# tkwa/iit

Measured on AMD Instinct MI355X. Metric: IIT (base,source) intervened pairs/sec, IOI GPT-2-small, IOI_ModelPair IIT+strict+behavior step, higher is better.
Workload: dtype bf16; 1 GPU; model=gpt2-small 12L/768d/12H (TL GPT-2 cfg, LNPre, gelu_new, V=50257), global_batch=256, seq_len=16, parallelism=dp1, engine=native, graphs=True

## Files before the change

### csrc/attn_mfma.hip

```cpp
#include "common.h"
#include "splice_spec.h"

typedef __attribute__((address_space(3))) i16x4 lds_i16x4_t;

__device__ __forceinline__ bf16x8 half_frag(const i16x4 v) {
  const i16x4 z = {0, 0, 0, 0};
  return __builtin_bit_cast(bf16x8, (i16x8)__builtin_shufflevector(v, z, 0, 1, 2, 3, 4, 5, 6, 7));
}

__device__ __forceinline__ bf16x8 regs_frag(float a, float b, float c, float d) {
  bf16x8 o = {f2bf(a), f2bf(b), f2bf(c), f2bf(d), f2bf(0.f), f2bf(0.f), f2bf(0.f), f2bf(0.f)};
  return o;
}

__device__ __forceinline__ bf16x8 load8(const __bf16* p, bool ok) {
  if (!ok) {
    const i16x8 z = {0, 0, 0, 0, 0, 0, 0, 0};
    return __builtin_bit_cast(bf16x8, z);
  }
  return *(const bf16x8*)p;
}

template <int LDSR>
__device__ __forceinline__ i16x4 tr_block(const __bf16* img, int g, int lane_in_group, int col0) {
  const int q = lane_in_group >> 2, p = lane_in_group & 3;
  return __builtin_amdgcn_ds_read_tr16_b64_v4i16((lds_i16x4_t*)(img + (4 * g + q) * LDSR + col0 + 4 * p));
}


template <int DH, bool SP>
__global__ __launch_bounds__(256) void attn_mfma_fwd_kernel(const __bf16* __restrict__ qkv, __bf16* __restrict__ z,
                                                            float* __restrict__ lse, const __bf16* __restrict__ zsrc,
                                                            unsigned long long head_mask, int BH, int S, int H,
                                                            long ld_qkv, long ld_z, long ld_src, float scale,
                                                            int causal, __bf16* __restrict__ z2, int pair_seqs,
                                                            unsigned long long pair_mask, SpliceSpec sp, int use_sp) {
  constexpr int LDSR = DH + 8;
  __shared__ __attribute__((aligned(16))) __bf16 smem[4][16 * LDSR];
  const int wave = threadIdx.x >> 6, l = threadIdx.x & 63, g = l >> 4, c = l & 15;
  const int bh = blockIdx.x * 4 + wave;
  const bool valid = bh < BH;
  const int b = valid ? bh / H : 0, h = valid ? bh % H : 0;
  const int HD = H * DH;
  const long row0 = (long)b * S;
  const bool patched = valid && ((head_mask >> h) & 1ull);
  const bool mirrored = valid && pair_seqs > 0 && ((pair_mask >> h) & 1ull);
  const bool mirror_base = mirrored && b < pair_seqs;
  const bool mirror_src = mirrored && b >= pair_seqs;
  __bf16* Vs = smem[wave];
  if (valid && !patched && !mirror_base) {
    for (int i = l; i < 16 * DH / 8; i += 64) {
      const int r = i / (DH / 8), ch = i % (DH / 8);
      *(bf16x8*)(Vs + r * LDSR + ch * 8) = load8(qkv + (row0 + r) * ld_qkv + 2 * HD + h * DH + ch * 8, r < S);
    }
  }
  __syncthreads();
  if (!valid) return;
  if (mirror_base) {
    if (lse && l < S) lse[(long)bh * S + l] = 0.f;
    return;
  }
  if (patched) {
    for (int i = l; i < S * DH / 8; i += 64) {
      const int r = i / (DH / 8), ch = i % (DH / 8);
      const uint4 v = *(const uint4*)(zsrc + (row0 + r) * ld_src + h * DH + ch * 8);
      *(uint4*)(z + (row0 + r) * ld_z + h * DH + ch * 8) = v;
      if (z2) *(uint4*)(z2 + (row0 + r) * ld_z + h * DH + ch * 8) = v;
    }
    if (lse && l < S) lse[(long)bh * S + l] = 0.f;
    return;
  }
  f32x4 acc = {0.f, 0.f, 0.f, 0.f};
#pragma unroll
  for (int s = 0; s < DH / 32; ++s) {
    const long off = (row0 + c) * ld_qkv + h * DH + 32 * s + 8 * g;
    const bf16x8 kf = load8(qkv + off + HD, c < S);
    const bf16x8 qf = load8(qkv + off, c < S);
    acc = __builtin_amdgcn_mfma_f32_16x16x32_bf16(kf, qf, acc, 0, 0, 0);
  }
  float sc[4];
  float m = -INFINITY;
#pragma unroll
  for (int r = 0; r < 4; ++r) {
    const int kj = 4 * g + r;
    const bool ok = kj < S && (!causal || kj <= c);
    sc[r] = ok ? acc[r] * scale : -INFINITY;
    m = fmaxf(m, sc[r]);
  }
  m = fmaxf(m, __shfl_xor(m, 16, 64));
  m = fmaxf(m, __shfl_xor(m, 32, 64));
  float p[4], sum = 0.f;
#pragma unroll
  for (int r = 0; r < 4; ++r) {
    p[r] = sc[r] == -INFINITY ? 0.f : __expf(sc[r] - m);
    sum += p[r];
  }
  sum += __shfl_xor(sum, 16, 64);
  sum += __shfl_xor(sum, 32, 64);
  const float inv = sum > 0.f ? 1.f / sum : 0.f;
  if (lse && g == 0 && c < S) lse[(long)bh * S + c] = m + __logf(sum);
  const bf16x8 bp = regs_frag(p[0] * inv, p[1] * inv, p[2] * inv, p[3] * inv);
  f32x4 o[DH / 16];
#pragma unroll
  for (int t = 0; t < DH / 16; ++t) {
    const bf16x8 av = half_frag(tr_block<LDSR>(Vs, g, c, 16 * t));
    const f32x4 zero = {0.f, 0.f, 0.f, 0.f};
    o[t] = __builtin_amdgcn_mfma_f32_16x16x32_bf16(av, bp, zero, 0, 0, 0);
  }
  asm volatile("s_waitcnt lgkmcnt(0)" ::: "memory");
#pragma unroll
  for (int t = 0; t < DH / 16; ++t)
    *(bf16x4*)(Vs + c * LDSR + 16 * t + 4 * g) = bf16x4{f2bf(o[t][0]), f2bf(o[t][1]), f2bf(o[t][2]), f2bf(o[t][3])};
  asm volatile("s_waitcnt lgkmcnt(0)" ::: "memory");
#pragma unroll
  for (int i = l; i < 16 * DH / 8; i += 64) {
    const int r = i / (DH / 8), ch = i % (DH / 8);
    if (r < S) {
      const bf16x8 v = *(const bf16x8*)(Vs + r * LDSR + ch * 8);
      __bf16* zo = z + (row0 + r) * ld_z + h * DH + ch * 8;
      if (SP && use_sp && pair_seqs > 0) {
        const bool base = b < pair_seqs;
        const int bb = base ? b : b - pair_seqs;
        const bool rowsel = in_ranges(sp, 0, bb) && in_ranges(sp, 1, r) && in_ranges(sp, 2, h);
        unsigned m = 0;
        if (rowsel) {
#pragma unroll
          for (int e = 0; e < 8; ++e) m |= (unsigned)in_ranges(sp, 3, ch * 8 + e) << e;
        }
        if (base) {
          if (m == 0) *(bf16x8*)zo = v;
          else if (m != 0xffu) {
#pragma unroll
            for (int e = 0; e < 8; ++e)
              if (!((m >> e) & 1u)) zo[e] = v[e];
          }
        } else {
          *(bf16x8*)zo = v;
          __bf16* zb = z + (row0 - (long)pair_seqs * S + r) * ld_z + h * DH + ch * 8;
          if (m == 0xffu) *(bf16x8*)zb = v;
          else if (m) {
#pragma unroll
            for (int e = 0; e < 8; ++e)
              if ((m >> e) & 1u) zb[e] = v[e];
          }
        }
        continue;
      }
      *(bf16x8*)zo = v;
      if (z2) *(bf16x8*)(z2 + (row0 + r) * ld_z + h * DH + ch * 8) = v;
      if (mirror_src) *(bf16x8*)(z + (row0 - (long)pair_seqs * S + r) * ld_z + h * DH + ch * 8) = v;
    }
  }
}

template <int DH, bool SP>
__global__ __launch_bounds__(256) void attn_mfma_bwd_kernel(const __bf16* __restrict__ qkv, const __bf16* __restrict__ dz,
                                                            const float* __restrict__ lse, __bf16* __restrict__ dqkv,
                                                            unsigned long long head_mask, int BH, int S, int H,
                                                            long ld_qkv, long ld_dz, float scale, int causal,
                                                            SpliceSpec sp, int use_sp) {
  constexpr int LDSR = DH + 8;
  __shared__ __attribute__((aligned(16))) __bf16 smem[4][3][16 * LDSR];
  __shared__ float Dsh[4][16];
  const int wave = threadIdx.x >> 6, l = threadIdx.x & 63, g = l >> 4, c = l & 15;
  const int bh = blockIdx.x * 4 + wave;
  const bool valid = bh < BH;
  const int b = valid ? bh / H : 0, h = valid ? bh % H : 0;
  const int HD = H * DH;
  const long row0 = (long)b * S;
  const bool patched = valid && ((head_mask >> h) & 1ull);
  const bool work = valid && !patched;
  __bf16* Qs = smem[wave][0];
  __bf16* Ks = smem[wave][1];
  __bf16* Gs = smem[wave][2];
  bf16x8 qf[DH / 32], kf[DH / 32], vf[DH / 32], gf[DH / 32];
#pragma unroll
  for (int s = 0; s < DH / 32; ++s) {
    const long off = (row0 + c) * ld_qkv + h * DH + 32 * s + 8 * g;
    const bool ok = work && c < S;
    qf[s] = load8(qkv + off, ok);
    kf[s] = load8(qkv + off + HD, ok);
    vf[s] = load8(qkv + off + 2 * HD, ok);
    gf[s] = load8(dz + (row0 + c) * ld_dz + h * DH + 32 * s + 8 * g, ok);
    if (SP && use_sp && ok && in_ranges(sp, 0, b) && in_ranges(sp, 1, c) && in_ranges(sp, 2, h)) {
#pragma unroll
      for (int e = 0; e < 8; ++e)
        if (in_ranges(sp, 3, 32 * s + 8 * g + e)) gf[s][e] = f2bf(0.f);
    }
    if (work) {
      *(bf16x8*)(Qs + c * LDSR + 32 * s + 8 * g) = qf[s];
      *(bf16x8*)(Ks + c * LDSR + 32 * s + 8 * g) = kf[s];
      *(bf16x8*)(Gs + c * LDSR + 32 * s + 8 * g) = gf[s];
    }
  }
  f32x4 Sa = {0.f, 0.f, 0.f, 0.f}, STa = Sa, dPa = Sa, dPTa = Sa;
#pragma unroll
  for (int s = 0; s < DH / 32; ++s) {
    Sa = __builtin_amdgcn_mfma_f32_16x16x32_bf16(qf[s], kf[s], Sa, 0, 0, 0);
    STa = __builtin_amdgcn_mfma_f32_16x16x32_bf16(kf[s], qf[s], STa, 0, 0, 0);
    dPa = __builtin_amdgcn_mfma_f32_16x16x32_bf16(gf[s], vf[s], dPa, 0, 0, 0);
    dPTa = __builtin_amdgcn_mfma_f32_16x16x32_bf16(vf[s], gf[s], dPTa, 0, 0, 0);
  }
  float P[4], PT[4], Dr[4];
  const float lse_c = (work && c < S) ? lse[(long)bh * S + c] : 0.f;
#pragma unroll
  for (int r = 0; r < 4; ++r) {
    const int qi = 4 * g + r, kj = c;
    const bool ok = work && qi < S && kj < S && (!causal || kj <= qi);
    P[r] = ok ? __expf(Sa[r] * scale - lse[(long)bh * S + qi]) : 0.f;
    const int kj2 = 4 * g + r, qi2 = c;
    const bool ok2 = work && qi2 < S && kj2 < S && (!causal || kj2 <= qi2);
    PT[r] = ok2 ? __expf(STa[r] * scale - lse_c) : 0.f;
    float d = P[r] * dPa[r];
    d += __shfl_xor(d, 1, 64);
    d += __shfl_xor(d, 2, 64);
    d += __shfl_xor(d, 4, 64);
    d += __shfl_xor(d, 8, 64);
    Dr[r] = d;
  }
  if (c == 0) {
#pragma unroll
    for (int r = 0; r < 4; ++r) Dsh[wave][4 * g + r] = Dr[r];
  }
  __syncthreads();
  if (!valid) return;
  __bf16* dq = dqkv + h * DH;
  __bf16* dk = dqkv + HD + h * DH;
  __bf16* dv = dqkv + 2 * HD + h * DH;
  if (patched) {
    for (int i = l; i < S * DH / 8; i += 64) {
      const int r = i / (DH / 8), ch = i % (DH / 8);
      const uint4 zz = make_uint4(0, 0, 0, 0);
      *(uint4*)(dq + (row0 + r) * ld_qkv + ch * 8) = zz;
      *(uint4*)(dk + (row0 + r) * ld_qkv + ch * 8) = zz;
      *(uint4*)(dv + (row0 + r) * ld_qkv + ch * 8) = zz;
    }
    return;
  }
  const float Dc = Dsh[wave][c];
  float dS[4], dST[4];
#pragma unroll
  for (int r = 0; r < 4; ++r) {
    dS[r] = P[r] * (dPa[r] - Dr[r]) * scale;
    dST[r] = PT[r] * (dPTa[r] - Dc) * scale;
  }
  const bf16x8 bP = regs_frag(P[0], P[1], P[2], P[3]);
  const bf16x8 bdS = regs_frag(dS[0], dS[1], dS[2], dS[3]);
  const bf16x8 bdST = regs_frag(dST[0], dST[1], dST[2], dST[3]);
  const f32x4 zero = {0.f, 0.f, 0.f, 0.f};
  f32x4 dvT[DH / 16], dkT[DH / 16], dqT[DH / 16];
#pragma unroll
  for (int t = 0; t < DH / 16; ++t) {
    const bf16x8 aG = half_frag(tr_block<LDSR>(Gs, g, c, 16 * t));
    const bf16x8 aQ = half_frag(tr_block<LDSR>(Qs, g, c, 16 * t));
    const bf16x8 aK = half_frag(tr_block<LDSR>(Ks, g, c, 16 * t));
    dvT[t] = __builtin_amdgcn_mfma_f32_16x16x32_bf16(aG, bP, zero, 0, 0, 0);
    dkT[t] = __builtin_amdgcn_mfma_f32_16x16x32_bf16(aQ, bdS, zero, 0, 0, 0);
    dqT[t] = __builtin_amdgcn_mfma_f32_16x16x32_bf16(aK, bdST, zero, 0, 0, 0);
  }
  asm volatile("s_waitcnt lgkmcnt(0)" ::: "memory");
#pragma unroll
  for (int t = 0; t < DH / 16; ++t) {
    const int o = c * LDSR + 16 * t + 4 * g;
    *(bf16x4*)(Gs + o) = bf16x4{f2bf(dvT[t][0]), f2bf(dvT[t][1]), f2bf(dvT[t][2]), f2bf(dvT[t][3])};
    *(bf16x4*)(Ks + o) = bf16x4{f2bf(dkT[t][0]), f2bf(dkT[t][1]), f2bf(dkT[t][2]), f2bf(dkT[t][3])};
    *(bf16x4*)(Qs + o) = bf16x4{f2bf(dqT[t][0]), f2bf(dqT[t][1]), f2bf(dqT[t][2]), f2bf(dqT[t][3])};
  }
  asm volatile("s_waitcnt lgkmcnt(0)" ::: "memory");
  constexpr int CPR = DH / 8;
#pragma unroll
  for (int i = l; i < 16 * CPR; i += 64) {
    const int r = i / CPR, ch = i % CPR;
    if (r < S) {
      const long o = (row0 + r) * ld_qkv + ch * 8;
      *(bf16x8*)(dv + o) = *(const bf16x8*)(Gs + r * LDSR + ch * 8);
      *(bf16x8*)(dk + o) = *(const bf16x8*)(Ks + r * LDSR + ch * 8);
      *(bf16x8*)(dq + o) = *(const bf16x8*)(Qs + r * LDSR + ch * 8);
    }
  }
}

IIT_EXPORT int iit_attn_mfma_fwd_pair(const void* qkv, void* z, float* lse, const void* zsrc,
                                      unsigned long long head_mask, int B, int S, int H, int dh, long ld_qkv, long ld_z,
                                      long ld_src, float scale, int causal, void* z2, int pair_seqs,
                                      unsigned long long pair_mask, void* stream);

IIT_EXPORT int iit_attn_mfma_fwd(const void* qkv, void* z, float* lse, const void* zsrc, unsigned long long head_mask,
                                 int B, int S, int H, int dh, long ld_qkv, long ld_z, long ld_src, float scale,
                                 int causal, void* stream) {
  return iit_attn_mfma_fwd_pair(qkv, z, lse, zsrc, head_mask, B, S, H, dh, ld_qkv, ld_z, ld_src, scale, causal,
                                nullptr, 0, 0ull, stream);
}

static int attn_fwd_launch(const void* qkv, void* z, float* lse, const void* zsrc, unsigned long long head_mask,
                           int B, int S, int H, int dh, long ld_qkv, long ld_z, long ld_src, float scale, int causal,
                           void* z2, int pair_seqs, unsigned long long pair_mask, const SpliceSpec& sp, int use_sp,
                           void* stream);

IIT_EXPORT int iit_attn_mfma_fwd_pair(const void* qkv, void* z, float* lse, const void* zsrc,
                                      unsigned long long head_mask, int B, int S, int H, int dh, long ld_qkv, long ld_z,
                                      long ld_src, float scale, int causal, void* z2, int pair_seqs,
                                      unsigned long long pair_mask, void* stream) {
  const SpliceSpec none{};
  return attn_fwd_launch(qkv, z, lse, zsrc, head_mask, B, S, H, dh, ld_qkv, ld_z, ld_src, scale, causal, z2,
                         pair_seqs, pair_mask, none, 0, stream);
}

IIT_EXPORT int iit_attn_mfma_fwd_spec(const void* qkv, void* z, float* lse, int B, int S, int H, int dh, long ld_qkv,
                                      long ld_z, float scale, int causal, int pair_seqs, const void* spec,
                                      void* stream) {
  if (pair_seqs <= 0) return (int)hipErrorInvalidValue;
  return attn_fwd_launch(qkv, z, lse, nullptr, 0ull, B, S, H, dh, ld_qkv, ld_z, 0, scale, causal, nullptr, pair_seqs,
                         0ull, *(const SpliceSpec*)spec, 1, stream);
}

static int attn_fwd_launch(const void* qkv, void* z, float* lse, const void* zsrc, unsigned long long head_mask,
                           int B, int S, int H, int dh, long ld_qkv, long ld_z, long ld_src, float scale, int causal,
                           void* z2, int pair_seqs, unsigned long long pair_mask, const SpliceSpec& sp, int use_sp,
                           void* stream) {
  if (S > 16) return (int)hipErrorInvalidValue;
  if (pair_seqs < 0 || (pair_seqs > 0 && 2 * pair_seqs != B)) return (int)hipErrorInvalidValue;
  const int BH = B * H;
  dim3 grid((BH + 3) / 4), block(256);
  hipStream_t s = (hipStream_t)stream;
#define AF(D)                                                                                                       \
  hipLaunchKernelGGL((use_sp ? attn_mfma_fwd_kernel<D, true> : attn_mfma_fwd_kernel<D, false>), grid, block, 0, s,    \
                     (const __bf16*)qkv, (__bf16*)z, lse,                                                           \
                     (const __bf16*)zsrc, head_mask, BH, S, H, ld_qkv, ld_z, ld_src, scale, causal, (__bf16*)z2,    \
                     pair_seqs, pair_mask, sp, use_sp)
  if (dh == 32) AF(32);
  else if (dh == 64) AF(64);
  else if (dh == 96) AF(96);
  else if (dh == 128) AF(128);
  else return (int)hipErrorInvalidValue;
#undef AF
  return hipGetLastError();
}

static int attn_bwd_launch(const void* qkv, const void* dz, const float* lse, void* dqkv, unsigned long long head_mask,
                           int B, int S, int H, int dh, long ld_qkv, long ld_dz, float scale, int causal,
                           const SpliceSpec& sp, int use_sp, void* stream);

IIT_EXPORT int iit_attn_mfma_bwd(const void* qkv, const void* dz, const float* lse, void* dqkv,
                                 unsigned long long head_mask, int B, int S, int H, int dh, long ld_qkv, long ld_dz,
                                 float scale, int causal, void* stream) {
  const SpliceSpec none{};
  return attn_bwd_launch(qkv, dz, lse, dqkv, head_mask, B, S, H, dh, ld_qkv, ld_dz, scale, causal, none, 0, stream);
}

IIT_EXPORT int iit_attn_mfma_bwd_spec(const void* qkv, const void* dz, const float* lse, void* dqkv, int B, int S,
                                      int H, int dh, long ld_qkv, long ld_dz, float scale, int causal,
                                      const void* spec, void* stream) {
  return attn_bwd_launch(qkv, dz, lse, dqkv, 0ull, B, S, H, dh, ld_qkv, ld_dz, scale, causal,
                         *(const SpliceSpec*)spec, 1, stream);
}

static int attn_bwd_launch(const void* qkv, const void* dz, const float* lse, void* dqkv, unsigned long long head_mask,
                           int B, int S, int H, int dh, long ld_qkv, long ld_dz, float scale, int causal,
                           const SpliceSpec& sp, int use_sp, void* stream) {
  if (S > 16) return (int)hipErrorInvalidValue;
  const int BH = B * H;
  dim3 grid((BH + 3) / 4), block(256);
// ... 14 lines not shown
```

### csrc/gemm_dual.hip

```cpp
#include "gemm_glds_body.h"
#include "gemm_tiles.h"
#include "prefetch.h"

namespace {

template <int BM_, int BN_, int NS_, int NW_ = 4, int OCC_ = 2>
struct Cfg {
  static constexpr int BM = BM_, BN = BN_, NS = NS_, NW = NW_, OCC = OCC_;
  static constexpr int SMEM = GldsSmem<BM_, BN_, NS_, NW_, 64, OCC_>::BYTES;
};


template <class TW, int EW, class TX, int EX>
__global__ __launch_bounds__(TW::NW * 64, TW::OCC) void gemm_dual_kernel(G2Args pw, G2Args px, int w_tiles,
                                                                         int w_splits, int x_tiles, Prefetch pf) {
  static_assert(TW::NW == TX::NW && TW::OCC == TX::OCC, "one launch geometry");
  __shared__ __attribute__((aligned(16))) char smem[TW::SMEM > TX::SMEM ? TW::SMEM : TX::SMEM];
  if ((int)blockIdx.x < pf.wgs) {
    prefetch_part(pf, blockIdx.x);
    return;
  }
  const int b = blockIdx.x - pf.wgs;
  const int nw = w_tiles * w_splits;
  if (b < nw) {
    gemm_glds_body<TW::BM, TW::BN, TW::NS, true, true, EW, TW::NW, 64, TW::OCC>(pw, b % w_tiles, w_tiles,
                                                                                b / w_tiles, w_splits, smem);
  } else {
    gemm_glds_body<TX::BM, TX::BN, TX::NS, false, false, EX, TX::NW, 64, TX::OCC>(px, b - nw, x_tiles, 0, 1, smem);
  }
}

template <class TW, int EW, class TX, int EX>
hipError_t launch2(const G2Args& w, const G2Args& x, int w_splits, const Prefetch& pf, hipStream_t s) {
  const int wt = (w.M / TW::BM) * (w.N / TW::BN), xt = (x.M / TX::BM) * (x.N / TX::BN);
  hipLaunchKernelGGL((gemm_dual_kernel<TW, EW, TX, EX>), dim3(pf.wgs + wt * w_splits + xt), dim3(TW::NW * 64), 0, s,
                     w, x, wt, w_splits, xt, pf);
  return hipGetLastError();
}

template <class TW, int EW, int EX>
hipError_t pick_x(const G2Args& w, const G2Args& x, int w_splits, int xtile, const Prefetch& pf, hipStream_t s) {
  switch (xtile) {
#define X(IDX, BM_, BN_, NS_, NW_, OCC_, GLDS)                                          \
  case IDX:                                                                             \
    if constexpr (TW::NW == NW_ && TW::OCC == OCC_)                                     \
      return launch2<TW, EW, Cfg<BM_, BN_, NS_, NW_, OCC_>, EX>(w, x, w_splits, pf, s); \
    break;
    IIT_DUAL_X_TILE_LIST(X)
#undef X
  }
  return hipErrorInvalidValue;
}

template <int EW, int EX>
hipError_t pick_w(const G2Args& w, const G2Args& x, int w_splits, int wtile, int xtile, const Prefetch& pf,
                  hipStream_t s) {
  switch (wtile) {
#define X(IDX, BM, BN, NS, NW, OCC, GLDS) \
  case IDX: return pick_x<Cfg<BM, BN, NS, NW, OCC>, EW, EX>(w, x, w_splits, xtile, pf, s);
    IIT_DUAL_W_TILE_LIST(X)
#undef X
    default: return hipErrorInvalidValue;
  }
}

}

extern "C" int iit_gemm_glds_ok(const void* A, const void* B, const void* C, const void* C2, const void* resid,
                                long lda, long ldb, long ldc, long ldc2, long ldr, int M, int N, int K, int mode,
                                int epi, int bias_cols, int tile, int splits, int reduce);

IIT_EXPORT int iit_gemm_dual_ok(const void* wA, const void* wB, const void* wC, long wlda, long wldb, long wldc, int wM,
                                int wN, int wK, int wepi, int wtile, int wsplits, int reduce, const void* xA,
                                const void* xB, const void* xC, const void* xC2, long xlda, long xldb, long xldc,
                                long xldc2, int xM, int xN, int xK, int xepi, int xtile) {
  const TileRow* wt = find_tile(kDualWRows, wtile);
  const TileRow* xt = find_tile(kDualXRows, xtile);
  if (!wt || !xt || wt->nw != xt->nw || wt->occ != xt->occ) return 0;
  if (!(wepi == E_F32_STORE || wepi == E_F32_ACC) || !(xepi == E_BF16 || xepi == E_DGELU)) return 0;
  if (!iit_gemm_glds_ok(wA, wB, wC, nullptr, nullptr, wlda, wldb, wldc, 0, 0, wM, wN, wK, 3, wepi, 0, wt->aux,
                        wsplits, reduce))
    return 0;
  if (!iit_gemm_glds_ok(xA, xB, xC, xepi == E_DGELU ? xC2 : nullptr, nullptr, xlda, xldb, xldc, xldc2, 0, xM, xN, xK,
                        0, xepi, 0, xt->aux, 1, 0))
    return 0;
  const long wg = (long)(wM / wt->bm) * (wN / wt->bn) * wsplits + (long)(xM / xt->bm) * (xN / xt->bn);
  return wg > 0 && wg < (1L << 31) ? 1 : 0;
}

static int g_dual_group_m = 0;
IIT_EXPORT void iit_gemm_dual_set_group_m(int gm) { g_dual_group_m = gm; }

IIT_EXPORT int iit_gemm_dual(const void* wA, const void* wB, void* wC, long wlda, long wldb, long wldc, int wM, int wN,
                             int wK, int wepi, int wtile, int wsplits, float* ws, int* counters, const void* xA,
                             const void* xB, void* xC, void* xC2, long xlda, long xldb, long xldc, long xldc2, int xM,
                             int xN, int xK, int xepi, int xtile, float* csum, float* bsum, float* gsq,
                             const void* pf0, long pf0_bytes, const void* pf1, long pf1_bytes, int pf_wgs,
                             void* stream) {
  const int reduce = ws != nullptr;
  if (!iit_gemm_dual_ok(wA, wB, wC, wlda, wldb, wldc, wM, wN, wK, wepi, wtile, wsplits, reduce, xA, xB, xC, xC2, xlda,
                        xldb, xldc, xldc2, xM, xN, xK, xepi, xtile))
    return (int)hipErrorInvalidValue;
  if (reduce && !counters) return (int)hipErrorInvalidValue;
  G2Args w{};
  w.A = (const __bf16*)wA; w.B = (const __bf16*)wB; w.C = wC;
  w.lda = wlda; w.ldb = wldb; w.ldc = wldc;
  w.M = wM; w.N = wN; w.K = wK; w.k_per_split = wK / wsplits;
  w.ws = reduce ? ws : nullptr;
  w.counters = reduce ? counters : nullptr;
  w.bsum = bsum;
  w.gsq = wepi == E_F32_STORE ? gsq : nullptr;
  G2Args x{};
  x.A = (const __bf16*)xA; x.B = (const __bf16*)xB; x.C = xC; x.C2 = xC2;
  x.lda = xlda; x.ldb = xldb; x.ldc = xldc; x.ldc2 = xldc2;
  x.M = xM; x.N = xN; x.K = xK; x.k_per_split = xK;
  x.csum = xepi == E_DGELU ? csum : nullptr;
  w.group_m = x.group_m = g_dual_group_m;
  Prefetch pf{{(const char*)pf0, (const char*)pf1}, {pf0 ? pf0_bytes : 0, pf1 ? pf1_bytes : 0}, 0};
  if ((pf.bytes[0] > 0 || pf.bytes[1] > 0) && pf_wgs > 0) pf.wgs = ((pf_wgs + 7) / 8) * 8;
  if (pf.wgs > 1024) pf.wgs = 1024;
  hipStream_t s = (hipStream_t)stream;
  if (wepi == E_F32_STORE && xepi == E_BF16)
    return (int)pick_w<E_F32_STORE, E_BF16>(w, x, wsplits, wtile, xtile, pf, s);
  if (wepi == E_F32_STORE && xepi == E_DGELU)
    return (int)pick_w<E_F32_STORE, E_DGELU>(w, x, wsplits, wtile, xtile, pf, s);
  if (wepi == E_F32_ACC && xepi == E_BF16) return (int)pick_w<E_F32_ACC, E_BF16>(w, x, wsplits, wtile, xtile, pf, s);
  if (wepi == E_F32_ACC && xepi == E_DGELU) return (int)pick_w<E_F32_ACC, E_DGELU>(w, x, wsplits, wtile, xtile, pf, s);
  return (int)hipErrorInvalidValue;
}
```

### csrc/gemm_glds.hip

```cpp
#include "gemm_glds_body.h"
#include "gemm_tiles.h"

namespace {

template <int BM, int BN, int NS, bool AKM, bool BKM, int EPI, int NW, int BK = 64, int OCC = 1>
__global__ __launch_bounds__(NW * 64, OCC) void gemm_glds_kernel(G2Args p) {
  __shared__ __attribute__((aligned(16))) char smem[GldsSmem<BM, BN, NS, NW, BK, OCC>::BYTES];
  gemm_glds_body<BM, BN, NS, AKM, BKM, EPI, NW, BK, OCC>(p, blockIdx.x, gridDim.x, blockIdx.y, gridDim.y, smem);
}

template <int BM, int BN, int NS, bool AKM, bool BKM, int EPI, int NW = 4, int BK = 64, int OCC = 1>
hipError_t launch(const G2Args& a, hipStream_t s) {
  const int tiles = (a.M / BM) * (a.N / BN);
  hipLaunchKernelGGL((gemm_glds_kernel<BM, BN, NS, AKM, BKM, EPI, NW, BK, OCC>), dim3(tiles, a.K / a.k_per_split),
                     dim3(NW * 64), 0, s, a);
  return hipGetLastError();
}

template <bool AKM, bool BKM, int EPI>
hipError_t launch_tile(const G2Args& a, int tile, hipStream_t s) {
  switch (tile) {
#define X(ID, BM, BN, NS, NW, BK, OCC) \
  case ID: return launch<BM, BN, NS, AKM, BKM, EPI, NW, BK, OCC>(a, s);
    IIT_GLDS_TILE_LIST(X)
// ... 27 lines not shown
extern "C" int iit_gemm_8ph_run(const void* args, int mode, int epi, void* stream);
extern "C" int iit_gemm_4w_run(const void* args, int mode, int epi, int bk, void* stream);

IIT_EXPORT int iit_gemm_glds_ok(const void* A, const void* B, const void* C, const void* C2, const void* resid,
                                long lda, long ldb, long ldc, long ldc2, long ldr, int M, int N, int K, int mode,
                                int epi, int bias_cols, int tile, int splits, int reduce) {
  if (tile == IIT_8PH_TILE || tile == IIT_4W_TILE || tile == IIT_4W32_TILE) {
    if (splits != 1 || reduce || !iit_gemm_8ph_ok(M, N, K, mode, epi)) return 0;
    if ((epi == E_DGELU || epi == E_DGELU_ERF) && !C2) return 0;
    if (lda % 8 || ldb % 8 || ldc % 8 || (C2 && ldc2 % 8) || (resid && ldr % 8)) return 0;
    if (((uintptr_t)A | (uintptr_t)B | (uintptr_t)C | (uintptr_t)C2 | (uintptr_t)resid) & 15) return 0;
    if (epi == E_BF16_BIAS3 && bias_cols % 8) return 0;
    return 1;
  }
  const TileRow* t = find_tile(kGldsRows, tile);
  if (!t) return 0;
  if (tile == 20 && mode != 3) return 0;
  const bool split_epi = epi == E_F32_ACC || (reduce && (epi == E_F32_STORE || epi == E_F32_RESID));
  const int bk = t->bk;
  if (splits < 1 || (splits > 1 && (!split_epi || K % (bk * splits)))) return 0;
  if (reduce && splits < 2) return 0;
  if (!combo_ok(mode, epi)) return 0;
  const bool dg = epi == E_DGELU || epi == E_DGELU_ERF;
  if (dg && (mode != 0 || !C2)) return 0;
  if (M <= 0 || N <= 0 || K <= 0 || M % t->bm || N % t->bn || K % bk) return 0;
  if (lda % 8 || ldb % 8 || ldc % 8 || (C2 && ldc2 % 8) || (resid && ldr % 8)) return 0;
  const uintptr_t al = (uintptr_t)A | (uintptr_t)B | (uintptr_t)C | (uintptr_t)C2 | (uintptr_t)resid;
  if (al & 15) return 0;
  if (epi == E_BF16_BIAS3 && bias_cols % 8) return 0;
  return 1;
}

static thread_local long long* g_prof_buf = nullptr;
IIT_EXPORT void iit_gemm_glds_set_prof(void* buf) { g_prof_buf = (long long*)buf; }
static int g_group_m = 0;
IIT_EXPORT void iit_gemm_glds_set_group_m(int gm) { g_group_m = gm; }

IIT_EXPORT int iit_gemm_glds_sm(const void* A, const void* B, void* C, void* C2, const float* bias0,
                                const float* bias1, const float* bias2, const float* resid, long lda, long ldb, long ldc,
                                long ldc2, long ldr, int M, int N, int K, int mode, int epi, int bias_cols, int tile,
                                int splits, float* csum, float* ws, int* counters, int store_mode, float* bsum,
                                float* gsq, void* stream) {
  const int reduce = ws != nullptr;
  if (!iit_gemm_glds_ok(A, B, C, C2, resid, lda, ldb, ldc, ldc2, ldr, M, N, K, mode, epi, bias_cols, tile, splits,
                        reduce))
    return (int)hipErrorInvalidValue;
  if (reduce && !counters) return (int)hipErrorInvalidValue;
  G2Args a{};
  a.A = (const __bf16*)A; a.B = (const __bf16*)B; a.C = C; a.C2 = C2;
  a.bias0 = bias0; a.bias1 = bias1; a.bias2 = bias2; a.resid = resid;
  a.lda = lda; a.ldb = ldb; a.ldc = ldc; a.ldc2 = ldc2; a.ldr = ldr;
  a.M = M; a.N = N; a.K = K; a.bias_cols = bias_cols; a.k_per_split = K / splits;
  a.csum = (epi == E_DGELU || epi == E_DGELU_ERF) ? csum : nullptr;
  a.ws = reduce ? ws : nullptr;
  a.counters = reduce ? counters : nullptr;
  a.store_mode = store_mode;
  a.prof = g_prof_buf;
  g_prof_buf = nullptr;
  a.group_m = g_group_m;
  a.bsum = mode == 3 ? bsum : nullptr;
  a.gsq = epi == E_F32_STORE ? gsq : nullptr;
  hipStream_t s = (hipStream_t)stream;
  if (tile == IIT_8PH_TILE) return iit_gemm_8ph_run(&a, mode, epi, stream);
  if (tile == IIT_4W_TILE) return iit_gemm_4w_run(&a, mode, epi, 64, stream);
  if (tile == IIT_4W32_TILE) return iit_gemm_4w_run(&a, mode, epi, 32, stream);
#define X(MODE, AKM, BKM, EPI) \
  if (mode == (MODE) && epi == (EPI)) return (int)launch_tile<AKM, BKM, EPI>(a, tile, s);
  IIT_GLDS_COMBO_LIST(X)
#undef X
  return (int)hipErrorInvalidValue;
}

IIT_EXPORT int iit_tile_table(int family, TileRow* out, int cap) {
  const TileRow* rows = nullptr;
  int n = 0;
#define FAMILY(F, ROWS) \
  if (family == (F)) rows = ROWS, n = (int)(sizeof(ROWS) / sizeof(TileRow));
  FAMILY(0, kGldsRows)
  FAMILY(1, kEdgeRows)
  FAMILY(2, kDualWRows)
  FAMILY(3, kDualXRows)
  FAMILY(4, kConvRows)
  FAMILY(5, kConvWgRows)
#undef FAMILY
  for (int i = 0; i < n && i < cap; ++i) out[i] = rows[i];
  return n;
}
```

### csrc/gemm_glds_body.h

```cpp
#pragma once
#include <type_traits>

#include "common.h"

namespace {

enum : int { E_BF16 = 0, E_BF16_BIAS3 = 1, E_F32_RESID = 2, E_GELU = 3, E_DGELU = 4, E_F32_ACC = 5,
             E_F32_STORE = 7, E_GELU_ERF = 8, E_DGELU_ERF = 9, E_BF16_CS = 10 };

struct G2Args {
  const __bf16* A;
  const __bf16* B;
  void* C;
  void* C2;
  const float* bias0;
  const float* bias1;
  const float* bias2;
  const float* resid;
  long lda, ldb, ldc, ldc2, ldr;
  int M, N, K, bias_cols;
  int k_per_split;
  float* csum;
  float* ws;
  int* counters;
  int store_mode;
  long long* prof;
  int group_m;
  float* bsum;
  float* gsq;
  const __bf16* zero;
  int conv_h, conv_w, conv_c, conv_flip;
  int conv_sh, conv_sw, conv_k, conv_s, conv_pad;
  float* cstat;
};

__device__ __forceinline__ void prof_mark(long long* prof, int slot, int e, bool on) {
  if (on) prof[(long)slot * 64 + e] = clock64();
}

typedef __attribute__((address_space(3))) void lds_void_t;
typedef __attribute__((address_space(3))) i16x4 lds_i16x4_t;
typedef const __attribute__((address_space(1))) void gbl_void_t;

__device__ __forceinline__ void glds16(const __bf16* g, char* lds_wave_base) {
  __builtin_amdgcn_global_load_lds((gbl_void_t*)g, (lds_void_t*)lds_wave_base, 16, 0, 0);
}

template <int R>
__device__ __forceinline__ int kmaj_swz(int kr) {
  if constexpr (R == 128) return (kr & 3) | (((kr >> 3) & 1) << 2);
  else if constexpr (R == 64) return ((kr >> 1) & 1) | (((kr >> 3) & 1) << 1);
  else return (kr >> 3) & 1;
}

template <int BK>
__device__ __forceinline__ int kcont_swz(int row) {
  if constexpr (BK == 128) return row & 15;
  else if constexpr (BK == 32) return (row >> 2) & 3;
  else return (row >> 1) & 7;
}

template <bool KMAJ, int R, int NW = 4, int BK = 64, bool LEAN = false>
struct Stager {
  static constexpr int RPI = 1024 / (BK * 2);
  static constexpr int N = KMAJ ? BK / (NW * (64 / (R / 8))) : R / (RPI * NW);
  static_assert(N >= 1, "tile too narrow for the workgroup's waves");
  static_assert(!LEAN || NW % 2 == 0, "the lean stager needs an even wave count");
  static constexpr int NP_ = LEAN ? 1 : N;
  const __bf16* ptr[NP_];
  int off[NP_];
  long kstep;
  long istep;
  int ostep;

  __device__ __forceinline__ void init(const __bf16* base, long ld, int r0g, int kbeg, int wave, int lane) {
    if constexpr (!KMAJ) {
      constexpr int CPR = BK / 8;
#pragma unroll
      for (int i = 0; i < NP_; ++i) {
        const int r0 = i * RPI * NW + wave * RPI;
        const int row = r0 + lane / CPR;
        const int c = (lane % CPR) ^ kcont_swz<BK>(row);
        ptr[i] = base + (long)(r0g + row) * ld + kbeg + c * 8;
        off[i] = r0 * BK * 2;
      }
      kstep = BK;
      istep = (long)RPI * NW * ld;
      ostep = RPI * NW * BK * 2;
    } else {
      constexpr int CH = R / 8;
      constexpr int KRI = 64 / CH;
// ... 299 lines not shown
      }
    } else if constexpr (EPI == E_F32_ACC) {
      float* dst = (float*)p.C + (long)row * p.ldc + col;
      add8v(v, pf[2 * k], pf[2 * k + 1]);
      store8_f32(dst, v, p.store_mode);
    } else {
      if (p.bias0) add8(v, p.bias0 + col);
      store8_f32((float*)p.C + (long)row * p.ldc + col, v, p.store_mode);
      if (p.gsq) {
#pragma unroll
        for (int e = 0; e < 8; ++e) sq += v[e] * v[e];
      }
    }
  }
  if constexpr (EPI == E_DGELU || EPI == E_DGELU_ERF) {
    if (p.csum) {
      __syncthreads();
      constexpr int G = NT / BN > 0 ? NT / BN : 1;
      for (int c = tid; c < BN * G; c += NT) {
        const int col = c % BN, g = c / BN;
        float s[8] = {0.f, 0.f, 0.f, 0.f, 0.f, 0.f, 0.f, 0.f};
#pragma unroll
        for (int r0 = g; r0 < ER; r0 += 8 * G)
#pragma unroll
          for (int u = 0; u < 8; ++u)
            if (r0 + u * G < ER) s[u] += E[(r0 + u * G) * EPS + col];
        atomicAdd(p.csum + n0 + col, ((s[0] + s[1]) + (s[2] + s[3])) + ((s[4] + s[5]) + (s[6] + s[7])));
      }
    }
  }
  if constexpr (EPI == E_BF16_CS) {
    __syncthreads();
    static_assert(NT % BN == 0, "column groups");
    constexpr int G = NT / BN;
    const int col = tid % BN, g = tid / BN;
    if (ch == 0) cpiv = E[col];
    for (int r = g; r < ER; r += G) {
      const float d = E[r * EPS + col] - cpiv;
      cs1 += d;
      cs2 = __builtin_fmaf(d, d, cs2);
    }
  }
  }
  if constexpr (EPI == E_BF16_CS) {
    constexpr int G = NT / BN;
    float* red = (float*)smem;
    __syncthreads();
    red[tid] = cs1;
    red[NT + tid] = cs2;
    __syncthreads();
    if (tid < BN) {
      float a = 0.f, b = 0.f;
#pragma unroll
      for (int g = 0; g < G; ++g) {
        a += red[g * BN + tid];
        b += red[NT + g * BN + tid];
      }
      const long T = p.M / BM, tm = m0 / BM, c = n0 + tid;
      p.cstat[c * T + tm] = cpiv;
      p.cstat[((long)p.N + c) * T + tm] = a;
      p.cstat[(2L * p.N + c) * T + tm] = b;
    }
  }
  if constexpr (EPI == E_F32_STORE) {
    if (p.gsq) {
      sq = wave_sum(sq);
      float* red = (float*)smem;
      __syncthreads();
      if (lane == 0) red[wave] = sq;
      __syncthreads();
      if (tid == 0) {
        float t = 0.f;
#pragma unroll
        for (int w = 0; w < NW; ++w) t += red[w];
        atomicAdd(p.gsq + (lin & 63), t);
      }
    }
  }
}

template <int BM, int BN, int NS, bool AKM, bool BKM, int EPI, int NW, int BK = 64, int OCC = 1, bool LEAN = false,
          class ASTG = void, class BSTG = void, bool EDGE = false>
__device__ __forceinline__ void gemm_glds_body(const G2Args& p, const int lin, const int nlin, const int split,
                                               const int nsplit, char* smem) {
  using SA = std::conditional_t<std::is_void_v<ASTG>, OperandStager<AKM, BM, NW, BK, LEAN>, ASTG>;
  using SB = std::conditional_t<std::is_void_v<BSTG>, OperandStager<BKM, BN, NW, BK, LEAN>, BSTG>;
  constexpr int HALVES = BK / 64;
  constexpr int NT = NW * 64;
  constexpr int WMR = NW / 2;
  constexpr int WM = BM / WMR, WN = BN / 2;
  constexpr int TM = WM / 16, TN = WN / 16;
  constexpr int A_BYTES = BM * BK * 2, B_BYTES = BN * BK * 2;
  constexpr int STAGE = A_BYTES + B_BYTES;
  constexpr int LOADS = SA::N + SB::N;
  using SM = GldsSmem<BM, BN, NS, NW, BK, OCC>;
  constexpr int EPS = SM::EPS;
  constexpr int ECH = SM::ECH;
  static_assert(SM::BYTES <= SM::LDS_BUDGET, "LDS budget");
  static_assert(STAGE == SM::STAGE, "stage size");

  constexpr bool TR = EPI != E_F32_ACC;
  const int tid = threadIdx.x, lane = tid & 63, wave = tid >> 6;
  const int wm = wave >> 1, wn = wave & 1;
  static_assert(!EDGE || (BKM && !std::is_void_v<BSTG>), "the edge variant stages its k-major B itself");
  const int tiles_n = EDGE ? (p.N + BN - 1) / BN : p.N / BN;
  const int t = xcd_remap(lin, nlin);
  int tm, tn;
  grouped_tile(t, p.M / BM, tiles_n, tm, tn, p.group_m > 0 ? p.group_m : 8);
  const int m0 = tm * BM, n0 = tn * BN;
  const int kbeg = split * p.k_per_split;
  const int nt = p.k_per_split / BK;
  const bool prof_on = p.prof != nullptr && tid == 0;
  const int prof_slot = split * nlin + lin;
  if (prof_on) {
    p.prof[(long)prof_slot * 64 + 63] = wall_clock64();
    prof_mark(p.prof, prof_slot, 0, true);
  }

  f32x4 acc[TM][TN];
  constexpr bool CS = AKM && BKM && (EPI == E_F32_ACC || EPI == E_F32_STORE);
  const bool do_cs = CS && p.bsum != nullptr && tm == 0 && wm == 0;
  float cs[CS ? TN : 1];
#pragma unroll
  for (int j = 0; j < (CS ? TN : 1); ++j) cs[j] = 0.f;
#pragma unroll
  for (int i = 0; i < TM; ++i)
#pragma unroll
    for (int j = 0; j < TN; ++j) acc[i][j] = f32x4{0.f, 0.f, 0.f, 0.f};

  RawFrag<AKM> ca[TM], na[TM];
  RawFrag<BKM> cb[TN], nb[TN];
  SA stA;
  SB stB;
  if constexpr (std::is_void_v<ASTG>) stA.init(p.A, p.lda, m0, kbeg, wave, lane);
  else stA.init(p, m0, kbeg, wave, lane);
  if constexpr (std::is_void_v<BSTG>) stB.init(p.B, p.ldb, n0, kbeg, wave, lane);
  else stB.init(p, n0, kbeg, wave, lane);
#pragma unroll
  for (int s = 0; s < NS; ++s)
    if (s < nt) {
      char* buf = smem + s * STAGE;
      stA.stage(s, buf);
      stB.stage(s, buf + A_BYTES);
    }
  wait_tiles<LOADS>(min(NS - 1, nt - 1));
  __builtin_amdgcn_s_barrier();
  prof_mark(p.prof, prof_slot, 1, prof_on);
#pragma unroll
  for (int i = 0; i < TM; ++i) frag_issue_t<AKM, BM, BK>(smem, wm * WM + i * 16, 0, lane, ca[i]);
#pragma unroll
  for (int j = 0; j < TN; ++j) frag_issue_t<BKM, BN, BK>(smem + A_BYTES, wn * WN + j * 16, 0, lane, cb[j]);

  for (int kt = 0; kt < nt; ++kt) {
    const char* sa = smem + (kt % NS) * STAGE;
    const char* sb = sa + A_BYTES;
#pragma unroll
    for (int h = 0; h < HALVES; ++h) {
    asm volatile("s_waitcnt lgkmcnt(0)" ::: "memory");
    __builtin_amdgcn_sched_barrier(0);
#pragma unroll
    for (int i = 0; i < TM; ++i) frag_issue_t<AKM, BM, BK>(sa, wm * WM + i * 16, h * 64 + 32, lane, na[i]);
#pragma unroll
    for (int j = 0; j < TN; ++j) frag_issue_t<BKM, BN, BK>(sb, wn * WN + j * 16, h * 64 + 32, lane, nb[j]);
    __builtin_amdgcn_sched_barrier(0);
    {
      bf16x8 a[TM], b[TN];
#pragma unroll
// ... 69 lines not shown
    __builtin_amdgcn_sched_barrier(0);
    }
  }
  prof_mark(p.prof, prof_slot, 61, prof_on);
  if constexpr (CS) {
    if (do_cs) {
#pragma unroll
      for (int j = 0; j < TN; ++j) {
        float v = cs[j];
        v += __shfl_xor(v, 16);
        v += __shfl_xor(v, 32);
        if (lane < 16 && (!EDGE || n0 + wn * WN + j * 16 + lane < p.N))
          atomicAdd(p.bsum + n0 + wn * WN + j * 16 + lane, v);
      }
    }
  }
  if constexpr (EPI == E_F32_ACC || EPI == E_F32_STORE || EPI == E_F32_RESID || EPI == E_BF16 || EPI == E_BF16_CS) {
    if (p.ws != nullptr) {
      const long tile_elems = (long)BM * BN;
      f32x4* mine = (f32x4*)(p.ws + ((long)split * nlin + t) * tile_elems);
#pragma unroll
      for (int i = 0; i < TM; ++i)
#pragma unroll
        for (int j = 0; j < TN; ++j)
          asm volatile("global_store_dwordx4 %0, %1, off sc1" ::"v"(mine + (i * TN + j) * NT + tid), "v"(acc[i][j])
                       : "memory");
      asm volatile("s_waitcnt vmcnt(0)" ::: "memory");
      __syncthreads();
      int* flag = (int*)smem;
      if (tid == 0) {
        const int last = atomicAdd(p.counters + t, 1) == nsplit - 1;
        if (last) __hip_atomic_store(p.counters + t, 0, __ATOMIC_RELAXED, __HIP_MEMORY_SCOPE_AGENT);
        flag[0] = last;
      }
      __syncthreads();
      if (!flag[0]) return;
      f32x4 sum[TM][TN];
#pragma unroll
      for (int i = 0; i < TM; ++i)
#pragma unroll
        for (int j = 0; j < TN; ++j) sum[i][j] = f32x4{0.f, 0.f, 0.f, 0.f};
      for (int sp = 0; sp < nsplit; ++sp) {
        if (sp == split) {
#pragma unroll
          for (int i = 0; i < TM; ++i)
#pragma unroll
            for (int j = 0; j < TN; ++j) sum[i][j] += acc[i][j];
          continue;
        }
        const f32x4* other = (const f32x4*)(p.ws + ((long)sp * nlin + t) * tile_elems);
        f32x4 v[TM][TN];
#pragma unroll
        for (int i = 0; i < TM; ++i)
#pragma unroll
          for (int j = 0; j < TN; ++j)
            asm volatile("global_load_dwordx4 %0, %1, off sc1" : "=v"(v[i][j]) : "v"(other + (i * TN + j) * NT + tid)
                         : "memory");
        asm volatile("s_waitcnt vmcnt(0)" ::: "memory");
#pragma unroll
        for (int i = 0; i < TM; ++i)
#pragma unroll
          for (int j = 0; j < TN; ++j) sum[i][j] += v[i][j];
      }
#pragma unroll
      for (int i = 0; i < TM; ++i)
#pragma unroll
        for (int j = 0; j < TN; ++j) acc[i][j] = sum[i][j];
    }
  }
  if constexpr (EPI == E_F32_ACC) {
    if (nsplit > 1 && p.ws == nullptr) {
#pragma unroll
      for (int i = 0; i < TM; ++i)
#pragma unroll
        for (int j = 0; j < TN; ++j) {
          const int col = n0 + wn * WN + j * 16 + (lane & 15);
          const int row = m0 + wm * WM + i * 16 + 4 * (lane >> 4);
#pragma unroll
          for (int r = 0; r < 4; ++r) unsafeAtomicAdd((float*)p.C + (long)(row + r) * p.ldc + col, acc[i][j][r]);
        }
      return;
    }
  }
  glds_epilogue<BM, BN, EPI, NT, ECH, SM::EPS, EDGE>(p, smem, m0, n0, lin, [&](float* E, int ch) {
    if (wm / (WMR / ECH) == ch) {
#pragma unroll
      for (int i = 0; i < TM; ++i)
#pragma unroll
        for (int j = 0; j < TN; ++j) {
          if constexpr (TR) {
            const int col = wn * WN + j * 16 + 4 * (lane >> 4);
            const int row = (wm % (WMR / ECH)) * WM + i * 16 + (lane & 15);
            *(f32x4*)(E + row * EPS + col) = acc[i][j];
          } else {
            const int col = wn * WN + j * 16 + (lane & 15);
            const int row = (wm % (WMR / ECH)) * WM + i * 16 + 4 * (lane >> 4);
#pragma unroll
            for (int r = 0; r < 4; ++r) E[(row + r) * EPS + col] = acc[i][j][r];
          }
        }
    }
  });
  if (p.prof != nullptr) {
    asm volatile("s_waitcnt vmcnt(0)" ::: "memory");
    __syncthreads();
    prof_mark(p.prof, prof_slot, 62, prof_on);
    if (prof_on) p.prof[(long)prof_slot * 64 + 60] = wall_clock64();
  }
}

}
```

### csrc/gemm_tiles.h

```cpp
#pragma once

struct TileRow { int id, bm, bn, bk, ns, nw, occ, aux; };

#define IIT_GLDS_TILE_LIST(X)                                                                                         \
  X(0, 128, 128, 3, 4, 64, 1) X(1, 128, 64, 4, 4, 64, 1) X(2, 64, 128, 4, 4, 64, 1) X(3, 64, 64, 4, 4, 64, 1)         \
            \
  X(5, 256, 192, 2, 8, 64, 1) X(6, 128, 128, 4, 8, 64, 1) X(7, 256, 128, 2, 8, 64, 1)                                 \
      \
                                                 \
  X(8, 96, 96, 4, 4, 64, 1)                                                                                           \
            \
  X(9, 128, 96, 4, 4, 64, 1)                                                                                          \
       \
                \
  X(10, 96, 192, 4, 4, 64, 1) X(11, 192, 96, 4, 4, 64, 1)                                                             \
      \
  X(12, 96, 96, 6, 4, 64, 1) X(13, 128, 96, 5, 4, 64, 1) X(14, 64, 64, 8, 4, 64, 1)                                   \
         \
  X(15, 128, 96, 2, 4, 128, 1) X(16, 96, 96, 3, 4, 128, 1) X(17, 64, 64, 4, 4, 128, 1) X(18, 128, 128, 2, 4, 128, 1)  \
      \
        \
                                                                \
                \
                                                         \
  X(20, 192, 192, 2, 4, 64, 1)                                                                                        \
                        \
  X(21, 192, 128, 4, 4, 64, 1) X(22, 128, 192, 4, 4, 64, 1)                                                           \
            \
                                    \
  X(23, 128, 96, 2, 4, 64, 2) X(24, 64, 96, 3, 4, 64, 2) X(25, 128, 128, 2, 4, 64, 2)                                 \
  X(26, 96, 96, 3, 4, 64, 2) X(27, 128, 192, 2, 4, 64, 2) X(28, 64, 192, 2, 4, 64, 2)                                 \
        \
  X(29, 64, 96, 2, 4, 64, 3) X(30, 64, 64, 2, 4, 64, 4) X(31, 64, 128, 2, 4, 64, 3)                                   \
      \
                                           \
  X(32, 256, 128, 3, 8, 64, 1) X(33, 128, 256, 3, 8, 64, 1) X(34, 256, 256, 2, 8, 64, 1)                              \
      \
        \
                                            \
  X(4, 128, 128, 4, 4, 64, 1)
#define IIT_GLDS_BIG_TILE_LIST(X) X(40, 256, 256, 2, 8, 64, 1) X(41, 256, 256, 2, 4, 64, 1) X(42, 256, 256, 4, 4, 64, 1)

#define IIT_EDGE_TILE_LIST(X) X(0, 128, 128, 3, 4, 1) X(7, 256, 128, 2, 8, 1) X(25, 128, 128, 2, 4, 2)

#define IIT_DUAL_W_TILE_LIST(X)                                                                                  \
  X(0, 128, 96, 2, 4, 2, 23) X(1, 128, 128, 2, 4, 2, 25) X(2, 96, 96, 3, 4, 2, 26) X(3, 64, 96, 3, 4, 2, 24)     \
  X(4, 64, 64, 4, 4, 2, 3)                                                                                       \
  X(5, 256, 128, 2, 8, 1, 7) X(6, 128, 128, 4, 8, 1, 6)                                                          \
  X(7, 128, 128, 4, 4, 1, 4) X(8, 128, 96, 4, 4, 1, 13)
#define IIT_DUAL_X_TILE_LIST(X)                                                                                  \
  X(0, 128, 96, 2, 4, 2, 23) X(1, 64, 96, 3, 4, 2, 24) X(2, 128, 192, 2, 4, 2, 27) X(3, 128, 128, 2, 4, 2, 25)   \
  X(4, 256, 192, 2, 8, 1, 5) X(5, 256, 128, 2, 8, 1, 7) X(6, 128, 128, 4, 8, 1, 6)                               \
  X(7, 128, 128, 4, 4, 1, 4) X(8, 128, 192, 3, 4, 1, 22)

#define IIT_CONV_TILE_LIST(X)                                                 \
  X(0, 128, 64, 4, 4, 1) X(1, 128, 128, 3, 4, 1) X(2, 64, 64, 4, 4, 2)        \
  X(3, 128, 128, 2, 4, 2) X(4, 64, 128, 2, 4, 3) X(5, 128, 64, 2, 4, 2)
#define IIT_CONV_WG_TILE_LIST(X) X(0, 64, 64, 4) X(1, 128, 64, 4) X(2, 128, 128, 3) X(3, 64, 128, 4)

#define IIT_ROW_GLDS(ID, BM, BN, NS, NW, BK, OCC) {ID, BM, BN, BK, NS, NW, OCC, 0},
#define IIT_ROW_K64(ID, BM, BN, NS, NW, OCC) {ID, BM, BN, 64, NS, NW, OCC, 0},
#define IIT_ROW_DUAL(ID, BM, BN, NS, NW, OCC, GLDS) {ID, BM, BN, 64, NS, NW, OCC, GLDS},
#define IIT_ROW_WG(ID, BM, BN, NS) {ID, BM, BN, 64, NS, 4, 1, 0},
constexpr TileRow kGldsRows[] = {IIT_GLDS_TILE_LIST(IIT_ROW_GLDS) IIT_GLDS_BIG_TILE_LIST(IIT_ROW_GLDS)};
constexpr TileRow kEdgeRows[] = {IIT_EDGE_TILE_LIST(IIT_ROW_K64)};
constexpr TileRow kDualWRows[] = {IIT_DUAL_W_TILE_LIST(IIT_ROW_DUAL)};
constexpr TileRow kDualXRows[] = {IIT_DUAL_X_TILE_LIST(IIT_ROW_DUAL)};
constexpr TileRow kConvRows[] = {IIT_CONV_TILE_LIST(IIT_ROW_K64)};
constexpr TileRow kConvWgRows[] = {IIT_CONV_WG_TILE_LIST(IIT_ROW_WG)};

template <int N>
constexpr const TileRow* find_tile(const TileRow (&rows)[N], int id) {
  for (int i = 0; i < N; ++i)
    if (rows[i].id == id) return &rows[i];
  return nullptr;
}

constexpr bool same_tile(const TileRow& r, const TileRow* g, bool ring) {
  return g && g->bm == r.bm && g->bn == r.bn && g->bk == r.bk &&
         (!ring || (g->ns == r.ns && g->nw == r.nw && g->occ == r.occ));
}
constexpr bool tile_lists_agree() {
  for (const TileRow& r : kEdgeRows)
    if (!same_tile(r, find_tile(kGldsRows, r.id), true)) return false;
  for (const TileRow& r : kDualWRows)
    if (!same_tile(r, find_tile(kGldsRows, r.aux), false)) return false;
  for (const TileRow& r : kDualXRows)
    if (!same_tile(r, find_tile(kGldsRows, r.aux), false)) return false;
  return true;
}
static_assert(tile_lists_agree(), "gemm_tiles.h: an edge or dual row disagrees with the glds row it names");
```

### iit_amd/ops/build.py

```python
from __future__ import annotations

import hashlib
import os
import subprocess
import sys

ROOT = os.path.dirname(os.path.dirname(os.path.dirname(os.path.abspath(__file__))))
CSRC = os.path.join(ROOT, "csrc")
OUT_DIR = os.path.join(ROOT, "iit_amd", "_native")
LIB = os.path.join(OUT_DIR, "libiit_hip.so")
OBJ_CACHE = os.path.join(ROOT, "build", "objcache")
SOURCES = ["gemm.hip", "gemm_glds.hip", "gemm_edge.hip", "gemm_dual.hip", "gemm_8ph.hip", "gemm_4w.hip", "conv_nhwc.hip", "kernels.hip", "layer_norm.hip", "attn_mfma.hip", "flash_attn.hip", "llama_ops.hip",
           "splice.hip", "ioi_hl.hip", "bn_nhwc.hip", "gemm_f32.hip", "attn_fp32.hip", "block_f32.hip"]
EXTRA_FLAGS = {"gemm_glds.hip": ["-mllvm", "-amdgpu-mfma-vgpr-form"], "gemm_edge.hip": ["-mllvm", "-amdgpu-mfma-vgpr-form"], "conv_nhwc.hip": ["-mllvm", "-amdgpu-mfma-vgpr-form"], "gemm_dual.hip": ["-mllvm", "-amdgpu-mfma-vgpr-form"],
               "gemm_8ph.hip": ["-mllvm", "-amdgpu-mfma-vgpr-form"]}
HEADERS = ["common.h", "gemm_glds_body.h", "gemm_tiles.h", "gemm_w4.h", "splice_spec.h", "prefetch.h"]
ARCH = os.environ.get("IIT_OFFLOAD_ARCH", "gfx950")


def _hipcc() -> str:
    for c in (os.environ.get("HIPCC"), "/opt/rocm/bin/hipcc"):
        if c and os.path.exists(c):
            return c
    return "hipcc"


def sources():
    return [os.path.join(CSRC, s) for s in SOURCES if os.path.exists(os.path.join(CSRC, s))]


def source_hash() -> str:
    h = hashlib.sha256()
    for p in sources() + [os.path.join(CSRC, h) for h in HEADERS]:
        with open(p, "rb") as f:
            h.update(f.read())
    h.update(ARCH.encode())
    h.update(repr(sorted(EXTRA_FLAGS.items())).encode())
    return h.hexdigest()[:16]


def is_up_to_date() -> bool:
    stamp = LIB + ".stamp"
    return os.path.exists(LIB) and os.path.exists(stamp) and open(stamp).read().strip() == source_hash()


def _obj_key(src: str) -> str:
    h = hashlib.sha256()
    for p in [src] + [os.path.join(CSRC, x) for x in HEADERS]:
        with open(p, "rb") as f:
            h.update(f.read())
    h.update(ARCH.encode())
    h.update(repr(EXTRA_FLAGS.get(os.path.basename(src), [])).encode())
    return h.hexdigest()[:16]


def build(force: bool = False, verbose: bool = False) -> str:
    if not force and is_up_to_date():
        return LIB
    os.makedirs(OBJ_CACHE, exist_ok=True)
    objs = []
    procs = []
    for src in sources():
        obj = os.path.join(OBJ_CACHE, f"{os.path.basename(src)}.{_obj_key(src)}.o")
        objs.append(obj)
        if os.path.exists(obj) and not force:
            continue
        cmd = [_hipcc(), f"--offload-arch={ARCH}", "-O3", "-std=c++17", "-fPIC", "-munsafe-fp-atomics",
               "-I", CSRC, "-c", src, "-o", obj + ".tmp"] + EXTRA_FLAGS.get(os.path.basename(src), [])
        procs.append((cmd, obj, subprocess.Popen(cmd, stdout=subprocess.PIPE, stderr=subprocess.STDOUT)))
    for cmd, obj, p in procs:
        out, _ = p.communicate()
        if p.returncode != 0:
            raise RuntimeError(f"hipcc failed: {' '.join(cmd)}\n{out.decode(errors='replace')}")
        os.replace(obj + ".tmp", obj)
        if verbose and out:
            print(out.decode(errors="replace"))
    tmp = LIB + ".tmp"
    cmd = [_hipcc(), f"--offload-arch={ARCH}", "-shared", "-fPIC", "-o", tmp] + objs
    res = subprocess.run(cmd, stdout=subprocess.PIPE, stderr=subprocess.STDOUT)
    if res.returncode != 0:
        raise RuntimeError(f"link failed: {res.stdout.decode(errors='replace')}")
    os.replace(tmp, LIB)
    keep = set(objs)
    for f in os.listdir(OBJ_CACHE):
        if os.path.join(OBJ_CACHE, f) not in keep:
            os.remove(os.path.join(OBJ_CACHE, f))
    with open(LIB + ".stamp", "w") as f:
        f.write(source_hash())
    return LIB


if __name__ == "__main__":
    print(build(force="--force" in sys.argv, verbose=True))
```

### iit_amd/ops/gemm_dispatch.py

```python
from __future__ import annotations

import os
import re
from typing import Dict, Optional, Tuple

import torch
import torch.nn.functional as F

from . import hip_kernels as K

POLICY = os.environ.get("IIT_GEMM", "auto")
DECISIONS: Dict[Tuple, Tuple[str, Dict[str, float]]] = {}
FORCE: Dict[Tuple, str] = {}
TIMING = None
BF16, F32 = torch.bfloat16, torch.float32
_BLAS_OK = {}
_BLAS_SELECTED = False


def select_graph_safe_blas() -> None:
    global _BLAS_SELECTED
    if _BLAS_SELECTED or not torch.cuda.is_available():
        return
    _BLAS_SELECTED = True
# ... 491 lines not shown

            def _passes(c):
                if sc_bs is not None:
                    K_.colsum_accum(B, ldb, sc_bs, Kd, N)
                if sc_sq is not None:
                    K_.sumsq_2d(c, ldc, M, N, sc_sq)

            timed = {name: (lambda c, c2, c3, f=f: f(c, c2, c3, bs=sc_bs, sq=sc_sq)) if name.startswith("glds") else
                     (lambda c, c2, c3, f=f: (f(c, c2, c3), _passes(c)))
                     for name, f in calls.items()}
        try:
            times = {name: min(_time(lambda f=f: f(sc, sc2, sc3)) for _ in range(2)) for name, f in timed.items()}
            for name in sorted(times, key=times.get)[:3] if len(times) > 1 else ():
                f = timed[name]
                times[name] = min(_time(lambda f=f: f(sc, sc2, sc3), reps=30) for _ in range(3))
        finally:
            if box is not None:
                box[0] = colsum
        best = min(times, key=times.get)
        choice = DECISIONS[key] = (best, times)
    if _decide_only:
        return choice[1][choice[0]]
    name = FORCE.get(key, choice[0])
    if name not in calls:
        name = choice[0]
    if _SPLIT_STORE and "s+hip" in calls:
        name = "s+hip"
    if _TRACE and key not in _TRACED:
        _TRACED.add(key)
        print(f"[gemm] {key!r} -> {name}", flush=True)
    if TIMING is not None:
        s_ev, e_ev = torch.cuda.Event(enable_timing=True), torch.cuda.Event(enable_timing=True)
        s_ev.record()
        _run(name)
        e_ev.record()
        TIMING.append((key, name, s_ev, e_ev))
        return name
    return _run(name)


K_ = K

DUAL = os.environ.get("IIT_GEMM_DUAL", "1") != "0"
DUAL_DECISIONS: Dict[Tuple, Tuple[str, Dict[str, float]]] = {}
_DUAL_X_EPIS = (K.EPI_BF16, K.EPI_DGELU)
_DUAL_W_EPIS = (K.EPI_F32_STORE, K.EPI_F32_ACC)


def _dual_eligible(x: dict, w: dict) -> bool:
    return (DUAL and POLICY == "auto" and x["A"].is_cuda and x.get("mode", 0) == 0 and x.get("epi", 0) in _DUAL_X_EPIS
            and w.get("mode") == (K.MODE_AKM | K.MODE_BKM) and w.get("epi") in _DUAL_W_EPIS
            and all(x.get(k) is None for k in ("bias0", "resid", "C2", "splits"))
            and all(w.get(k) is None for k in ("bias0", "resid", "C2", "splits", "aux", "colsum")))


def _dual_specs(x: dict, w: dict, xc, wc, csum, bsum=None, gsq=None):
    ws = dict(A=w["A"], B=w["B"], C=wc, M=w["M"], N=w["N"], K=w["K"], lda=w["lda"], ldb=w["ldb"], ldc=w["ldc"],
              epi=w["epi"], bsum=bsum, gsq=gsq)
    xs = dict(A=x["A"], B=x["B"], C=xc, C2=x.get("aux"), M=x["M"], N=x["N"], K=x["K"], lda=x["lda"], ldb=x["ldb"],
              ldc=x["ldc"], ldc2=x.get("ldc2", 0), epi=x["epi"], csum=csum)
    return ws, xs


def _dual_candidates(x: dict, w: dict, xc, wc, csum, bsum=None, gsq=None):
    ws, xs = _dual_specs(x, w, xc, wc, csum, bsum, gsq)
    det = deterministic()
    out = {}
    for wt in K.DUAL_W_TILES:
        for xt in K.DUAL_X_TILES:
            if not K.dual_family_ok(wt, xt):
                continue
            for sp, red in ((1, False), (2, True), (4, True), (8, True), (2, False), (4, False), (8, False)):
                if not red and sp > 1 and (w["epi"] != K.EPI_F32_ACC or det):
                    continue
                if sp > 1 and w["K"] // sp < 256:
                    continue
                if K.gemm_dual_ok(ws, xs, wt, xt, sp, red) and not _excluded(
                        f"dual{wt}.{xt}" + (f"{'r' if red else 'k'}{sp}" if sp > 1 else "")):
                    out[f"dual{wt}.{xt}" + (f"{'r' if red else 'k'}{sp}" if sp > 1 else "")] = \
                        lambda wt=wt, xt=xt, sp=sp, red=red: K.gemm_dual(ws, xs, wt, xt, sp, red)
    return out


def gemm_pair(x: dict, w: dict, prefetch=None) -> Optional[str]:
    def serial():
        gemm(**x)
        return gemm(**w)

    if not _dual_eligible(x, w):
        return serial()
    fresh = bool(w.get("fresh")) and w["epi"] == K.EPI_F32_STORE
    key = ("dual", x["M"], x["N"], x["K"], x["epi"], x.get("colsum") is not None,
           w["M"], w["N"], w["K"], w["epi"], fresh, deterministic())
    choice = DUAL_DECISIONS.get(key)
    if choice is None:
        shipped = _table().get(repr(key))
        if shipped is not None and not _excluded(shipped):
            choice = DUAL_DECISIONS[key] = (shipped, {shipped: float("nan")})
    if choice is None:
        if torch.cuda.is_current_stream_capturing():
            return serial()
        _frozen_miss(key)
        xc = _scratch(x["C"], x["M"], max(x["ldc"], x["N"]))
        wc = _scratch(w["C"], w["M"], max(w["ldc"], w["N"]))
        cs = torch.zeros_like(x["colsum"]) if x.get("colsum") is not None else None
        bs = torch.zeros_like(w["bsum"]) if w.get("bsum") is not None else None
        sq = torch.zeros_like(w["gsq"]) if w.get("gsq") is not None else None
        calls = _dual_candidates(x, w, xc, wc, cs, bs, sq)
        calls["serial"] = lambda: (gemm(**{**x, "C": xc, "colsum": cs}),
                                   gemm(**{**w, "C": wc, "bsum": bs, "gsq": sq}))
        times = {n: min(_time(f) for _ in range(2)) for n, f in calls.items()}
        for n in sorted(times, key=times.get)[:3] if len(times) > 1 else ():
            times[n] = min(_time(calls[n], reps=30) for _ in range(3))
        best = min(times, key=times.get)
        choice = DUAL_DECISIONS[key] = (best, times)
    name = FORCE.get(key, choice[0])
    cfg = _parse_dual(name)
    ws, xs = _dual_specs(x, w, x["C"], w["C"], x.get("colsum"), w.get("bsum"), w.get("gsq"))
    if cfg is None or not K.gemm_dual_ok(ws, xs, *cfg):
        name, cfg = "serial", None
    s_ev = e_ev = None
    if TIMING is not None:
        s_ev, e_ev = torch.cuda.Event(enable_timing=True), torch.cuda.Event(enable_timing=True)
        s_ev.record()
    if cfg is None:
        res = serial()
    else:
        K.gemm_dual(ws, xs, *cfg, prefetch=prefetch)
        res = name
    if TIMING is not None:
        e_ev.record()
        TIMING.append((key, name, s_ev, e_ev))
    return res


def _parse_dual(name: str):
    import re
    m = re.fullmatch(r"dual(\d+)\.(\d+)(?:([rk])(\d+))?", name)
    if m is None:
        return None
    return int(m.group(1)), int(m.group(2)), int(m.group(4) or 1), m.group(3) == "r"

_TABLE_PATH = os.path.join(os.path.dirname(os.path.abspath(__file__)), "tuned", "gemm_decisions_gfx950.json")
_TABLE = None
_RAGGED_TABLE: Dict[str, bool] = {}
_EDGE_TABLE: Dict[str, str] = {}


def _edge_table() -> Dict[str, str]:
    _table()
    return _EDGE_TABLE


def _ragged_table() -> Dict[str, bool]:
    _table()
    return _RAGGED_TABLE


def _table() -> Dict[str, str]:
    global _TABLE
    if _TABLE is None:
        _TABLE = {}
        _RAGGED_TABLE.clear()
        _EDGE_TABLE.clear()
        path = os.environ.get("IIT_GEMM_TABLE", _TABLE_PATH)
        if path != "0" and os.path.exists(path) and torch.cuda.is_available():
            import json
            try:
                with open(path) as f:
                    data = json.load(f)
                arch = getattr(torch.cuda.get_device_properties(0), "gcnArchName", "").split(":")[0]
                if data.get("arch") == arch:
                    _TABLE = dict(data.get("decisions", {}))
                    _RAGGED_TABLE.update({k: bool(v) for k, v in data.get("ragged", {}).items()})
                    _EDGE_TABLE.update({k: str(v) for k, v in data.get("edge", {}).items()})
            except (OSError, ValueError) as e:
                print(f"[iit] GEMM decision table not loaded ({e})")
    return _TABLE


def sync_decisions(group=None) -> int:
    import torch.distributed as dist
    if not (dist.is_available() and dist.is_initialized()) or dist.get_world_size(group) == 1:
        return 0
    ws = dist.get_world_size(group)
    mine = {"gemm": dict(DECISIONS), "dual": dict(DUAL_DECISIONS), "ragged": dict(RAGGED)}
    every = [None] * ws
    dist.all_gather_object(every, mine, group=group)
    changed = 0
    for name, table in (("gemm", DECISIONS), ("dual", DUAL_DECISIONS), ("ragged", RAGGED)):
        merged = {}
        for r in reversed(range(ws)):
            merged.update(every[r][name])
        for k, v in merged.items():
            old = table.get(k)
            if old is None or old[0] != v[0]:
                changed += 1
            table[k] = v
    return changed


def export_table(path: str) -> int:
    import json
    dec = {repr(k): v[0] for k, v in DECISIONS.items()}
    dec.update({repr(k): v[0] for k, v in DUAL_DECISIONS.items()})
    ragged = {repr(k): bool(v[0]) for k, v in RAGGED.items() if v[0] is not None}
    arch = getattr(torch.cuda.get_device_properties(0), "gcnArchName", "").split(":")[0] \
        if torch.cuda.is_available() else None
    with open(path, "w") as f:
        json.dump({"arch": arch, "device": torch.cuda.get_device_name(0) if torch.cuda.is_available() else None,
                   "decisions": dec, "ragged": ragged, "edge": {repr(k): v for k, v in EDGE.items() if v}}, f,
# ... 18 lines not shown
```

### iit_amd/ops/hip_kernels.py

```python
from __future__ import annotations

import ctypes
import math
import os
from typing import Optional, Sequence

import numpy as np
import torch

from . import build as _build

c_void_p, c_long, c_int, c_float, c_ull = ctypes.c_void_p, ctypes.c_long, ctypes.c_int, ctypes.c_float, ctypes.c_ulonglong

EPI_BF16, EPI_BF16_BIAS3, EPI_F32_RESID, EPI_GELU, EPI_DGELU, EPI_F32_ACC, EPI_F32_ACC_QKV, EPI_F32_STORE = range(8)
EPI_GELU_ERF = 8
EPI_DGELU_ERF = 9
MODE_NN, MODE_AKM, MODE_BKM, MODE_AF32, MODE_BF32 = 0, 1, 2, 4, 8

_LIB = None
GEMM_GROUP_M = 4
GEMM_DUAL_GROUP_M = 2

_SIGS = {
    "iit_gemm": [c_void_p] * 10 + [c_long] * 5 + [c_int] * 12 + [c_void_p],
# ... 11 lines not shown
    "iit_attn_f32_lds": [c_int] * 3,
    "iit_attn_f32_waves": [c_int] * 3,
    "iit_attn_f32_ok": [c_void_p] * 4 + [c_int] * 4,
    "iit_attn_f32_fwd": [c_void_p] * 6 + [c_int] * 4 + [c_float, c_int, c_void_p],
    "iit_attn_f32_bwd": [c_void_p] * 9 + [c_int] * 4 + [c_float, c_int, c_void_p],
    "iit_gemm_glds_ok": [c_void_p] * 5 + [c_long] * 5 + [c_int] * 9,
    "iit_gemm_glds_sm": [c_void_p] * 8 + [c_long] * 5 + [c_int] * 8 + [c_void_p] * 3 + [c_int] + [c_void_p] * 3,
    "iit_embed_pos_fwd": [c_void_p, c_void_p, c_void_p, c_void_p, c_int, c_int, c_int, c_void_p],
    "iit_embed_pos_bwd": [c_void_p, c_void_p, c_void_p, c_void_p, c_int, c_int, c_int, c_void_p],
    "iit_ln_fwd": [c_void_p] * 7 + [c_int, c_int, c_float, c_ull, c_int, c_int, c_void_p],
    "iit_ln_fwd_pf": [c_void_p] * 7 + [c_int, c_int, c_float, c_ull, c_int, c_int, c_void_p, c_long, c_void_p, c_long,
                      c_int, c_void_p],
    "iit_ln_bwd": [c_void_p, c_int, c_void_p, c_int] + [c_void_p] * 10 + [c_int, c_int, c_int, c_ull, c_int, c_void_p],
    "iit_ln_bwd_part_rows": [],
    "iit_attn_small_fwd": [c_void_p] * 4 + [c_ull, c_int, c_int, c_int, c_int, c_long, c_long, c_long, c_float, c_int,
                                            c_void_p],
    "iit_attn_small_bwd": [c_void_p] * 4 + [c_ull, c_int, c_int, c_int, c_int, c_long, c_long, c_float, c_int, c_void_p],
    "iit_attn_mfma_fwd": [c_void_p] * 4 + [c_ull, c_int, c_int, c_int, c_int, c_long, c_long, c_long, c_float, c_int,
                                           c_void_p],
    "iit_attn_mfma_fwd_pair": [c_void_p] * 4 + [c_ull, c_int, c_int, c_int, c_int, c_long, c_long, c_long, c_float,
                                                c_int, c_void_p, c_int, c_ull, c_void_p],
    "iit_attn_mfma_bwd": [c_void_p] * 4 + [c_ull, c_int, c_int, c_int, c_int, c_long, c_long, c_float, c_int, c_void_p],
    "iit_attn_mfma_fwd_spec": [c_void_p] * 3 + [c_int] * 4 + [c_long, c_long, c_float, c_int, c_int, c_void_p,
                                                               c_void_p],
    "iit_attn_mfma_bwd_spec": [c_void_p] * 4 + [c_int] * 4 + [c_long, c_long, c_float, c_int, c_void_p, c_void_p],
    "iit_ce_fwd": [c_void_p, c_long, c_void_p, c_void_p, c_void_p, c_void_p, c_int, c_int, c_void_p],
    "iit_ce_bwd": [c_void_p, c_long, c_void_p, c_void_p, c_void_p, c_float, c_void_p, c_long, c_int, c_int, c_int,
                   c_void_p, c_void_p],
    "iit_gemm_glds_edge_ok": [c_void_p] * 4 + [c_long] * 3 + [c_int] * 6,
    "iit_gemm_glds_edge": [c_void_p] * 4 + [c_long] * 3 + [c_int] * 7 + [c_void_p, c_void_p, c_int, c_void_p],
    "iit_gemm_edge_plan": [c_int, c_int, c_long, c_int, c_int, c_void_p],
    "iit_ce_bwd16": [c_void_p, c_long, c_void_p, c_void_p, c_void_p, c_float, c_void_p, c_long, c_int, c_int, c_void_p],
    "iit_adam_flat": [c_void_p] * 6 + [c_int, c_void_p, c_int] + [c_float] * 6 + [c_void_p] * 3
                     + [c_void_p, c_int, c_void_p, c_void_p],
    "iit_sumsq_2d": [c_void_p, c_long, c_int, c_int, c_void_p, c_void_p],
    "iit_kl_rows": [c_void_p, c_long, c_void_p, c_long, c_int, c_int, c_void_p, c_void_p],
    "iit_adam_span_size": [],
    "iit_sumsq_spans": [c_void_p, c_void_p, c_int, c_void_p, c_int, c_int, c_void_p, c_void_p],
    "iit_adam_spans": [c_void_p] * 6 + [c_int, c_void_p] + [c_float] * 6 + [c_void_p] * 4,
    "iit_gelu_fwd": [c_void_p, c_long, c_void_p, c_long, c_int, c_int, c_int, c_void_p],
    "iit_shadow_refresh": [c_void_p, c_int, c_void_p],
    "iit_shadow_desc_size": [],
    "iit_colsum_accum": [c_void_p, c_int, c_long, c_void_p, c_int, c_int, c_void_p],
    "iit_dgelu": [c_void_p, c_void_p, c_void_p, c_long, c_int, c_void_p],
    "iit_add_bf16": [c_void_p, c_long, c_void_p, c_long, c_void_p, c_long, c_void_p, c_int, c_int, c_void_p],
    "iit_device_sync": [],
    "iit_zero_chunks": [c_void_p, c_void_p, c_int, c_void_p],
    "iit_zero_ranges": [c_void_p, c_void_p, c_void_p, c_int, c_void_p],
    "iit_colsum_multi": [c_void_p] * 6 + [c_int, c_void_p],
    "iit_rms_fwd": [c_void_p, c_int, c_void_p, c_void_p, c_void_p, c_int, c_int, c_float, c_void_p],
    "iit_rms_bwd": [c_void_p, c_void_p, c_int, c_void_p, c_void_p, c_void_p, c_void_p, c_int, c_int, c_void_p],
    "iit_rms_bwd_res": [c_void_p, c_void_p, c_int, c_void_p, c_void_p, c_void_p, c_void_p, c_void_p, c_int, c_int,
                        c_void_p],
    "iit_rotary": [c_void_p, c_long, c_long, c_long, c_void_p, c_void_p, c_void_p] + [c_int] * 8 + [c_void_p],
    "iit_swiglu_fwd": [c_void_p, c_void_p, c_void_p, c_long, c_void_p],
    "iit_swiglu_bwd": [c_void_p] * 5 + [c_long, c_void_p],
    "iit_swiglu_splice_fwd": [c_void_p] * 4 + [c_long, c_void_p, c_void_p],
    "iit_sparse_pair": [c_void_p, c_long, c_long, c_void_p, c_int, c_void_p],
    "iit_gemm_dual_set_group_m": [c_int],
    "iit_swiglu_splice_bwd": [c_void_p] * 5 + [c_long, c_void_p, c_void_p],
    "iit_embed_splice_fwd": [c_void_p, c_void_p, c_long, c_void_p, c_void_p, c_long, c_int, c_void_p, c_void_p],
    "iit_embed_splice_bwd": [c_void_p, c_void_p, c_int, c_void_p, c_long, c_long, c_int, c_void_p, c_void_p],
    "iit_flash_fwd": [c_void_p] * 3 + [c_void_p, c_void_p, c_void_p, c_void_p, c_void_p, c_void_p, c_ull] + [c_int] * 5
                     + [c_float, c_int, c_void_p, c_void_p],
    "iit_flash_bwd": [c_void_p] * 3 + [c_void_p] * 11 + [c_ull] + [c_int] * 5 + [c_float, c_int, c_void_p, c_void_p],
    "iit_flash_fwd_blocks": [c_void_p] * 3 + [c_void_p, c_void_p, c_void_p, c_void_p, c_void_p, c_void_p, c_ull]
                            + [c_int] * 5 + [c_float, c_int, c_void_p, c_void_p, c_int],
    "iit_flash_bwd_blocks": [c_void_p] * 3 + [c_void_p] * 11 + [c_ull] + [c_int] * 5 + [c_float, c_int, c_void_p,
                                                                                       c_void_p, c_int],
    "iit_flash_plan": [c_int] * 6 + [c_void_p],
    "iit_splice": [c_void_p, c_void_p, c_void_p, c_long, c_void_p, c_int, c_int, c_float, c_void_p],
    "iit_splice_spec_size": [],
    "iit_bn_fwd": [c_void_p] * 8 + [c_long, c_int, c_float, c_int, c_int, c_void_p, c_float, c_void_p, c_void_p,
                                    c_void_p, c_int, c_int, c_int, c_int, c_void_p],
    "iit_bn_bwd": [c_void_p] * 7 + [c_long, c_int, c_int, c_void_p, c_void_p, c_void_p, c_void_p, c_void_p, c_void_p,
                                    c_int, c_int, c_int, c_int, c_void_p],
    "iit_gemm_glds_set_prof": [c_void_p],
    "iit_maxpool3s2_fwd": [c_void_p] * 3 + [c_int] * 5 + [c_void_p],
    "iit_bn_ws_floats": [c_int],
    "iit_maxpool3s2_bwd": [c_void_p] * 3 + [c_int] * 5 + [c_void_p],
    "iit_gemm_dual_ok": [c_void_p] * 3 + [c_long] * 3 + [c_int] * 7 + [c_void_p] * 4 + [c_long] * 4 + [c_int] * 5,
    "iit_gemm_dual": [c_void_p] * 3 + [c_long] * 3 + [c_int] * 6 + [c_void_p] * 2 + [c_void_p] * 4 + [c_long] * 4
                     + [c_int] * 5 + [c_void_p] * 3 + [c_void_p, c_long, c_void_p, c_long, c_int, c_void_p],
    "iit_gemm_glds_set_group_m": [c_int],
    "iit_ioi_hl_label": [c_void_p, c_void_p, c_void_p, c_int, c_int, c_int, c_int, c_int, c_void_p, c_void_p],
    "iit_tile_table": [c_int, c_void_p, c_int],
    "iit_conv2d_ok": [c_long] + [c_int] * 12,
    "iit_conv2d": [c_void_p] * 4 + [c_long] + [c_int] * 12 + [c_void_p] * 4,
    "iit_conv2d_wgrad_ok": [c_long] + [c_int] * 11,
    "iit_conv2d_wgrad": [c_void_p] * 4 + [c_long] + [c_int] * 12 + [c_void_p] * 3,
    "iit_bn_fwd_tiles": [c_void_p] * 4 + [c_int, c_int] + [c_void_p] * 4 + [c_long, c_int, c_float, c_int, c_void_p,
                                                                           c_float, c_void_p, c_void_p],
}


def lib():
    global _LIB
    if _LIB is None:
        if not _build.is_up_to_date():
            _build.build()
        L = ctypes.CDLL(_build.LIB)
        for name, argtypes in _SIGS.items():
            fn = getattr(L, name)
            fn.argtypes = argtypes
            fn.restype = c_int
        check_tile_tables(L)
        _LIB = L
        gm = os.environ.get("IIT_GEMM_GROUP_M", str(GEMM_GROUP_M))
        if gm:
            L.iit_gemm_glds_set_group_m(int(gm))
        dgm = os.environ.get("IIT_GEMM_DUAL_GROUP_M", str(GEMM_DUAL_GROUP_M))
        if dgm:
            L.iit_gemm_dual_set_group_m(int(dgm))
    return _LIB


TILE_FAMILIES = ("glds", "edge", "dual_w", "dual_x", "conv", "conv_wgrad")
TILE_FIELDS = ("bm", "bn", "bk", "ns", "nw", "occ", "aux")


def tile_table(family: str, L=None) -> dict:
    L = L or lib()
    fam = TILE_FAMILIES.index(family)
    n = L.iit_tile_table(fam, None, 0)
    buf = (c_int * (8 * n))()
    L.iit_tile_table(fam, buf, n)
    return {buf[8 * i]: dict(zip(TILE_FIELDS, buf[8 * i + 1:8 * i + 8])) for i in range(n)}


def check_tile_tables(L=None) -> None:
    ours = {"glds": GLDS_TILES, "edge": {t: GLDS_TILES.get(t) for t in GLDS_EDGE_TILES}, "conv": CONV_TILES,
            "conv_wgrad": CONV_WG_TILES, "dual_w": {t: v + DUAL_W_WAVES.get(t, ()) for t, v in DUAL_W_TILES.items()},
            "dual_x": {t: v + DUAL_X_WAVES.get(t, ()) for t, v in DUAL_X_TILES.items()}}
    for family, mine in ours.items():
        theirs = {t: (r["bm"], r["bn"], r["nw"], r["occ"])[:4 if family.startswith("dual") else 2]
                  for t, r in tile_table(family, L).items()}
        for t in sorted(set(mine) | set(theirs)):
            if mine.get(t) != theirs.get(t):
                raise RuntimeError(f"tile table {family!r}, tile {t}: hip_kernels.py has {mine.get(t)}, the library "
                                   f"has {theirs.get(t)} (csrc/gemm_tiles.h)")


def available() -> bool:
    try:
        lib()
        return True
    except Exception:
        return False


def _p(t: Optional[torch.Tensor]):
    return None if t is None else t.data_ptr()


def _stream():
    return torch.cuda.current_stream().cuda_stream


CHECK_BOUNDS = os.environ.get("IIT_CHECK_BOUNDS", "0") == "1"


def _avail(t: torch.Tensor) -> int:
    st = t.untyped_storage()
    return (st.nbytes() - (t.data_ptr() - st.data_ptr())) // t.element_size()


def _bounds(what: str, *spans):
    for name, t, rows, cols, ld in spans:
        if t is None or rows <= 0 or cols <= 0:
            continue
        need = (rows - 1) * ld + cols
        have = _avail(t)
        if need > have or ld < cols and rows > 1:
            raise RuntimeError(f"{what}: operand {name} needs {rows}x{cols} (ld {ld}) = {need} elements, "
                               f"storage holds {have} (shape {tuple(t.shape)}, stride {t.stride()})")


def _check(rc: int, what: str):
    if rc != 0:
        raise RuntimeError(f"{what} failed with hip error {rc}")


N_CU = 256


def _tiling(M: int, N: int, K: int, allow_split: bool):
    t128 = math.ceil(M / 128) * math.ceil(N / 128)
    if t128 >= 240:
        return 1, 1
    t64 = math.ceil(M / 64) * math.ceil(N / 64)
    splits = 1
    if allow_split and t64 < 240 and K >= 1024:
        splits = max(1, min(math.ceil(480 / t64), K // 512))
    return 0, splits


def gemm(A, B, C, *, M: int, N: int, K: int, lda: int, ldb: int, ldc: int, mode: int = MODE_NN, epi: int = EPI_BF16,
         C2=None, C3=None, bias0=None, bias1=None, bias2=None, resid=None, ldr: int = 0, aux=None, ldc2: int = 0,
         bias_cols: int = 0, qkv=(0, 0, 0), atomic: bool = False, splits: Optional[int] = None):
    can_split = epi in (EPI_F32_ACC, EPI_F32_ACC_QKV)
    big, auto_splits = _tiling(M, N, K, can_split)
    if splits is None:
        splits = auto_splits
    if CHECK_BOUNDS:
        _gemm_bounds("iit_gemm", A, B, C, C2, resid, M, N, K, lda, ldb, ldc, ldc2, ldr, mode, qkv)
    rc = lib().iit_gemm(_p(A), _p(B), _p(C), _p(C2), _p(C3), _p(bias0), _p(bias1), _p(bias2), _p(resid), _p(aux),
                        lda, ldb, ldc, ldc2, ldr, M, N, K, mode, epi, splits, big, bias_cols, qkv[0], qkv[1], qkv[2],
                        int(atomic), _stream())
    _check(rc, "iit_gemm")


GLDS_TILES = {0: (128, 128), 1: (128, 64), 2: (64, 128), 3: (64, 64), 4: (128, 128),
              5: (256, 192),
              6: (128, 128), 7: (256, 128),
              8: (96, 96),
              9: (128, 96),
# ... 209 lines not shown
    n = pre.numel()
    _vec_f32("dgelu_f32", n, dpost=dpost, pre=pre, dpre=dpre)
    if not lib().iit_dgelu_f32_ok(_p(dpost), _p(pre), _p(dpre), n):
        raise ValueError(f"dgelu_f32: iit_dgelu_f32_ok refuses n={n}")
    _check(lib().iit_dgelu_f32(_p(dpost), _p(pre), _p(dpre), n, _stream()), "iit_dgelu_f32")


ATTN_F32_LDS_MAX = 160 * 1024
ATTN_F32_MAX_S = ATTN_F32_MAX_DH = 64


def attn_f32_lds(S: int, dh: int, backward: bool) -> int:
    return int(lib().iit_attn_f32_lds(S, dh, int(backward))) * attn_f32_waves(S, dh, backward)


def attn_f32_waves(S: int, dh: int, backward: bool) -> int:
    return int(lib().iit_attn_f32_waves(S, dh, int(backward)))


def _attn_f32_why(ts: dict) -> Optional[str]:
    shape = None
    for name, t in ts.items():
        if not isinstance(t, torch.Tensor) or t.dim() != 4:
            return f"{name} must be a [B][S][H][dh] tensor"
        if not t.is_cuda or t.dtype != torch.float32:
            return f"{name} must be fp32 on the GPU, got {t.dtype} on {t.device}"
        shape = shape or tuple(t.shape)
        if tuple(t.shape) != shape:
            return f"{name} has shape {tuple(t.shape)}, expected {shape}"
        if t.shape[3] > 1 and t.stride(3) != 1:
            return f"{name} must have unit stride on its last dimension, got stride {t.stride()}"
    B, S, H, dh = shape
    if min(shape) < 1 or S > ATTN_F32_MAX_S or dh > ATTN_F32_MAX_DH:
        return f"shape {shape} outside 1 <= S <= {ATTN_F32_MAX_S}, 1 <= dh <= {ATTN_F32_MAX_DH}"
    ptrs = [_p(t) for t in ts.values()][:4]
    ptrs += ptrs[:1] * (4 - len(ptrs))
    if not lib().iit_attn_f32_ok(*ptrs, B, S, H, dh):
        return f"iit_attn_f32_ok refuses shape {shape}"
    return None


def attn_f32_ok(q, k, v) -> bool:
    return _attn_f32_why({"q": q, "k": k, "v": v}) is None


def _strides3(*ts):
    vals = [s for t in ts for s in t.stride()[:3]]
    return (c_long * len(vals))(*vals)


def _attn_f32_check(what: str, ts: dict, lse):
    why = _attn_f32_why(ts)
    if why is None:
        B, S, H, _ = next(iter(ts.values())).shape
        if not (lse.is_cuda and lse.dtype == torch.float32 and tuple(lse.shape) == (B, H, S) and lse.is_contiguous()):
            why = f"lse must be contiguous fp32 [B][H][S] on the GPU, got {lse.dtype} {tuple(lse.shape)}"
    if why is not None:
        raise ValueError(f"{what}: {why}")


def attn_f32_fwd(q, k, v, z, lse, scale: float, causal: bool):
    _attn_f32_check("attn_f32_fwd", {"q": q, "k": k, "v": v, "z": z}, lse)
    B, S, H, dh = q.shape
    _check(lib().iit_attn_f32_fwd(_p(q), _p(k), _p(v), _p(z), _p(lse), _strides3(q, k, v, z), B, S, H, dh, scale,
                                  int(causal), _stream()), "iit_attn_f32_fwd")


def attn_f32_bwd(q, k, v, do, lse, dq, dk, dv, scale: float, causal: bool):
    _attn_f32_check("attn_f32_bwd", {"q": q, "k": k, "v": v, "do": do, "dq": dq, "dk": dk, "dv": dv}, lse)
    B, S, H, dh = q.shape
    _check(lib().iit_attn_f32_bwd(_p(q), _p(k), _p(v), _p(do), _p(lse), _p(dq), _p(dk), _p(dv),
                                  _strides3(q, k, v, do, dq, dk, dv), B, S, H, dh, scale, int(causal), _stream()),
           "iit_attn_f32_bwd")


DUAL_W_TILES = {0: (128, 96), 1: (128, 128), 2: (96, 96), 3: (64, 96), 4: (64, 64),
                5: (256, 128), 6: (128, 128), 7: (128, 128), 8: (128, 96)}
DUAL_X_TILES = {0: (128, 96), 1: (64, 96), 2: (128, 192), 3: (128, 128),
                4: (256, 192), 5: (256, 128), 6: (128, 128), 7: (128, 128), 8: (128, 192)}


DUAL_W_WAVES = {0: (4, 2), 1: (4, 2), 2: (4, 2), 3: (4, 2), 4: (4, 2), 5: (8, 1), 6: (8, 1), 7: (4, 1), 8: (4, 1)}
DUAL_X_WAVES = {0: (4, 2), 1: (4, 2), 2: (4, 2), 3: (4, 2), 4: (8, 1), 5: (8, 1), 6: (8, 1), 7: (4, 1), 8: (4, 1)}


def dual_family_ok(wtile: int, xtile: int) -> bool:
    return DUAL_W_WAVES[wtile] == DUAL_X_WAVES[xtile]


def _bf16_cuda(*ts) -> bool:
    return all(t is not None and t.is_cuda and t.dtype == torch.bfloat16 for t in ts)


def gemm_dual_ok(w: dict, x: dict, wtile: int, xtile: int, splits: int = 1, reduce: bool = False) -> bool:
    if not _bf16_cuda(w["A"], w["B"], x["A"], x["B"]):
        return False
    return bool(lib().iit_gemm_dual_ok(
        _p(w["A"]), _p(w["B"]), _p(w["C"]), w["lda"], w["ldb"], w["ldc"], w["M"], w["N"], w["K"], w["epi"], wtile,
        splits, int(reduce), _p(x["A"]), _p(x["B"]), _p(x["C"]), _p(x.get("C2")), x["lda"], x["ldb"], x["ldc"],
        x.get("ldc2", 0), x["M"], x["N"], x["K"], x["epi"], xtile))


def gemm_dual(w: dict, x: dict, wtile: int, xtile: int, splits: int = 1, reduce: bool = False,
              prefetch=None) -> None:
    ws = cnt = None
    if reduce:
        ws, cnt = split_workspace(w["M"], w["N"], DUAL_W_TILES[wtile], splits, w["A"].device)
    if CHECK_BOUNDS:
        _gemm_bounds("iit_gemm_dual(dW)", w["A"], w["B"], w["C"], None, None, w["M"], w["N"], w["K"], w["lda"],
                     w["ldb"], w["ldc"], 0, 0, MODE_AKM | MODE_BKM)
        _gemm_bounds("iit_gemm_dual(dX)", x["A"], x["B"], x["C"], x.get("C2"), None, x["M"], x["N"], x["K"],
                     x["lda"], x["ldb"], x["ldc"], x.get("ldc2", 0), 0, MODE_NN)
        _bounds("iit_gemm_dual", ("csum", x.get("csum"), 1, x["N"], x["N"]))
    _check(lib().iit_gemm_dual(
        _p(w["A"]), _p(w["B"]), _p(w["C"]), w["lda"], w["ldb"], w["ldc"], w["M"], w["N"], w["K"], w["epi"], wtile,
        splits, _p(ws), _p(cnt), _p(x["A"]), _p(x["B"]), _p(x["C"]), _p(x.get("C2")), x["lda"], x["ldb"], x["ldc"],
        x.get("ldc2", 0), x["M"], x["N"], x["K"], x["epi"], xtile, _p(x.get("csum")), _p(w.get("bsum")),
        _p(w.get("gsq")) if w["epi"] == EPI_F32_STORE else None, *_prefetch_args(prefetch), _stream()),
        "iit_gemm_dual")


_PF_PER_MB = float(os.environ.get("IIT_DUAL_PREFETCH_WGS_PER_MB", "16"))


def _prefetch_args(prefetch):
    ts = [t for t in (prefetch or ()) if t is not None and t.is_cuda and t.is_contiguous()
          and t.numel() * t.element_size() >= 64][:2]
    if not ts or _PF_PER_MB <= 0:
        return (None, 0, None, 0, 0)
    ts += [None] * (2 - len(ts))
    nb = [t.numel() * t.element_size() // 64 * 64 if t is not None else 0 for t in ts]
    wgs = max(8, min(1024, int(sum(nb) / 2 ** 20 * _PF_PER_MB)))
    return (_p(ts[0]), nb[0], _p(ts[1]), nb[1], wgs)


def kl_rows(a, b):
    R, V = a.shape
    out = torch.empty(R, 4, dtype=torch.float32, device=a.device)
    if CHECK_BOUNDS:
        _bounds("kl_rows", ("a", a, R, V, a.stride(0)), ("b", b, R, V, b.stride(0)))
    _check(lib().iit_kl_rows(_p(a), a.stride(0), _p(b), b.stride(0), R, V, _p(out), _stream()), "kl_rows")
    return out


_ADAM_SPAN4 = int(os.environ.get("IIT_ADAM_SPAN4", "1024"))


def sumsq_2d(c, ldc: int, M: int, N: int, gsq) -> None:
    if CHECK_BOUNDS:
        _bounds("sumsq_2d", ("c", c, M, N, ldc))
    _check(lib().iit_sumsq_2d(_p(c), ldc, M, N, _p(gsq), _stream()), "sumsq_2d")


def sumsq_spans(g, spans, nspans, part, step_dev, do_norm: bool):
    _check(lib().iit_sumsq_spans(_p(g), _p(spans), nspans, _p(part), part.numel(), int(do_norm), _p(step_dev),
                                 _stream()), "sumsq_spans")


def adam_spans(flat, g, m, v, spans, nspans, total, step_dev, *, lr, b1, b2, eps, wd, clip_norm, skipped=None,
               hyper=None):
    _check(lib().iit_adam_spans(_p(flat.data), _p(g), _p(m), _p(v), _p(flat.shadow), _p(spans), nspans, _p(total),
                                float(clip_norm or 0.0), lr, b1, b2, eps, wd, _p(hyper), _p(step_dev), _p(skipped),
                                _stream()), "adam_spans")


def splice(act, src, out, n, spec_ptr, f32, mode, scale=1.0):
    if CHECK_BOUNDS:
        _bounds("iit_splice", ("act", act, 1, n, n), ("out", out, 1, n, n))
    _check(lib().iit_splice(_p(act), _p(src), _p(out), n, spec_ptr, int(f32), int(mode), float(scale), _stream()),
           "iit_splice")


def embed_pos_fwd(tokens, W_E, W_pos, out, B, S, d):
    _check(lib().iit_embed_pos_fwd(_p(tokens), _p(W_E), _p(W_pos), _p(out), B * S, S, d, _stream()), "embed_pos_fwd")


def embed_pos_bwd(tokens, g, dWE, dWpos, B, S, d):
    _check(lib().iit_embed_pos_bwd(_p(tokens), _p(g), _p(dWE), _p(dWpos), B, S, d, _stream()), "embed_pos_bwd")


def prefetch_wgs(nbytes: int, per_mb: float) -> int:
    gran = int(nbytes) // 64
    if gran <= 0 or per_mb <= 0:
        return 0
    return max(1, min(1024, gran, int(nbytes / 2 ** 20 * per_mb)))


def _ln_prefetch_args(prefetch, wgs):
    ts = [t for t in (prefetch or ()) if t is not None and t.is_cuda and t.is_contiguous()][:2]
    nb = [t.numel() * t.element_size() // 64 * 64 for t in ts]
    if wgs is None:
        wgs = prefetch_wgs(sum(nb), _PF_PER_MB)
    if not any(nb) or wgs <= 0:
        return (None, 0, None, 0, 0)
    ts += [None] * (2 - len(ts))
    nb += [0] * (2 - len(nb))
    return (_p(ts[0]), nb[0], _p(ts[1]), nb[1], int(wgs))


def _ln_fwd(what, x, w, b, y, y32, mean, rstd, T, d, eps, pos_mask=0, S=1, Tb=0, prefetch=None,
            pf_wgs=None) -> int:
    if CHECK_BOUNDS:
# ... 536 lines not shown
```

### iit_amd/ops/hip_ops.py

```python
from __future__ import annotations

import math
import os
from typing import Optional, Sequence

import torch
from torch.autograd import Function

from ..engine import grad_hooks
from . import hip_kernels as K
from .gemm_dispatch import gemm, gemm_pair
from .torch_ops import TorchOps, act_fn

BF16 = torch.bfloat16
F32 = torch.float32


def _pad8(n: int) -> int:
    return (n + 7) // 8 * 8


def _grad_slot(p: Optional[torch.Tensor]) -> Optional[torch.Tensor]:
    if p is None or not p.requires_grad:
        return None
    g = p.grad
    if g is None:
        flat = getattr(p, "_iit_flat", None)
        if flat is not None and flat.owns(p):
            return flat.bind_zero(p)
        g = torch.zeros_like(p, memory_format=torch.contiguous_format)
        p.grad = g
    return g


def _settle_claim(choice, *ps) -> None:
    if choice is not None and choice.startswith("z+"):
        ps[0]._iit_flat.unclaim(*ps)


def _claim_store(*ps) -> bool:
    if any(p is None or not p.requires_grad for p in ps):
        return False
    flat = getattr(ps[0], "_iit_flat", None)
    if flat is None or not all(flat.owns(p) for p in ps):
        return False
    return flat.claim(*ps)


_FUSE_BIAS = os.environ.get("IIT_FUSED_BIAS_SUMS", "1") != "0"
_FUSE_BIAS_MAX_N = int(os.environ.get("IIT_FUSED_BIAS_MAX_N", str(1 << 30)))


def _fused_bias(gb: Optional[torch.Tensor], N: int) -> Optional[torch.Tensor]:
    if gb is None or not _FUSE_BIAS or not gb.is_cuda or gb.dtype != F32 or not gb.is_contiguous() or \
            gb.numel() != N or N > _FUSE_BIAS_MAX_N:
        return None
    from .gemm_dispatch import deterministic
    return None if deterministic() else gb


def _norm_slots(store: bool, *ps) -> Optional[torch.Tensor]:
    flat = getattr(ps[0], "_iit_flat", None)
    if flat is None:
        return None
    flat.norm_intent(*ps)
    return flat.norm_cover(*ps) if store else None


def _done(*params):
    for p in params:
        if p is not None and p.requires_grad:
            grad_hooks.notify(p)


class _BiasSums:

    def __init__(self):
        self.items, self.params, self.stream = [], [], None
        self.task = None

    def add(self, x, ld, out, T, N, *params):
        if _DEFER_BIAS_SUMS and x.is_cuda and K.colsum_vec_ok(x, ld, out, N) and self._armed():
            self.items.append((x, ld, out, T, N))
            self.params.extend(params)
            return
        K.colsum_accum(x, ld, out, T, N)
        _done(*params)

    def _armed(self) -> bool:
        task = torch._C._current_graph_task_id()
        if task < 0:
            return False
        if task == self.task:
            return True
# ... 334 lines not shown
        return _ln_forward(ctx, x, w, b, eps)[0]

    @staticmethod
    def backward(ctx, dy):
        return _ln_backward(ctx, dy), None, None, None


class LayerNormTwinFn(Function):

    @staticmethod
    def forward(ctx, x, w, b, eps):
        return _ln_forward(ctx, x, w, b, eps, twin=True)

    @staticmethod
    def backward(ctx, dy, dy32):
        return _ln_backward(ctx, dy, dy2=dy32), None, None, None


def _f32_of(t: torch.Tensor) -> torch.Tensor:
    twin = getattr(t, "_iit_f32", None)
    if twin is not None and twin[0] == t.data_ptr() and twin[1] == t._version and twin[2].shape == t.shape:
        return twin[2]
    return t


def _set_bf16_twin(t: torch.Tensor, t16: torch.Tensor) -> None:
    t._iit_bf16 = (t.data_ptr(), t._version, t16)


def _bf16_of(t: torch.Tensor) -> torch.Tensor:
    if t.dtype == BF16:
        return t
    twin = getattr(t, "_iit_bf16", None)
    if twin is not None and twin[0] == t.data_ptr() and twin[1] == t._version and twin[2].numel() == t.numel():
        return twin[2].view(t.shape)
    return t.to(BF16)


class LayerNormForkFn(Function):

    @staticmethod
    def forward(ctx, x, w, b, eps):
        y, _ = _ln_forward(ctx, x, w, b, eps, xhat16=_xhat16(w, b, x.shape[-1]))
        return y, x.view_as(x)

    @staticmethod
    def backward(ctx, dy, dpass):
        return _ln_backward(ctx, dy, dres=dpass), None, None, None


def _packed3(a: Optional[torch.Tensor], b: Optional[torch.Tensor], c: Optional[torch.Tensor], n: int) -> bool:
    if a is None or b is None or c is None:
        return False
    st = a.untyped_storage().data_ptr()
    if b.untyped_storage().data_ptr() != st or c.untyped_storage().data_ptr() != st:
        return False
    es = a.element_size()
    return b.data_ptr() == a.data_ptr() + n * es and c.data_ptr() == a.data_ptr() + 2 * n * es


def _rows_bf16(x, x_full):
    rows = x if x_full is None else x_full
    x2 = _flat2(rows.to(BF16).contiguous())
    return x2, x2.shape[0] * x.shape[0] // rows.shape[0]


def _base_rows(t2, T: int):
    return t2 if t2.shape[0] == T else t2[:T]


def _wgrad_slots(layout_ok: bool, *Ws):
    store = layout_ok and _claim_store(*Ws)
    return store, [W.grad if store else _grad_slot(W) for W in Ws]


def _wgrad_rows(gW, Kd: int, N: int):
    if gW is None:
        return None, 0
    gW2 = gW.reshape(Kd, N) if gW.is_contiguous() else gW
    assert gW2.stride(-1) == 1 and gW2.dim() == 2, "weight gradient must have unit column stride"
    return gW2, gW2.stride(0)


def _wgrad_tail(ctx, xspec, x2, g2, ldg, Ws, C, ldc, store, gb):
    bs = None
    if C is not None:
        T, N = g2.shape
        bs = _fused_bias(gb, N)
        wspec = dict(A=x2, B=g2, C=C, M=x2.shape[1], N=N, K=T, lda=x2.shape[1], ldb=ldg, ldc=ldc,
                     mode=K.MODE_AKM | K.MODE_BKM, epi=K.EPI_F32_STORE if store else K.EPI_F32_ACC, fresh=store,
                     bsum=bs, gsq=_norm_slots(store, *Ws))
        choice = gemm_pair(xspec, wspec, prefetch=_pf_next(ctx)) if xspec is not None else gemm(**wspec)
        if store:
            _settle_claim(choice, *Ws)
    elif xspec is not None:
        gemm(**xspec)
    return bs


def _bias_tail(bs, gb, g2, ldg, bias, Ws) -> None:
    if gb is not None and bs is None:
        _BIAS_SUMS.add(g2, ldg, gb, g2.shape[0], gb.numel(), *bias)
    else:
        _done(*bias)
    _done(*Ws)


def _qkv_forward(ctx, x, layer, bias_bf16, W_Q, W_K, W_V, b_Q, b_K, b_V, x_full=None):
    ctx.set_materialize_grads(False)
    B, S, d = x.shape
    H, dh = W_Q.shape[0], W_Q.shape[2]
    HD = H * dh
    x2, T = _rows_bf16(x, x_full)
    T2 = x2.shape[0]
    out = torch.empty(T2 // S, S, 3, H, dh, dtype=BF16, device=x.device)
    gemm(x2, layer["qkv"], out, M=T2, N=3 * HD, K=d, lda=d, ldb=3 * HD, ldc=3 * HD, mode=K.MODE_BKM,
         epi=K.EPI_BF16_BIAS3, bias0=b_Q, bias1=b_K, bias2=b_V, bias_cols=HD, blas_bias=bias_bf16)
    xb = _base_rows(x2, T)
    ctx.save_for_backward(xb)
    ctx.layer = layer
    ctx.params = (W_Q, W_K, W_V, b_Q, b_K, b_V)
    ctx.dims = (B, S, d, H, dh)
    _pf_register(ctx, xb, layer["qkv"])
    return out


class QKVFn(Function):

    @staticmethod
    def forward(ctx, x, layer, bias_bf16, W_Q, W_K, W_V, b_Q, b_K, b_V):
        return _qkv_forward(ctx, x, layer, bias_bf16, W_Q, W_K, W_V, b_Q, b_K, b_V)

    @staticmethod
    def backward(ctx, dqkv):
        if dqkv is None:
            return (None,) * 9
        (x2,) = ctx.saved_tensors
        W_Q, W_K, W_V, b_Q, b_K, b_V = ctx.params
        B, S, d, H, dh = ctx.dims
        HD = H * dh
        T = B * S
        g = dqkv.to(BF16).contiguous().view(T, 3 * HD)
        dx = torch.empty(T, d, dtype=BF16, device=g.device)
        xspec = dict(A=g, B=ctx.layer["qkv"], C=dx, M=T, N=d, K=3 * HD, lda=3 * HD, ldb=3 * HD, ldc=d, epi=K.EPI_BF16)
        Ws = (W_Q, W_K, W_V)
        store, (gq, gk, gv) = _wgrad_slots(W_Q.stride() == (dh, 3 * HD, 1) and _packed3(W_Q, W_K, W_V, HD), *Ws)
        gbs = [_grad_slot(bp) for bp in (b_Q, b_K, b_V)]
        have_b = all(s is not None for s in gbs)
        gb = None
        if have_b and all(s.is_contiguous() for s in gbs) and _packed3(*gbs, HD):
            gb = torch.as_strided(gbs[0], (3 * HD,), (1,))
        have_w = gq is not None and gk is not None and gv is not None
        packed_w = have_w and gq.stride() == (dh, 3 * HD, 1) and _packed3(gq, gk, gv, HD)
        bs = _wgrad_tail(ctx, xspec, x2, g, 3 * HD, Ws, gq if packed_w else None, 3 * HD, store, gb)
        if have_w and not packed_w:
            gemm(x2, g, gq, C2=gk, C3=gv, M=d, N=3 * HD, K=T, lda=d, ldb=3 * HD, ldc=0,
                 mode=K.MODE_AKM | K.MODE_BKM, epi=K.EPI_F32_ACC_QKV, qkv=(dh, H, d))
        if have_b and gb is None:
            K.colsum3_accum(g, 3 * HD, gbs, T, HD)
        _bias_tail(bs, gb, g, 3 * HD, (b_Q, b_K, b_V) if have_b else (), Ws)
        return (dx.view(B, S, d),) + (None,) * 8


class AttnFn(Function):

    @staticmethod
    def forward(ctx, qkv, zsrc, mask, causal, scale):
        ctx.set_materialize_grads(False)
        B, S, _, H, dh = qkv.shape
        qkv = qkv.contiguous()
        z = torch.empty(B, S, H, dh, dtype=BF16, device=qkv.device)
        lse = torch.empty(B * H * S, dtype=F32, device=qkv.device)
        src = None
        if mask:
            src = zsrc.to(BF16).contiguous()
        K.attn_small_fwd(qkv, z, lse, src, mask, B, S, H, dh, 3 * H * dh, H * dh, H * dh, scale, causal)
        ctx.save_for_backward(qkv, lse)
        ctx.cfg = (mask, causal, scale)
        return z

    @staticmethod
    def backward(ctx, dz):
        if dz is None:
            return None, None, None, None, None
        qkv, lse = ctx.saved_tensors
        mask, causal, scale = ctx.cfg
        B, S, _, H, dh = qkv.shape
        dz = dz.to(BF16).contiguous()
        dqkv = torch.empty_like(qkv)
        K.attn_small_bwd(qkv, dz, lse, dqkv, mask, B, S, H, dh, 3 * H * dh, H * dh, scale, causal)
        return dqkv, None, None, None, None


def _flash_grads(ctx, dz, q, k, v, dq, dk, dv):
    z, lse = ctx.saved_tensors[-2:]
    mask, causal, scale = ctx.cfg
    B, S, Hq, _ = q.shape
    dz = dz.to(BF16)
    if dz.stride(-1) != 1 or dz.stride(1) % 8 or dz.stride(2) % 8:
        dz = dz.contiguous()
    dd = torch.empty(B, Hq, S, dtype=F32, device=q.device)
    K.flash_bwd(q, k, v, z, dz, lse, dd, dq, dk, dv, mask, scale, causal, spec=getattr(ctx, "spec", None))


class FlashPackedFn(Function):

    @staticmethod
    def forward(ctx, qkv, zsrc, mask, causal, scale):
        ctx.set_materialize_grads(False)
        B, S, _, H, dh = qkv.shape
        q, k, v = qkv[:, :, 0], qkv[:, :, 1], qkv[:, :, 2]
        z = torch.empty(B, S, H, dh, dtype=BF16, device=qkv.device)
        lse = torch.empty(B, H, S, dtype=F32, device=qkv.device)
        src = zsrc.to(BF16).contiguous() if mask else None
        K.flash_fwd(q, k, v, z, lse, src, mask, scale, causal)
        ctx.save_for_backward(qkv, z, lse)
        ctx.cfg = (mask, causal, scale)
        return z

    @staticmethod
    def backward(ctx, dz):
        if dz is None:
            return None, None, None, None, None
        qkv = ctx.saved_tensors[0]
        dqkv = torch.empty_like(qkv)
        _flash_grads(ctx, dz, qkv[:, :, 0], qkv[:, :, 1], qkv[:, :, 2], dqkv[:, :, 0], dqkv[:, :, 1], dqkv[:, :, 2])
        return dqkv, None, None, None, None


class FlashFn(Function):

    @staticmethod
    def forward(ctx, q, k, v, causal, scale, src=None, spec=None):
        ctx.set_materialize_grads(False)
        B, S, Hq, dh = q.shape
        z = torch.empty(B, S, Hq, dh, dtype=BF16, device=q.device)
        lse = torch.empty(B, Hq, S, dtype=F32, device=q.device)
        K.flash_fwd(q, k, v, z, lse, src, 0, scale, causal, spec=spec)
        ctx.save_for_backward(q, k, v, z, lse)
        ctx.cfg = (0, causal, scale)
        ctx.spec = spec
        ctx.keep = src
        return z

    @staticmethod
    def backward(ctx, dz):
        if dz is None:
            return None, None, None, None, None, None, None
        q, k, v = ctx.saved_tensors[:3]
        dq, dk, dv = torch.empty_like(q), torch.empty_like(k), torch.empty_like(v)
        _flash_grads(ctx, dz, q, k, v, dq, dk, dv)
        return dq, dk, dv, None, None, None, None


def _flash_view(t: torch.Tensor) -> torch.Tensor:
    t = t.to(BF16)
    if t.stride(-1) != 1 or t.stride(1) % 8 or t.stride(2) % 8 or t.stride(0) % 8 or t.data_ptr() % 16:
        t = t.contiguous()
    return t


def flash_supported(q: torch.Tensor) -> bool:
    return q.is_cuda and q.shape[-1] in (64, 128) and os.environ.get("IIT_FLASH", "1") != "0"


def flash_attention(q, k, v, causal: bool, attn_scale: float) -> torch.Tensor:
    return FlashFn.apply(_flash_view(q), _flash_view(k), _flash_view(v), causal, 1.0 / attn_scale)


def flash_attention_spliced(q, k, v, causal: bool, attn_scale: float, index, src) -> Optional[torch.Tensor]:
    if os.environ.get("IIT_FLASH_SPLICE", "1") == "0":
        return None
    from .splice import patch_spec
# ... 142 lines not shown
    return SwiGLUSpliceFn.apply(pre, pre_linear, src, spec)


class EmbedSpliceFn(Function):

    @staticmethod
    def forward(ctx, tokens, W_E, flat, src, spec):
        tok = tokens.reshape(-1).to(torch.int64).contiguous()
        W16 = flat.shadow_view(W_E)
        out = torch.empty(*tokens.shape, W_E.shape[-1], dtype=BF16, device=W_E.device)
        K.embed_splice_fwd(tok, W16, out, src, spec.ptr)
        ctx.save_for_backward(tok)
        ctx.p, ctx.flat, ctx.spec = W_E, flat, spec
        return out

    @staticmethod
    def backward(ctx, g):
        (tok,) = ctx.saved_tensors
        from ..engine import grad_hooks
        W_E = ctx.p
        slot = W_E.grad
        if slot is None:
            slot = ctx.flat.bind_zero(W_E)
        g = g.reshape(-1, g.shape[-1])
        if g.dtype not in (BF16, torch.float32):
            g = g.float()
        K.embed_splice_bwd(tok, g.contiguous(), slot, ctx.spec.ptr)
        grad_hooks.notify(W_E)
        return None, None, None, None, None


def embed_spliced(tokens, W_E, flat, index, src) -> Optional[torch.Tensor]:
    from .splice import patch_spec
    d = W_E.shape[-1]
    if os.environ.get("IIT_EMBED_SPLICE", "1") == "0" or d % 8 or W_E.stride(-1) != 1 or W_E.stride(0) % 8:
        return None
    if src.dtype != BF16 or src.device != W_E.device:
        src = src.to(device=W_E.device, dtype=BF16)
    shape = tuple(tokens.shape) + (d,)
    spec = patch_spec(index, shape, src)
    if spec is None or spec.dims[3][0] % 8:
        return None
    return EmbedSpliceFn.apply(tokens, W_E, flat, src, spec)


def llama_fused_ok(x: torch.Tensor) -> bool:
    return x.is_cuda and x.dtype == BF16 and os.environ.get("IIT_LLAMA_FUSED", "1") != "0"


def _resid_rows(resid, resid_full):
    return _flat2((resid if resid_full is None else resid_full).float().contiguous())


def _linear_forward(ctx, x, W, b, w, ldw, resid, out_kind, x_full=None, resid_full=None):
    ctx.set_materialize_grads(False)
    lead = (x if x_full is None else x_full).shape[:-1]
    Kd = x.shape[-1]
    N = W.shape[-1]
    x2, T = _rows_bf16(x, x_full)
    T2 = x2.shape[0]
    dev = x.device
    if out_kind == "bf16":
        out = torch.empty(T2, N, dtype=BF16, device=dev)
        gemm(x2, w, out, M=T2, N=N, K=Kd, lda=Kd, ldb=ldw, ldc=N, mode=K.MODE_BKM, epi=K.EPI_BF16, bias0=b)
        res = out.view(*lead, N)
    elif out_kind == "f32":
        Np = _pad8(N)
        out = torch.empty(T2, Np, dtype=F32, device=dev)
        gemm(x2, w, out, M=T2, N=N, K=Kd, lda=Kd, ldb=ldw, ldc=Np, mode=K.MODE_BKM, epi=K.EPI_F32_STORE, bias0=b)
        res = out[:, :N]
        res = res.unflatten(0, lead) if len(lead) != 1 else res
    else:
        out = torch.empty(T2, N, dtype=F32, device=dev)
        gemm(x2, w, out, M=T2, N=N, K=Kd, lda=Kd, ldb=ldw, ldc=N, mode=K.MODE_BKM, epi=K.EPI_F32_RESID, bias0=b,
             resid=_resid_rows(resid, resid_full), ldr=N)
        res = out.view(*lead, N)
    xb = _base_rows(x2, T)
    ctx.save_for_backward(xb)
    ctx.params = (W, b)
    ctx.w = w
    _pf_register(ctx, xb, w)
    ctx.ldw = ldw
    ctx.meta = (x.shape[:-1], Kd, N, out_kind, x.dtype)
    return res


class LinearFn(Function):

    @staticmethod
    def forward(ctx, x, W, b, w, ldw, resid, out_kind):
        return _linear_forward(ctx, x, W, b, w, ldw, resid, out_kind)

    @staticmethod
    def backward(ctx, gy):
        if gy is None:
            return (None,) * 7
        (x2,) = ctx.saved_tensors
        W, b = ctx.params
        lead, Kd, N, out_kind, x_dtype = ctx.meta
        T = x2.shape[0]
        gres = gy if out_kind == "resid" else None
        g16 = _bf16_of(gy)
        g2 = _aligned_rows(g16, T, N)
        ldg = g2.stride(0)
        dx = xspec = dxb = None
        if ctx.needs_input_grad[0]:
            amode = K.MODE_NN
            _, splits = K._tiling(T, Kd, N, True)
            if splits == 1:
                dxb = torch.empty(T, Kd, dtype=BF16, device=g2.device)
                xspec = dict(A=g2, B=ctx.w, C=dxb, M=T, N=Kd, K=N, lda=ldg, ldb=ctx.ldw, ldc=Kd, mode=amode,
                             epi=K.EPI_BF16)
            else:
                dxf = torch.zeros(T, Kd, dtype=F32, device=g2.device)
                gemm(g2, ctx.w, dxf, M=T, N=Kd, K=N, lda=ldg, ldb=ctx.ldw, ldc=Kd, mode=amode, epi=K.EPI_F32_ACC,
                     splits=splits)
                dx = dxf.to(x_dtype).view(*lead, Kd)
        store, (gW,) = _wgrad_slots(True, W)
        gb = _grad_slot(b)
        bs = _wgrad_tail(ctx, xspec, x2, g2, ldg, (W,), *_wgrad_rows(gW, Kd, N), store, gb)
        if dxb is not None:
            dx = (dxb if x_dtype == BF16 else dxb.to(x_dtype)).view(*lead, Kd)
        _bias_tail(bs, gb, g2, ldg, (b,), (W,))
        return dx, None, None, None, None, gres, None


class UnembedFn(LinearFn):

    @staticmethod
    def forward(ctx, x, W, b, w, ldw):
        res = LinearFn.forward(ctx, x, W, b, w, ldw, None, "f32")
        handle = torch.empty(1, dtype=BF16, device=res.device).expand(res.shape)
        return res, handle

    @staticmethod
    def backward(ctx, gy, gh=None):
        if gh is not None:
            gy = gh if gy is None else gy.float() + gh.float()
        return LinearFn.backward(ctx, gy)[:5]


def _mlp_in_forward(ctx, x, W_in, b_in, w, erf, x_full=None, spec=None):
    ctx.set_materialize_grads(False)
    ctx.erf = erf
    ctx.zero_spec = spec
    lead = (x if x_full is None else x_full).shape[:-1]
    d = x.shape[-1]
    dm = W_in.shape[1]
    x2, T = _rows_bf16(x, x_full)
    T2 = x2.shape[0]
    post = torch.empty(T2, dm, dtype=BF16, device=x.device)
    pre = torch.empty(T2, dm, dtype=BF16, device=x.device)
    gemm(x2, w, post, C2=pre, M=T2, N=dm, K=d, lda=d, ldb=dm, ldc=dm, ldc2=dm, mode=K.MODE_BKM,
         epi=K.EPI_GELU_ERF if erf else K.EPI_GELU, bias0=b_in)
    if spec is not None:
        K.sparse_pair(post, T, dm, spec.ptr, 0)
    xb = _base_rows(x2, T)
    ctx.save_for_backward(xb, _base_rows(pre, T))
    ctx.params = (W_in, b_in)
    ctx.w = w
    _pf_register(ctx, xb, w)
    ctx.meta = (x.shape[:-1], d, dm)
    return pre.view(*lead, dm), post.view(*lead, dm)


class MLPInFn(Function):

    @staticmethod
    def forward(ctx, x, W_in, b_in, w, erf=False):
        return _mlp_in_forward(ctx, x, W_in, b_in, w, erf)

    @staticmethod
    def backward(ctx, gpre, gpost):
        if gpre is None and gpost is None:
            return None, None, None, None, None
        x2, pre = ctx.saved_tensors
        W_in, b_in = ctx.params
        lead, d, dm = ctx.meta
        T = x2.shape[0]
        if gpost is not None:
            dpre = torch.empty(T, dm, dtype=BF16, device=x2.device)
            K.dgelu(gpost.to(BF16).contiguous().view(T, dm), pre, dpre, erf=ctx.erf)
            zs = getattr(ctx, "zero_spec", None)
            if zs is not None:
                K.sparse_pair(dpre, T, dm, zs.ptr, 1)
            if gpre is not None:
                dpre = (dpre.float() + gpre.float().reshape(T, dm)).to(BF16)
        else:
            dpre = gpre.to(BF16).contiguous().view(T, dm)
        dx = torch.empty(T, d, dtype=BF16, device=x2.device)
        xspec = dict(A=dpre, B=ctx.w, C=dx, M=T, N=d, K=dm, lda=dm, ldb=dm, ldc=d, epi=K.EPI_BF16)
        store, (gW,) = _wgrad_slots(W_in.is_contiguous(), W_in)
        summed = _bias_sum_done(gpre if gpost is None else None, b_in)
        gb = None if summed else _grad_slot(b_in)
        bs = _wgrad_tail(ctx, xspec, x2, dpre, dm, (W_in,), gW, dm, store, gb)
        _bias_tail(bs, gb, dpre, dm, (b_in,), (W_in,))
        return dx.view(*lead, d), None, None, None, None


def _bias_sum_done(g: Optional[torch.Tensor], b: Optional[torch.Tensor]) -> bool:
    tag = getattr(g, "_iit_bias_sum", None) if g is not None else None
    return tag is not None and b is not None and tag == (g.data_ptr(), g._version, id(b))


# ... 137 lines not shown
    def forward(ctx, tokens, W_E, W_pos, tokens_full, box):
        ctx.set_materialize_grads(False)
        B2, S = tokens_full.shape
        d = W_E.shape[1]
        B = tokens.shape[0]
        out = torch.empty(B2, S, d, dtype=F32, device=tokens.device)
        K.embed_pos_fwd(tokens_full, W_E, W_pos, out, B2, S, d)
        ctx.save_for_backward(tokens_full[:B])
        ctx.params = (W_E, W_pos)
        box.append(out)
        return out[:B]

    @staticmethod
    def backward(ctx, g):
        return EmbedPosFn.backward(ctx, g) + (None, None)


class LayerNormForkPairFn(LayerNormForkFn):
    @staticmethod
    def forward(ctx, x, w, b, eps, x_full, box):
        yf, _ = _ln_forward(ctx, x, w, b, eps, x_full, xhat16=_xhat16(w, b, x.shape[-1]))
        box.append(yf)
        return yf[:x.shape[0]], x.view_as(x)

    @staticmethod
    def backward(ctx, dy, dpass):
        return LayerNormForkFn.backward(ctx, dy, dpass) + (None, None)


class LayerNormPairTwinFn(Function):

    @staticmethod
    def forward(ctx, x, w, b, eps, x_full, box):
        yf, yf32 = _ln_forward(ctx, x, w, b, eps, x_full, twin=True)
        box.append((yf, yf32))
        return yf[:x.shape[0]], yf32[:x.shape[0]]

    @staticmethod
    def backward(ctx, dy, dy32):
        return LayerNormTwinFn.backward(ctx, dy, dy32) + (None, None)


class LayerNormPairFn(LayerNormFn):

    @staticmethod
    def forward(ctx, x, w, b, eps, x_full, box, pos_mask=0):
        yf, _ = _ln_forward(ctx, x, w, b, eps, x_full, pos_mask=pos_mask)
        box.append(yf)
        return yf[:x.shape[0]]

    @staticmethod
    def backward(ctx, dy):
        return (_ln_backward(ctx, dy, sel=ctx.sel),) + (None,) * 6


class QKVPairFn(QKVFn):
    @staticmethod
    def forward(ctx, x, layer, bias_bf16, W_Q, W_K, W_V, b_Q, b_K, b_V, x_full, box):
        out = _qkv_forward(ctx, x, layer, bias_bf16, W_Q, W_K, W_V, b_Q, b_K, b_V, x_full)
        box.append(out)
        return out[:x.shape[0]]

    @staticmethod
    def backward(ctx, dqkv):
        return QKVFn.backward(ctx, dqkv) + (None, None)


class AttnPairFn(AttnFn):

    @staticmethod
    def forward(ctx, qkv, causal, scale, mask, qkv_full, box):
        ctx.set_materialize_grads(False)
        B = qkv.shape[0]
        B2, S, _, H, dh = qkv_full.shape
        z = torch.empty(B2, S, H, dh, dtype=BF16, device=qkv.device)
        lse = torch.empty(B2 * H * S, dtype=F32, device=qkv.device)
        if mask:
            K.attn_pair_fwd(qkv_full, z, lse, B2, S, H, dh, 3 * H * dh, H * dh, scale, causal, pair_seqs=B,
                            pair_mask=mask)
        else:
            K.attn_small_fwd(qkv_full, z, lse, None, 0, B2, S, H, dh, 3 * H * dh, H * dh, H * dh, scale, causal)
        ctx.save_for_backward(qkv_full[:B], lse[:B * H * S])
        ctx.cfg = (mask, causal, scale)
        box.append(z)
        return z[:B]

    @staticmethod
    def backward(ctx, dz):
        g = AttnFn.backward(ctx, dz)
        return (g[0], None, None, None, None, None)


class AttnPairSpecFn(Function):

    @staticmethod
    def forward(ctx, qkv, causal, scale, spec, qkv_full, box):
        ctx.set_materialize_grads(False)
        B = qkv.shape[0]
        B2, S, _, H, dh = qkv_full.shape
        z = torch.empty(B2, S, H, dh, dtype=BF16, device=qkv.device)
        lse = torch.empty(B2 * H * S, dtype=F32, device=qkv.device)
        K.attn_pair_fwd_spec(qkv_full, z, lse, B2, S, H, dh, 3 * H * dh, H * dh, scale, causal, B, spec.ptr)
        ctx.save_for_backward(qkv_full[:B], lse[:B * H * S])
        ctx.cfg = (spec, causal, scale)
        box.append(z)
        return z[:B]

    @staticmethod
    def backward(ctx, dz):
        if dz is None:
            return None, None, None, None, None, None
        qkv, lse = ctx.saved_tensors
        spec, causal, scale = ctx.cfg
        B, S, _, H, dh = qkv.shape
        qkv = qkv.contiguous()
        dz = dz.to(BF16).contiguous()
        dqkv = torch.empty_like(qkv)
        K.attn_bwd_spec(qkv, dz, lse, dqkv, B, S, H, dh, 3 * H * dh, H * dh, scale, causal, spec.ptr)
        return dqkv, None, None, None, None, None


class LinearPairFn(LinearFn):

    @staticmethod
    def forward(ctx, x, W, b, w, ldw, resid, out_kind, x_full, resid_full, box):
        of = _linear_forward(ctx, x, W, b, w, ldw, resid, out_kind, x_full, resid_full)
        box.append(of)
        return of[:x.shape[0]]

    @staticmethod
    def backward(ctx, gy):
        return LinearFn.backward(ctx, gy) + (None, None, None)


class MLPInPairFn(MLPInFn):

    @staticmethod
    def forward(ctx, x, W_in, b_in, w, erf, x_full, spec, box):
        pf, qf = _mlp_in_forward(ctx, x, W_in, b_in, w, erf, x_full, spec)
        box.append((pf, qf))
        return pf[:x.shape[0]], qf[:x.shape[0]]

    @staticmethod
    def backward(ctx, gpre, gpost):
        return MLPInFn.backward(ctx, gpre, gpost) + (None, None, None)


class MLPOutGeluPairFn(MLPOutGeluFn):
    @staticmethod
    def forward(ctx, pre, post, W, b, w, ldw, resid, b_in, erf, post_full, resid_full, box):
        of = _mlp_out_forward(ctx, pre, post, W, b, w, ldw, resid, b_in, erf, post_full, resid_full)
        box.append(of)
        return of[:post.shape[0]]

    @staticmethod
    def backward(ctx, gy):
        return MLPOutGeluFn.backward(ctx, gy) + (None, None, None)


class PairSpliceFn(Function):

    @staticmethod
    def forward(ctx, act, act_full, spec_pair, spec_base, box):
        out = torch.empty_like(act_full)
        B = act.shape[0]
        K.splice(act_full, act_full[B:], out, act_full.numel(), spec_pair.ptr, act_full.dtype == F32, 0)
# ... 31 lines not shown
        self._layer_of = {}
        self._mirror_key = {}
        for i, blk in enumerate(model.blocks):
            mats = [(blk.attn.W_Q, "qkv"), (blk.attn.W_O, "o")]
            if not model.cfg.attn_only:
                mats += [(blk.mlp.W_in, "in"), (blk.mlp.W_out, "out")]
            for W, key in mats:
                self._layer_of[id(W)] = i
                self._mirror_key[id(W)] = key

    def begin_forward(self):
        self.shadow.ensure()
        _PF_SEQ.clear()
        _PF_ON[0] = self.prefetch
        pol = os.environ.get("IIT_FWD_PREFETCH", "auto")
        self.fwd_pf = pol == "1" or (pol == "auto" and type(self.model).__name__ == "HookedTransformer")

    def _L(self, p):
        return self.shadow.layers[self._layer_of[id(p)]]

    def embed(self, tokens, W_E):
        return W_E[tokens]

    def pos_embed(self, batch, seq, W_pos, offset: int = 0):
        return W_pos[offset:offset + seq].unsqueeze(0).expand(batch, seq, W_pos.shape[-1])

    def embed_pos(self, tokens, W_E, W_pos):
        return EmbedPosFn.apply(tokens, W_E, W_pos)

    def residual(self, a, b):
        return a.float() + b.float()

    def w(self, p: torch.Tensor) -> torch.Tensor:
        return p.to(BF16)

    def fwd_prefetch(self, *Ws):
        if not self.fwd_pf:
            return None
        return tuple(self._L(W)[self._mirror_key[id(W)]] for W in Ws)

    def layer_norm(self, x, w, b, eps, prefetch=None):
        return _ln_apply(LayerNormFn, prefetch, x, w, b, eps)

    def layer_norm_twin(self, x, w, b, eps, prefetch=None):
        if os.environ.get("IIT_LN_TWIN", "1") == "0":
            return _ln_apply(LayerNormFn, prefetch, x, w, b, eps)
        y, y32 = _ln_apply(LayerNormTwinFn, prefetch, x, w, b, eps)
        y._iit_f32 = (y.data_ptr(), y._version, y32)
        return y

    def layer_norm_fork(self, x, w, b, eps, prefetch=None):
        return _ln_apply(LayerNormForkFn, prefetch, x, w, b, eps)

    def qkv(self, x, W_Q, W_K, W_V, b_Q, b_K, b_V):
        i = self._layer_of[id(W_Q)]
        packed = QKVFn.apply(x, self.shadow.layers[i], self.shadow.biases[i], W_Q, W_K, W_V, b_Q, b_K, b_V)
        q, k, v = packed[:, :, 0], packed[:, :, 1], packed[:, :, 2]
        q._iit_packed = k._iit_packed = v._iit_packed = packed
        return q, k, v

    def attention(self, q, k, v, causal, attn_scale, patch_heads: Optional[Sequence[int]] = None, patch_src=None,
                  hook_scores=None, hook_pattern=None, ignore=float("-inf")):
        S, dh = q.shape[1], q.shape[-1]
        if S > 16 and flash_supported(q):
            packed = getattr(q, "_iit_packed", None)
            if packed is not None and getattr(k, "_iit_packed", None) is packed and \
                    getattr(v, "_iit_packed", None) is packed and packed.is_contiguous():
                return FlashPackedFn.apply(packed, patch_src, K.heads_to_mask(patch_heads), causal, 1.0 / attn_scale)
            z = flash_attention(q, k, v, causal, attn_scale)
            if patch_heads:
                z = z.clone()
                z[:, :, list(patch_heads)] = patch_src[:, :, list(patch_heads)].to(z.dtype)
            return z
        if not K.attn_small_ok(S, dh):
            z = TorchOps.attention(self, q, k, v, causal, attn_scale)
            if patch_heads:
                z = z.clone()
                z[:, :, list(patch_heads)] = patch_src[:, :, list(patch_heads)].to(z.dtype)
            return z
        packed = getattr(q, "_iit_packed", None)
        if packed is None or getattr(k, "_iit_packed", None) is not packed or getattr(v, "_iit_packed", None) is not packed:
            packed = torch.stack([q, k, v], dim=2).to(BF16)
        mask = K.heads_to_mask(patch_heads)
        return AttnFn.apply(packed, patch_src, mask, causal, 1.0 / attn_scale)

    def o_proj(self, z, W_O, b_O):
        B, S, H, dh = z.shape
        return LinearFn.apply(z.reshape(B, S, H * dh), W_O, b_O, self._L(W_O)["o"], W_O.shape[-1], None, "bf16")

    def o_proj_residual(self, z, W_O, b_O, resid):
        resid = _f32_of(resid)
        B, S, H, dh = z.shape
        return LinearFn.apply(z.reshape(B, S, H * dh), W_O, b_O, self._L(W_O)["o"], W_O.shape[-1], resid, "resid")

    def o_result(self, z, W_O):
        return torch.einsum("bshe,hed->bshd", z.to(BF16), W_O.to(BF16))

    def mlp_in(self, x, W_in, b_in, act: str, hook_pre=None):
        w = self._L(W_in)["in"]
        if hook_pre is None and act in ("gelu_new", "gelu_fast", "gelu_pytorch_tanh", "gelu"):
            return MLPInFn.apply(x, W_in, b_in, w, act == "gelu")
        pre = LinearFn.apply(x, W_in, b_in, w, W_in.shape[1], None, "bf16")
        if hook_pre is not None:
            pre = hook_pre(pre)
        return pre, act_fn(act)(pre)

    def mlp_gelu_residual(self, x, W_in, b_in, W_out, b_out, resid, erf: bool = False):
        resid = _f32_of(resid)
        if not torch.is_grad_enabled():
            lead, d, dm, N = x.shape[:-1], x.shape[-1], W_in.shape[1], W_out.shape[1]
            x2 = _flat2(x.to(BF16).contiguous())
            T = x2.shape[0]
            post = torch.empty(T, dm, dtype=BF16, device=x.device)
            gemm(x2, self._L(W_in)["in"], post, C2=None, M=T, N=dm, K=d, lda=d, ldb=dm, ldc=dm, ldc2=dm,
                 mode=K.MODE_BKM, epi=K.EPI_GELU_ERF if erf else K.EPI_GELU, bias0=b_in)
            r2 = _flat2(resid.float().contiguous())
            out = torch.empty(T, N, dtype=F32, device=x.device)
            gemm(post, self._L(W_out)["out"], out, M=T, N=N, K=dm, lda=dm, ldb=W_out.shape[1], ldc=N,
                 mode=K.MODE_BKM, epi=K.EPI_F32_RESID, bias0=b_out, resid=r2, ldr=N)
            return out.view(*lead, N)
        pre, post = MLPInFn.apply(x, W_in, b_in, self._L(W_in)["in"], erf)
        return MLPOutGeluFn.apply(pre, post.detach(), W_out, b_out, self._L(W_out)["out"], W_out.shape[1], resid,
                                  b_in, erf)

    def mlp_out(self, post, W_out, b_out):
        return LinearFn.apply(post, W_out, b_out, self._L(W_out)["out"], W_out.shape[1], None, "bf16")

    def mlp_out_residual(self, post, W_out, b_out, resid):
        resid = _f32_of(resid)
        return LinearFn.apply(post, W_out, b_out, self._L(W_out)["out"], W_out.shape[1], resid, "resid")

    def unembed(self, x, W_U, b_U):
        sh = self.shadow
        if sh.U is None:
            raise RuntimeError("unembed before begin_forward(): the bf16 shadow of W_U is not bound")
        logits, handle = UnembedFn.apply(x, W_U, b_U, sh.U, sh.Vp)
        logits._iit_grad16 = (logits.data_ptr(), logits._version, handle)
        return logits

    def unembed_argmax(self, x, W_U, b_U, chunk: int = 8192):
        sh = self.shadow
        lead = x.shape[:-1]
        d = x.shape[-1]
        x2 = _flat2(x.to(BF16).contiguous())
        T = x2.shape[0]
        V = W_U.shape[1]
        buf = torch.empty(T, chunk, dtype=F32, device=x.device)
        best_v = best_i = None
        for s in range(0, V, chunk):
            n = min(chunk, V - s)
            gemm(x2, sh.U[:, s:], buf, M=T, N=n, K=d, lda=d, ldb=sh.Vp, ldc=chunk, mode=K.MODE_BKM,
                 epi=K.EPI_F32_STORE, bias0=b_U[s:s + n])
            v, i = buf[:, :n].max(dim=-1)
            i = i + s
            if best_v is None:
                best_v, best_i = v, i
            else:
                upd = v > best_v
                best_v = torch.where(upd, v, best_v)
                best_i = torch.where(upd, i, best_i)
        return best_i.view(*lead)


    supports_pairs = True

    def pair_embed_pos(self, tokens, src_tokens, W_E, W_pos) -> Paired:
        full_tok = torch.cat([tokens, src_tokens]).contiguous()
        out, full = _one(EmbedPosPairFn, tokens, W_E, W_pos, full_tok)
        return Paired(out, full)

    def pair_layer_norm_fork(self, p: Paired, w, b, eps, prefetch=None):
        box = []
        y, x_pass = _ln_apply(LayerNormForkPairFn, prefetch, p.base, w, b, eps, p.full.float().contiguous(), box)
        return Paired(y, box[0]), Paired(x_pass, p.full)

    def pair_layer_norm(self, p: Paired, w, b, eps, pos_mask: int = 0, twin: bool = False, prefetch=None) -> Paired:
        box = []
        if twin and not pos_mask and w is not None and os.environ.get("IIT_LN_TWIN", "1") != "0":
            y, y32 = _ln_apply(LayerNormPairTwinFn, prefetch, p.base, w, b, eps, p.full.float().contiguous(), box)
            yf, yf32 = box[0]
            y._iit_f32 = (y.data_ptr(), y._version, y32)
            return Paired(y, yf, (y32, yf32))
        y = _ln_apply(LayerNormPairFn, prefetch, p.base, w, b, eps, p.full.float().contiguous(), box, int(pos_mask))
        return Paired(y, box[0])

    @staticmethod
    def position_mask(index, shape) -> int:
        if len(shape) != 3 or shape[1] > 64:
            return 0
        ranges = index.to_ranges(tuple(shape))
        if ranges is None or ranges[0] != [(0, shape[0])] or ranges[2] != [(0, shape[2])]:
            return 0
        m = 0
        for lo, hi in ranges[1]:
            for s_ in range(lo, hi):
                m |= 1 << s_
        return m

    def pair_qkv(self, p: Paired, W_Q, W_K, W_V, b_Q, b_K, b_V) -> Paired:
        i = self._layer_of[id(W_Q)]
        out, full = _one(QKVPairFn, p.base, self.shadow.layers[i], self.shadow.biases[i], W_Q, W_K, W_V, b_Q, b_K,
                         b_V, p.full)
        return Paired(out, full)

    def pair_attention(self, p: Paired, causal: bool, attn_scale: float, heads: Optional[Sequence[int]] = None
                       ) -> Paired:
        out, full = _one(AttnPairFn, p.base, causal, 1.0 / attn_scale, K.heads_to_mask(heads) if heads else 0,
                         p.full)
        return Paired(out, full)

    def pair_attention_spliced(self, p: Paired, causal: bool, attn_scale: float, index) -> Optional[Paired]:
        from .splice import patch_spec
        if os.environ.get("IIT_ATTN_SPLICE", "1") == "0":
            return None
        B2, S, _, H, dh = p.full.shape
        B = p.base.shape[0]
        spec = patch_spec(index, (B, S, H, dh))
        if spec is None or [d[0] for d in spec.dims] != [B, S, H, dh]:
            return None
        out, full = _one(AttnPairSpecFn, p.base, causal, 1.0 / attn_scale, spec, p.full)
        return Paired(out, full)

    def attention_dual(self, q, causal: bool, attn_scale: float) -> torch.Tensor:
        packed = q._iit_packed
        B, S, _, H, dh = packed.shape
        zf = torch.empty(2 * B, S, H, dh, dtype=BF16, device=packed.device)
        K.attn_pair_fwd(packed, zf[B:], None, B, S, H, dh, 3 * H * dh, H * dh, 1.0 / attn_scale, causal, z2=zf[:B])
        return zf

    def pair_heads_ok(self, S: int, dh: int) -> bool:
        return K.attn_pair_ok(S, dh)

    def pair_o_proj_residual(self, z: Paired, W_O, b_O, resid: Paired) -> Paired:
        B2, S, H, dh = z.full.shape
        B = z.base.shape[0]
        rb, rf = resid.resid_operands()
        out, full = _one(LinearPairFn, z.base.reshape(B, S, H * dh), W_O, b_O, self._L(W_O)["o"], W_O.shape[-1],
                         rb, "resid", z.full.reshape(B2, S, H * dh), rf)
        return Paired(out, full)

    def pair_mlp_in(self, x: Paired, W_in, b_in, erf: bool = False, index=None):
        spec = None
        if index is not None:
            from .splice import patch_spec
            B, S = x.base.shape[0], x.base.shape[1]
            spec = patch_spec(index, (B, S, W_in.shape[1])) if os.environ.get("IIT_MLP_SPLICE", "1") != "0" else None
            if spec is None:
                return None
        (pre, post), (pf, qf) = _one(MLPInPairFn, x.base, W_in, b_in, self._L(W_in)["in"], erf, x.full, spec)
        return Paired(pre, pf), Paired(post, qf)

    def pair_mlp_out_residual(self, post: Paired, W_out, b_out, resid: Paired) -> Paired:
        rb, rf = resid.resid_operands()
        out, full = _one(LinearPairFn, post.base, W_out, b_out, self._L(W_out)["out"], W_out.shape[1], rb,
                         "resid", post.full, rf)
        return Paired(out, full)

    def pair_mlp_gelu_residual(self, x: Paired, W_in, b_in, W_out, b_out, resid: Paired, erf: bool = False):
        pre, post = self.pair_mlp_in(x, W_in, b_in, erf)
        rb, rf = resid.resid_operands()
        out, full = _one(MLPOutGeluPairFn, pre.base, post.base.detach(), W_out, b_out, self._L(W_out)["out"],
                         W_out.shape[1], rb, b_in, erf, post.full, rf)
        return Paired(out, full)

    def pair_splice(self, p: Paired, index) -> Optional[Paired]:
        if not p.full.is_contiguous():
            return None
        specs = pair_specs(index, tuple(p.base.shape))
        if specs is None:
            return None
        out, full = _one(PairSpliceFn, p.base, p.full, specs[0], specs[1])
        return Paired(out, full)


def pair_specs(index, shape):
    from . import splice as _sp
    key = ("pair",) + tuple(shape)
    cache = getattr(index, "_iit_specs", None)
    if cache is not None and key in cache:
        return cache[key]
    ranges = index.to_ranges(tuple(shape))
    base_spec = _sp.patch_spec(index, tuple(shape))
    out = None
    if ranges is not None and base_spec is not None:
        B = shape[0]
        rest = list(shape[1:])
        row = 1
        for n in rest:
            row *= n
        cstr = []
        acc = 1
        for n in reversed(rest):
            cstr.insert(0, acc)
            acc *= n
        if ranges[0] == [(0, B)]:
            dims = _sp._collapse((2 * B,) + tuple(rest), [[(0, B)]] + ranges[1:], [row] + cstr)
        else:
            dims = _sp._collapse((2, B) + tuple(rest), [[(0, 1)]] + ranges, [0, row] + cstr)
        if dims is not None:
            out = (_sp.PatchSpec(dims), base_spec)
    if cache is None:
        cache = index._iit_specs = {}
    cache[key] = out
    return out


def get_hip_ops(model) -> HipOps:
    K.lib()
    ops = getattr(model, "_iit_hip_ops", None)
    if ops is None:
        ops = HipOps(model)
        model._iit_hip_ops = ops
    return ops
```

Before: 17400 pairs/s.

## Fuse small-attention backward into the O-projection dual-GEMM dX epilogue

Adds a fused kernel in which the O-projection backward's dX tiles feed an attention-backward epilogue directly. It computes dQKV per head from the GEMM accumulator held in LDS, so dz never makes a round trip to HBM and the separate attention-backward launch goes away. The attention autograd node is linked to the following linear layer and receives a zero stand-in gradient, then returns the precomputed dqkv. The shared backward body is factored into a header. This adds complex cross-op autograd plumbing and constrains shapes (dh=64, S<=16, 128-aligned sizes), and the epilogue serialises several sequences per wave.

Result: no change. 17380 pairs/s (-0.1%).

```diff
diff --git a/csrc/attn_mfma.hip b/csrc/attn_mfma.hip
--- a/csrc/attn_mfma.hip
+++ b/csrc/attn_mfma.hip
@@ -1,31 +1,8 @@
+#include "attn_small_body.h"
 #include "common.h"
 #include "splice_spec.h"
 
-typedef __attribute__((address_space(3))) i16x4 lds_i16x4_t;
-
-__device__ __forceinline__ bf16x8 half_frag(const i16x4 v) {
-  const i16x4 z = {0, 0, 0, 0};
-  return __builtin_bit_cast(bf16x8, (i16x8)__builtin_shufflevector(v, z, 0, 1, 2, 3, 4, 5, 6, 7));
-}
-
-__device__ __forceinline__ bf16x8 regs_frag(float a, float b, float c, float d) {
-  bf16x8 o = {f2bf(a), f2bf(b), f2bf(c), f2bf(d), f2bf(0.f), f2bf(0.f), f2bf(0.f), f2bf(0.f)};
-  return o;
-}
-
-__device__ __forceinline__ bf16x8 load8(const __bf16* p, bool ok) {
-  if (!ok) {
-    const i16x8 z = {0, 0, 0, 0, 0, 0, 0, 0};
-    return __builtin_bit_cast(bf16x8, z);
-  }
-  return *(const bf16x8*)p;
-}
-
-template <int LDSR>
-__device__ __forceinline__ i16x4 tr_block(const __bf16* img, int g, int lane_in_group, int col0) {
-  const int q = lane_in_group >> 2, p = lane_in_group & 3;
-  return __builtin_amdgcn_ds_read_tr16_b64_v4i16((lds_i16x4_t*)(img + (4 * g + q) * LDSR + col0 + 4 * p));
-}
+using namespace attn_small;
 
 
 template <int DH, bool SP>
@@ -164,20 +141,16 @@
   __shared__ float Dsh[4][16];
   const int wave = threadIdx.x >> 6, l = threadIdx.x & 63, g = l >> 4, c = l & 15;
   const int bh = blockIdx.x * 4 + wave;
-  const bool valid = bh < BH;
-  const int b = valid ? bh / H : 0, h = valid ? bh % H : 0;
+  if (bh >= BH) return;
+  const int b = bh / H, h = bh % H;
   const int HD = H * DH;
   const long row0 = (long)b * S;
-  const bool patched = valid && ((head_mask >> h) & 1ull);
-  const bool work = valid && !patched;
-  __bf16* Qs = smem[wave][0];
-  __bf16* Ks = smem[wave][1];
-  __bf16* Gs = smem[wave][2];
+  const bool patched = (head_mask >> h) & 1ull;
   bf16x8 qf[DH / 32], kf[DH / 32], vf[DH / 32], gf[DH / 32];
 #pragma unroll
   for (int s = 0; s < DH / 32; ++s) {
     const long off = (row0 + c) * ld_qkv + h * DH + 32 * s + 8 * g;
-    const bool ok = work && c < S;
+    const bool ok = !patched && c < S;
     qf[s] = load8(qkv + off, ok);
     kf[s] = load8(qkv + off + HD, ok);
     vf[s] = load8(qkv + off + 2 * HD, ok);
@@ -187,97 +160,13 @@
       for (int e = 0; e < 8; ++e)
         if (in_ranges(sp, 3, 32 * s + 8 * g + e)) gf[s][e] = f2bf(0.f);
     }
-    if (work) {
-      *(bf16x8*)(Qs + c * LDSR + 32 * s + 8 * g) = qf[s];
-      *(bf16x8*)(Ks + c * LDSR + 32 * s + 8 * g) = kf[s];
-      *(bf16x8*)(Gs + c * LDSR + 32 * s + 8 * g) = gf[s];
-    }
-  }
-  f32x4 Sa = {0.f, 0.f, 0.f, 0.f}, STa = Sa, dPa = Sa, dPTa = Sa;
-#pragma unroll
-  for (int s = 0; s < DH / 32; ++s) {
-    Sa = __builtin_amdgcn_mfma_f32_16x16x32_bf16(qf[s], kf[s], Sa, 0, 0, 0);
-    STa = __builtin_amdgcn_mfma_f32_16x16x32_bf16(kf[s], qf[s], STa, 0, 0, 0);
-    dPa = __builtin_amdgcn_mfma_f32_16x16x32_bf16(gf[s], vf[s], dPa, 0, 0, 0);
-    dPTa = __builtin_amdgcn_mfma_f32_16x16x32_bf16(vf[s], gf[s], dPTa, 0, 0, 0);
-  }
-  float P[4], PT[4], Dr[4];
-  const float lse_c = (work && c < S) ? lse[(long)bh * S + c] : 0.f;
-#pragma unroll
-  for (int r = 0; r < 4; ++r) {
-    const int qi = 4 * g + r, kj = c;
-    const bool ok = work && qi < S && kj < S && (!causal || kj <= qi);
-    P[r] = ok ? __expf(Sa[r] * scale - lse[(long)bh * S + qi]) : 0.f;
-    const int kj2 = 4 * g + r, qi2 = c;
-    const bool ok2 = work && qi2 < S && kj2 < S && (!causal || kj2 <= qi2);
-    PT[r] = ok2 ? __expf(STa[r] * scale - lse_c) : 0.f;
-    float d = P[r] * dPa[r];
-    d += __shfl_xor(d, 1, 64);
-    d += __shfl_xor(d, 2, 64);
-    d += __shfl_xor(d, 4, 64);
-    d += __shfl_xor(d, 8, 64);
-    Dr[r] = d;
-  }
-  if (c == 0) {
-#pragma unroll
-    for (int r = 0; r < 4; ++r) Dsh[wave][4 * g + r] = Dr[r];
-  }
-  __syncthreads();
-  if (!valid) return;
-  __bf16* dq = dqkv + h * DH;
-  __bf16* dk = dqkv + HD + h * DH;
-  __bf16* dv = dqkv + 2 * HD + h * DH;
-  if (patched) {
-    for (int i = l; i < S * DH / 8; i += 64) {
-      const int r = i / (DH / 8), ch = i % (DH / 8);
-      const uint4 zz = make_uint4(0, 0, 0, 0);
-      *(uint4*)(dq + (row0 + r) * ld_qkv + ch * 8) = zz;
-      *(uint4*)(dk + (row0 + r) * ld_qkv + ch * 8) = zz;
-      *(uint4*)(dv + (row0 + r) * ld_qkv + ch * 8) = zz;
-    }
-    return;
-  }
-  const float Dc = Dsh[wave][c];
-  float dS[4], dST[4];
-#pragma unroll
-  for (int r = 0; r < 4; ++r) {
-    dS[r] = P[r] * (dPa[r] - Dr[r]) * scale;
-    dST[r] = PT[r] * (dPTa[r] - Dc) * scale;
-  }
-  const bf16x8 bP = regs_frag(P[0], P[1], P[2], P[3]);
-  const bf16x8 bdS = regs_frag(dS[0], dS[1], dS[2], dS[3]);
-  const bf16x8 bdST = regs_frag(dST[0], dST[1], dST[2], dST[3]);
-  const f32x4 zero = {0.f, 0.f, 0.f, 0.f};
-  f32x4 dvT[DH / 16], dkT[DH / 16], dqT[DH / 16];
-#pragma unroll
-  for (int t = 0; t < DH / 16; ++t) {
-    const bf16x8 aG = half_frag(tr_block<LDSR>(Gs, g, c, 16 * t));
-    const bf16x8 aQ = half_frag(tr_block<LDSR>(Qs, g, c, 16 * t));
-    const bf16x8 aK = half_frag(tr_block<LDSR>(Ks, g, c, 16 * t));
-    dvT[t] = __builtin_amdgcn_mfma_f32_16x16x32_bf16(aG, bP, zero, 0, 0, 0);
-    dkT[t] = __builtin_amdgcn_mfma_f32_16x16x32_bf16(aQ, bdS, zero, 0, 0, 0);
-    dqT[t] = __builtin_amdgcn_mfma_f32_16x16x32_bf16(aK, bdST, zero, 0, 0, 0);
-  }
-  asm volatile("s_waitcnt lgkmcnt(0)" ::: "memory");
-#pragma unroll
-  for (int t = 0; t < DH / 16; ++t) {
-    const int o = c * LDSR + 16 * t + 4 * g;
-    *(bf16x4*)(Gs + o) = bf16x4{f2bf(dvT[t][0]), f2bf(dvT[t][1]), f2bf(dvT[t][2]), f2bf(dvT[t][3])};
-    *(bf16x4*)(Ks + o) = bf16x4{f2bf(dkT[t][0]), f2bf(dkT[t][1]), f2bf(dkT[t][2]), f2bf(dkT[t][3])};
-    *(bf16x4*)(Qs + o) = bf16x4{f2bf(dqT[t][0]), f2bf(dqT[t][1]), f2bf(dqT[t][2]), f2bf(dqT[t][3])};
-  }
-  asm volatile("s_waitcnt lgkmcnt(0)" ::: "memory");
-  constexpr int CPR = DH / 8;
-#pragma unroll
-  for (int i = l; i < 16 * CPR; i += 64) {
-    const int r = i / CPR, ch = i % CPR;
-    if (r < S) {
-      const long o = (row0 + r) * ld_qkv + ch * 8;
-      *(bf16x8*)(dv + o) = *(const bf16x8*)(Gs + r * LDSR + ch * 8);
-      *(bf16x8*)(dk + o) = *(const bf16x8*)(Ks + r * LDSR + ch * 8);
-      *(bf16x8*)(dq + o) = *(const bf16x8*)(Qs + r * LDSR + ch * 8);
-    }
-  }
+  }
+  __bf16* Qs = smem[wave][0];
+  __bf16* Ks = smem[wave][1];
+  __bf16* Gs = smem[wave][2];
+  bwd_body<DH>(Qs, Ks, Gs, Dsh[wave], qf, kf, vf, gf, lse + (long)bh * S, S, scale, causal, patched);
+  __bf16* dq = dqkv + row0 * ld_qkv + h * DH;
+  store_rows<DH>(Qs, Ks, Gs, dq, dq + HD, dq + 2 * HD, ld_qkv, S);
 }
 
 IIT_EXPORT int iit_attn_mfma_fwd_pair(const void* qkv, void* z, float* lse, const void* zsrc,
diff --git a/csrc/attn_small_body.h b/csrc/attn_small_body.h
--- /dev/null
+++ b/csrc/attn_small_body.h
@@ -0,0 +1,207 @@
+#pragma once
+#include "common.h"
+
+namespace attn_small {
+
+typedef __attribute__((address_space(3))) i16x4 lds_i16x4_t;
+
+__device__ __forceinline__ bf16x8 half_frag(const i16x4 v) {
+  const i16x4 z = {0, 0, 0, 0};
+  return __builtin_bit_cast(bf16x8, (i16x8)__builtin_shufflevector(v, z, 0, 1, 2, 3, 4, 5, 6, 7));
+}
+
+__device__ __forceinline__ bf16x8 regs_frag(float a, float b, float c, float d) {
+  bf16x8 o = {f2bf(a), f2bf(b), f2bf(c), f2bf(d), f2bf(0.f), f2bf(0.f), f2bf(0.f), f2bf(0.f)};
+  return o;
+}
+
+__device__ __forceinline__ bf16x8 zero8() {
+  const i16x8 z = {0, 0, 0, 0, 0, 0, 0, 0};
+  return __builtin_bit_cast(bf16x8, z);
+}
+
+__device__ __forceinline__ bf16x8 load8(const __bf16* p, bool ok) {
+  if (!ok) return zero8();
+  return *(const bf16x8*)p;
+}
+
+template <int LDSR>
+__device__ __forceinline__ i16x4 tr_block(const __bf16* img, int g, int lane_in_group, int col0) {
+  const int q = lane_in_group >> 2, p = lane_in_group & 3;
+  return __builtin_amdgcn_ds_read_tr16_b64_v4i16((lds_i16x4_t*)(img + (4 * g + q) * LDSR + col0 + 4 * p));
+}
+
+template <int DH>
+__device__ __forceinline__ void bwd_body(__bf16* Qs, __bf16* Ks, __bf16* Gs, float* Dsh, const bf16x8 (&qf)[DH / 32],
+                                         const bf16x8 (&kf)[DH / 32], const bf16x8 (&vf)[DH / 32],
+                                         const bf16x8 (&gf)[DH / 32], const float* __restrict__ lse, int S, float scale,
+                                         int causal, bool masked) {
+  constexpr int LDSR = DH + 8;
+  const int l = threadIdx.x & 63, g = l >> 4, c = l & 15;
+  if (masked) {
+#pragma unroll
+    for (int s = 0; s < DH / 32; ++s) {
+      const int o = c * LDSR + 32 * s + 8 * g;
+      *(bf16x8*)(Qs + o) = zero8();
+      *(bf16x8*)(Ks + o) = zero8();
+      *(bf16x8*)(Gs + o) = zero8();
+    }
+    asm volatile("s_waitcnt lgkmcnt(0)" ::: "memory");
+    return;
+  }
+#pragma unroll
+  for (int s = 0; s < DH / 32; ++s) {
+    const int o = c * LDSR + 32 * s + 8 * g;
+    *(bf16x8*)(Qs + o) = qf[s];
+    *(bf16x8*)(Ks + o) = kf[s];
+    *(bf16x8*)(Gs + o) = gf[s];
+  }
+  f32x4 Sa = {0.f, 0.f, 0.f, 0.f}, STa = Sa, dPa = Sa, dPTa = Sa;
+#pragma unroll
+  for (int s = 0; s < DH / 32; ++s) {
+    Sa = __builtin_amdgcn_mfma_f32_16x16x32_bf16(qf[s], kf[s], Sa, 0, 0, 0);
+    STa = __builtin_amdgcn_mfma_f32_16x16x32_bf16(kf[s], qf[s], STa, 0, 0, 0);
+    dPa = __builtin_amdgcn_mfma_f32_16x16x32_bf16(gf[s], vf[s], dPa, 0, 0, 0);
+    dPTa = __builtin_amdgcn_mfma_f32_16x16x32_bf16(vf[s], gf[s], dPTa, 0, 0, 0);
+  }
+  float P[4], PT[4], Dr[4];
+  const float lse_c = c < S ? lse[c] : 0.f;
+#pragma unroll
+  for (int r = 0; r < 4; ++r) {
+    const int qi = 4 * g + r, kj = c;
+    const bool ok = qi < S && kj < S && (!causal || kj <= qi);
+    P[r] = ok ? __expf(Sa[r] * scale - lse[qi]) : 0.f;
+    const int kj2 = 4 * g + r, qi2 = c;
+    const bool ok2 = qi2 < S && kj2 < S && (!causal || kj2 <= qi2);
+    PT[r] = ok2 ? __expf(STa[r] * scale - lse_c) : 0.f;
+    float d = P[r] * dPa[r];
+    d += __shfl_xor(d, 1, 64);
+    d += __shfl_xor(d, 2, 64);
+    d += __shfl_xor(d, 4, 64);
+    d += __shfl_xor(d, 8, 64);
+    Dr[r] = d;
+  }
+  if (c == 0) {
+#pragma unroll
+    for (int r = 0; r < 4; ++r) Dsh[4 * g + r] = Dr[r];
+  }
+  asm volatile("s_waitcnt lgkmcnt(0)" ::: "memory");
+  const float Dc = Dsh[c];
+  float dS[4], dST[4];
+#pragma unroll
+  for (int r = 0; r < 4; ++r) {
+    dS[r] = P[r] * (dPa[r] - Dr[r]) * scale;
+    dST[r] = PT[r] * (dPTa[r] - Dc) * scale;
+  }
+  const bf16x8 bP = regs_frag(P[0], P[1], P[2], P[3]);
+  const bf16x8 bdS = regs_frag(dS[0], dS[1], dS[2], dS[3]);
+  const bf16x8 bdST = regs_frag(dST[0], dST[1], dST[2], dST[3]);
+  const f32x4 zero = {0.f, 0.f, 0.f, 0.f};
+  f32x4 dvT[DH / 16], dkT[DH / 16], dqT[DH / 16];
+#pragma unroll
+  for (int t = 0; t < DH / 16; ++t) {
+    const bf16x8 aG = half_frag(tr_block<LDSR>(Gs, g, c, 16 * t));
+    const bf16x8 aQ = half_frag(tr_block<LDSR>(Qs, g, c, 16 * t));
+    const bf16x8 aK = half_frag(tr_block<LDSR>(Ks, g, c, 16 * t));
+    dvT[t] = __builtin_amdgcn_mfma_f32_16x16x32_bf16(aG, bP, zero, 0, 0, 0);
+    dkT[t] = __builtin_amdgcn_mfma_f32_16x16x32_bf16(aQ, bdS, zero, 0, 0, 0);
+    dqT[t] = __builtin_amdgcn_mfma_f32_16x16x32_bf16(aK, bdST, zero, 0, 0, 0);
+  }
+  asm volatile("s_waitcnt lgkmcnt(0)" ::: "memory");
+#pragma unroll
+  for (int t = 0; t < DH / 16; ++t) {
+    const int o = c * LDSR + 16 * t + 4 * g;
+    *(bf16x4*)(Gs + o) = bf16x4{f2bf(dvT[t][0]), f2bf(dvT[t][1]), f2bf(dvT[t][2]), f2bf(dvT[t][3])};
+    *(bf16x4*)(Ks + o) = bf16x4{f2bf(dkT[t][0]), f2bf(dkT[t][1]), f2bf(dkT[t][2]), f2bf(dkT[t][3])};
+    *(bf16x4*)(Qs + o) = bf16x4{f2bf(dqT[t][0]), f2bf(dqT[t][1]), f2bf(dqT[t][2]), f2bf(dqT[t][3])};
+  }
+  asm volatile("s_waitcnt lgkmcnt(0)" ::: "memory");
+}
+
+template <int DH>
+__device__ __forceinline__ void store_rows(const __bf16* Qs, const __bf16* Ks, const __bf16* Gs, __bf16* dq, __bf16* dk,
+                                           __bf16* dv, long ld, int S) {
+  constexpr int LDSR = DH + 8, CPR = DH / 8;
+  const int l = threadIdx.x & 63;
+#pragma unroll
+  for (int i = l; i < 16 * CPR; i += 64) {
+    const int r = i / CPR, ch = i % CPR;
+    if (r < S) {
+      const long o = r * ld + ch * 8;
+      *(bf16x8*)(dv + o) = *(const bf16x8*)(Gs + r * LDSR + ch * 8);
+      *(bf16x8*)(dk + o) = *(const bf16x8*)(Ks + r * LDSR + ch * 8);
+      *(bf16x8*)(dq + o) = *(const bf16x8*)(Qs + r * LDSR + ch * 8);
+    }
+  }
+}
+
+struct AttnEpi {
+  const __bf16* qkv;
+  const float* lse;
+  __bf16* dqkv;
+  unsigned long long head_mask;
+  long ld_qkv;
+  int S, H;
+  float scale;
+  int causal;
+};
+
+constexpr int kEpiWaveBytes = (64 + 3 * 16) * 72 * 2 + 64;
+constexpr int kEpiBytes = 4 * kEpiWaveBytes;
+
+struct EpiFrags {
+  bf16x8 q[2], k[2], v[2];
+};
+
+__device__ __forceinline__ void epi_load(EpiFrags& f, const AttnEpi& a, long row0, int h, bool ok) {
+  const int l = threadIdx.x & 63, g = l >> 4, c = l & 15;
+  const int HD = a.H * 64;
+#pragma unroll
+  for (int s = 0; s < 2; ++s) {
+    const long off = (row0 + c) * a.ld_qkv + h * 64 + 32 * s + 8 * g;
+    f.q[s] = load8(a.qkv + off, ok);
+    f.k[s] = load8(a.qkv + off + HD, ok);
+    f.v[s] = load8(a.qkv + off + 2 * HD, ok);
+  }
+}
+
+__device__ __forceinline__ void bwd_epilogue(const AttnEpi& a, char* smem, const f32x4 (&acc)[4][4], int m0, int n0) {
+  constexpr int LDSR = 72, IMG = 16 * LDSR;
+  const int wave = threadIdx.x >> 6, l = threadIdx.x & 63, g = l >> 4, c = l & 15;
+  const int wm = wave >> 1, wn = wave & 1;
+  const int S = a.S, h = n0 / 64 + wn, np = 64 / S;
+  const bool masked = (a.head_mask >> h) & 1ull;
+  const long wrow0 = m0 + wm * 64;
+  EpiFrags cur;
+  epi_load(cur, a, wrow0, h, !masked && c < S);
+  __bf16* Z = (__bf16*)(smem + wave * kEpiWaveBytes);
+  __bf16* Qs = Z + 64 * LDSR;
+  __bf16* Ks = Qs + IMG;
+  __bf16* Gs = Ks + IMG;
+  float* Dsh = (float*)(Gs + IMG);
+  __syncthreads();
+#pragma unroll
+  for (int i = 0; i < 4; ++i)
+#pragma unroll
+    for (int j = 0; j < 4; ++j)
+      *(bf16x4*)(Z + (i * 16 + c) * LDSR + j * 16 + 4 * g) =
+          bf16x4{f2bf(acc[i][j][0]), f2bf(acc[i][j][1]), f2bf(acc[i][j][2]), f2bf(acc[i][j][3])};
+  const int HD = a.H * 64;
+  for (int p = 0; p < np; ++p) {
+    asm volatile("s_waitcnt lgkmcnt(0)" ::: "memory");
+    const long row0 = wrow0 + p * S;
+    EpiFrags nxt;
+    if (p + 1 < np) epi_load(nxt, a, row0 + S, h, !masked && c < S);
+    bf16x8 gf[2];
+#pragma unroll
+    for (int s = 0; s < 2; ++s)
+      gf[s] = (!masked && c < S) ? *(const bf16x8*)(Z + (p * S + c) * LDSR + 32 * s + 8 * g) : zero8();
+    bwd_body<64>(Qs, Ks, Gs, Dsh, cur.q, cur.k, cur.v, gf, a.lse + ((row0 / S) * a.H + h) * S, S, a.scale, a.causal,
+                 masked);
+    __bf16* dq = a.dqkv + row0 * a.ld_qkv + h * 64;
+    store_rows<64>(Qs, Ks, Gs, dq, dq + HD, dq + 2 * HD, a.ld_qkv, S);
+    if (p + 1 < np) cur = nxt;
+  }
+}
+
+}
diff --git a/csrc/gemm_dual.hip b/csrc/gemm_dual.hip
--- a/csrc/gemm_dual.hip
+++ b/csrc/gemm_dual.hip
@@ -36,6 +36,53 @@
   hipLaunchKernelGGL((gemm_dual_kernel<TW, EW, TX, EX>), dim3(pf.wgs + wt * w_splits + xt), dim3(TW::NW * 64), 0, s,
                      w, x, wt, w_splits, xt, pf);
   return hipGetLastError();
+}
+
+template <class TW, int EW, class TX>
+__global__ __launch_bounds__(TW::NW * 64, TW::OCC) void gemm_dual_attn_kernel(G2Args pw, G2Args px, int w_tiles,
+                                                                              int w_splits, int x_tiles, Prefetch pf,
+                                                                              attn_small::AttnEpi at) {
+  static_assert(TW::NW == TX::NW && TW::OCC == TX::OCC, "one launch geometry");
+  __shared__ __attribute__((aligned(16))) char smem[TW::SMEM > TX::SMEM ? TW::SMEM : TX::SMEM];
+  if ((int)blockIdx.x < pf.wgs) {
+    prefetch_part(pf, blockIdx.x);
+    return;
+  }
+  const int b = blockIdx.x - pf.wgs;
+  const int nw = w_tiles * w_splits;
+  if (b < nw) {
+    gemm_glds_body<TW::BM, TW::BN, TW::NS, true, true, EW, TW::NW, 64, TW::OCC>(pw, b % w_tiles, w_tiles,
+                                                                                b / w_tiles, w_splits, smem);
+  } else {
+    gemm_glds_body<TX::BM, TX::BN, TX::NS, false, false, E_ATTN_BWD, TX::NW, 64, TX::OCC>(px, b - nw, x_tiles, 0, 1,
+                                                                                          smem, &at);
+  }
+}
+
+#define X(IDX, BM, BN, NS, NW, OCC, GLDS) \
+  using AttnTX = Cfg<BM, BN, NS, NW, OCC>; \
+  constexpr int kAttnXTile = IDX;
+IIT_DUAL_ATTN_X_TILE_LIST(X)
+#undef X
+
+template <int EW>
+hipError_t pick_w_attn(const G2Args& w, const G2Args& x, int w_splits, int wtile, const Prefetch& pf,
+                       const attn_small::AttnEpi& at, hipStream_t s) {
+  switch (wtile) {
+#define X(IDX, BM_, BN_, NS_, NW_, OCC_, GLDS)                                                                    \
+  case IDX:                                                                                                       \
+    if constexpr (NW_ == AttnTX::NW && OCC_ == AttnTX::OCC) {                                                     \
+      using TW = Cfg<BM_, BN_, NS_, NW_, OCC_>;                                                                   \
+      const int wt = (w.M / TW::BM) * (w.N / TW::BN), xt = (x.M / AttnTX::BM) * (x.N / AttnTX::BN);               \
+      hipLaunchKernelGGL((gemm_dual_attn_kernel<TW, EW, AttnTX>), dim3(pf.wgs + wt * w_splits + xt),              \
+                         dim3(TW::NW * 64), 0, s, w, x, wt, w_splits, xt, pf, at);                                \
+      return hipGetLastError();                                                                                   \
+    }                                                                                                             \
+    break;
+    IIT_DUAL_W_TILE_LIST(X)
+#undef X
+  }
+  return hipErrorInvalidValue;
 }
 
 template <class TW, int EW, int EX>
@@ -128,3 +175,52 @@
   if (wepi == E_F32_ACC && xepi == E_DGELU) return (int)pick_w<E_F32_ACC, E_DGELU>(w, x, wsplits, wtile, xtile, pf, s);
   return (int)hipErrorInvalidValue;
 }
+
+IIT_EXPORT int iit_gemm_dual_attn_ok(const void* wA, const void* wB, const void* wC, long wlda, long wldb, long wldc,
+                                     int wM, int wN, int wK, int wepi, int wtile, int wsplits, int reduce,
+                                     const void* xA, const void* xB, long xlda, long xldb, int xM, int xN, int xK,
+                                     const void* qkv, const void* lse, const void* dqkv, long ld_qkv, int S, int H,
+                                     int dh, int pair_seqs, const void* spec) {
+  if (pair_seqs != 0 || spec != nullptr) return 0;
+  if (dh != 64 || S < 1 || S > 16 || 128 % S != 0 || H < 1 || H > 64) return 0;
+  if (xM <= 0 || xM % 128 != 0 || xN != H * dh || xN % 128 != 0) return 0;
+  if (!qkv || !lse || !dqkv || ld_qkv < 3L * H * dh || ld_qkv % 8 != 0) return 0;
+  if ((uintptr_t)qkv % 16 != 0 || (uintptr_t)dqkv % 16 != 0 || (uintptr_t)lse % 4 != 0) return 0;
+  return iit_gemm_dual_ok(wA, wB, wC, wlda, wldb, wldc, wM, wN, wK, wepi, wtile, wsplits, reduce, xA, xB, dqkv, nullptr,
+                          xlda, xldb, ld_qkv, 0, xM, xN, xK, E_BF16, kAttnXTile);
+}
+
+IIT_EXPORT int iit_gemm_dual_attn(const void* wA, const void* wB, void* wC, long wlda, long wldb, long wldc, int wM,
+                                  int wN, int wK, int wepi, int wtile, int wsplits, float* ws, int* counters,
+                                  const void* xA, const void* xB, long xlda, long xldb, int xM, int xN, int xK,
+                                  float* bsum, float* gsq, const void* qkv, const float* lse, void* dqkv, long ld_qkv,
+                                  unsigned long long head_mask, int S, int H, int dh, float scale, int causal,
+                                  int pair_seqs, const void* spec, const void* pf0, long pf0_bytes, const void* pf1,
+                                  long pf1_bytes, int pf_wgs, void* stream) {
+  const int reduce = ws != nullptr;
+  if (!iit_gemm_dual_attn_ok(wA, wB, wC, wlda, wldb, wldc, wM, wN, wK, wepi, wtile, wsplits, reduce, xA, xB, xlda, xldb,
+                             xM, xN, xK, qkv, lse, dqkv, ld_qkv, S, H, dh, pair_seqs, spec))
+    return (int)hipErrorInvalidValue;
+  if (reduce && !counters) return (int)hipErrorInvalidValue;
+  G2Args w{};
+  w.A = (const __bf16*)wA; w.B = (const __bf16*)wB; w.C = wC;
+  w.lda = wlda; w.ldb = wldb; w.ldc = wldc;
+  w.M = wM; w.N = wN; w.K = wK; w.k_per_split = wK / wsplits;
+  w.ws = reduce ? ws : nullptr;
+  w.counters = reduce ? counters : nullptr;
+  w.bsum = bsum;
+  w.gsq = wepi == E_F32_STORE ? gsq : nullptr;
+  G2Args x{};
+  x.A = (const __bf16*)xA; x.B = (const __bf16*)xB;
+  x.lda = xlda; x.ldb = xldb;
+  x.M = xM; x.N = xN; x.K = xK; x.k_per_split = xK;
+  w.group_m = x.group_m = g_dual_group_m;
+  const attn_small::AttnEpi at{(const __bf16*)qkv, lse, (__bf16*)dqkv, head_mask, ld_qkv, S, H, scale, causal};
+  Prefetch pf{{(const char*)pf0, (const char*)pf1}, {pf0 ? pf0_bytes : 0, pf1 ? pf1_bytes : 0}, 0};
+  if ((pf.bytes[0] > 0 || pf.bytes[1] > 0) && pf_wgs > 0) pf.wgs = ((pf_wgs + 7) / 8) * 8;
+  if (pf.wgs > 1024) pf.wgs = 1024;
+  hipStream_t s = (hipStream_t)stream;
+  if (wepi == E_F32_STORE) return (int)pick_w_attn<E_F32_STORE>(w, x, wsplits, wtile, pf, at, s);
+  if (wepi == E_F32_ACC) return (int)pick_w_attn<E_F32_ACC>(w, x, wsplits, wtile, pf, at, s);
+  return (int)hipErrorInvalidValue;
+}
diff --git a/csrc/gemm_glds.hip b/csrc/gemm_glds.hip
--- a/csrc/gemm_glds.hip
+++ b/csrc/gemm_glds.hip
@@ -133,6 +133,7 @@
   FAMILY(3, kDualXRows)
   FAMILY(4, kConvRows)
   FAMILY(5, kConvWgRows)
+  FAMILY(6, kDualAttnXRows)
 #undef FAMILY
   for (int i = 0; i < n && i < cap; ++i) out[i] = rows[i];
   return n;
diff --git a/csrc/gemm_glds_body.h b/csrc/gemm_glds_body.h
--- a/csrc/gemm_glds_body.h
+++ b/csrc/gemm_glds_body.h
@@ -1,12 +1,13 @@
 #pragma once
 #include <type_traits>
 
+#include "attn_small_body.h"
 #include "common.h"
 
 namespace {
 
 enum : int { E_BF16 = 0, E_BF16_BIAS3 = 1, E_F32_RESID = 2, E_GELU = 3, E_DGELU = 4, E_F32_ACC = 5,
-             E_F32_STORE = 7, E_GELU_ERF = 8, E_DGELU_ERF = 9, E_BF16_CS = 10 };
+             E_F32_STORE = 7, E_GELU_ERF = 8, E_DGELU_ERF = 9, E_BF16_CS = 10, E_ATTN_BWD = 11 };
 
 struct G2Args {
   const __bf16* A;
@@ -472,7 +473,8 @@
 template <int BM, int BN, int NS, bool AKM, bool BKM, int EPI, int NW, int BK = 64, int OCC = 1, bool LEAN = false,
           class ASTG = void, class BSTG = void, bool EDGE = false>
 __device__ __forceinline__ void gemm_glds_body(const G2Args& p, const int lin, const int nlin, const int split,
-                                               const int nsplit, char* smem) {
+                                               const int nsplit, char* smem,
+                                               const attn_small::AttnEpi* attn = nullptr) {
   using SA = std::conditional_t<std::is_void_v<ASTG>, OperandStager<AKM, BM, NW, BK, LEAN>, ASTG>;
   using SB = std::conditional_t<std::is_void_v<BSTG>, OperandStager<BKM, BN, NW, BK, LEAN>, BSTG>;
   constexpr int HALVES = BK / 64;
@@ -708,6 +710,11 @@
       return;
     }
   }
+  if constexpr (EPI == E_ATTN_BWD) {
+    static_assert(BM == 128 && BN == 128 && NW == 4 && !EDGE, "2 x 2 waves of 64 rows x one 64-wide head");
+    static_assert(attn_small::kEpiBytes <= SM::BYTES, "the epilogue's images fit the launch's LDS object");
+    attn_small::bwd_epilogue(*attn, smem, acc, m0, n0);
+  } else {
   glds_epilogue<BM, BN, EPI, NT, ECH, SM::EPS, EDGE>(p, smem, m0, n0, lin, [&](float* E, int ch) {
     if (wm / (WMR / ECH) == ch) {
 #pragma unroll
@@ -733,6 +740,7 @@
     prof_mark(p.prof, prof_slot, 62, prof_on);
     if (prof_on) p.prof[(long)prof_slot * 64 + 60] = wall_clock64();
   }
-}
-
-}
+  }
+}
+
+}
diff --git a/csrc/gemm_tiles.h b/csrc/gemm_tiles.h
--- a/csrc/gemm_tiles.h
+++ b/csrc/gemm_tiles.h
@@ -52,6 +52,7 @@
   X(0, 128, 96, 2, 4, 2, 23) X(1, 64, 96, 3, 4, 2, 24) X(2, 128, 192, 2, 4, 2, 27) X(3, 128, 128, 2, 4, 2, 25)   \
   X(4, 256, 192, 2, 8, 1, 5) X(5, 256, 128, 2, 8, 1, 7) X(6, 128, 128, 4, 8, 1, 6)                               \
   X(7, 128, 128, 4, 4, 1, 4) X(8, 128, 192, 3, 4, 1, 22)
+#define IIT_DUAL_ATTN_X_TILE_LIST(X) X(3, 128, 128, 2, 4, 2, 25)
 
 #define IIT_CONV_TILE_LIST(X)                                                 \
   X(0, 128, 64, 4, 4, 1) X(1, 128, 128, 3, 4, 1) X(2, 64, 64, 4, 4, 2)        \
@@ -66,6 +67,7 @@
 constexpr TileRow kEdgeRows[] = {IIT_EDGE_TILE_LIST(IIT_ROW_K64)};
 constexpr TileRow kDualWRows[] = {IIT_DUAL_W_TILE_LIST(IIT_ROW_DUAL)};
 constexpr TileRow kDualXRows[] = {IIT_DUAL_X_TILE_LIST(IIT_ROW_DUAL)};
+constexpr TileRow kDualAttnXRows[] = {IIT_DUAL_ATTN_X_TILE_LIST(IIT_ROW_DUAL)};
 constexpr TileRow kConvRows[] = {IIT_CONV_TILE_LIST(IIT_ROW_K64)};
 constexpr TileRow kConvWgRows[] = {IIT_CONV_WG_TILE_LIST(IIT_ROW_WG)};
 
@@ -87,6 +89,8 @@
     if (!same_tile(r, find_tile(kGldsRows, r.aux), false)) return false;
   for (const TileRow& r : kDualXRows)
     if (!same_tile(r, find_tile(kGldsRows, r.aux), false)) return false;
+  for (const TileRow& r : kDualAttnXRows)
+    if (!same_tile(r, find_tile(kDualXRows, r.id), true) || r.bm != 128 || r.bn != 128 || r.nw != 4) return false;
   return true;
 }
 static_assert(tile_lists_agree(), "gemm_tiles.h: an edge or dual row disagrees with the glds row it names");
diff --git a/iit_amd/ops/build.py b/iit_amd/ops/build.py
--- a/iit_amd/ops/build.py
+++ b/iit_amd/ops/build.py
@@ -14,7 +14,7 @@
            "splice.hip", "ioi_hl.hip", "bn_nhwc.hip", "gemm_f32.hip", "attn_fp32.hip", "block_f32.hip"]
 EXTRA_FLAGS = {"gemm_glds.hip": ["-mllvm", "-amdgpu-mfma-vgpr-form"], "gemm_edge.hip": ["-mllvm", "-amdgpu-mfma-vgpr-form"], "conv_nhwc.hip": ["-mllvm", "-amdgpu-mfma-vgpr-form"], "gemm_dual.hip": ["-mllvm", "-amdgpu-mfma-vgpr-form"],
                "gemm_8ph.hip": ["-mllvm", "-amdgpu-mfma-vgpr-form"]}
-HEADERS = ["common.h", "gemm_glds_body.h", "gemm_tiles.h", "gemm_w4.h", "splice_spec.h", "prefetch.h"]
+HEADERS = ["common.h", "attn_small_body.h", "gemm_glds_body.h", "gemm_tiles.h", "gemm_w4.h", "splice_spec.h", "prefetch.h"]
 ARCH = os.environ.get("IIT_OFFLOAD_ARCH", "gfx950")
 
 
diff --git a/iit_amd/ops/gemm_dispatch.py b/iit_amd/ops/gemm_dispatch.py
--- a/iit_amd/ops/gemm_dispatch.py
+++ b/iit_amd/ops/gemm_dispatch.py
@@ -597,16 +597,60 @@
     return out
 
 
-def gemm_pair(x: dict, w: dict, prefetch=None) -> Optional[str]:
+ATTN_BWD_FUSE = os.environ.get("IIT_ATTN_BWD_FUSE", "auto")
+
+
+def _attn_candidates(x: dict, w: dict, attn: dict, wc, bsum=None, gsq=None, dqkv=None):
+    ws, xs = _dual_specs(x, w, None, wc, None, bsum, gsq)
+    at = {**attn, "dqkv": attn["dqkv"] if dqkv is None else dqkv}
+    det = deterministic()
+    out = {}
+    for wt in K.DUAL_W_TILES:
+        if not all(K.dual_family_ok(wt, xt) for xt in K.DUAL_ATTN_X_TILES):
+            continue
+        for sp, red in ((1, False), (2, True), (4, True), (8, True), (2, False), (4, False), (8, False)):
+            if not red and sp > 1 and (w["epi"] != K.EPI_F32_ACC or det):
+                continue
+            if sp > 1 and w["K"] // sp < 256:
+                continue
+            name = f"attn{wt}" + (f"{'r' if red else 'k'}{sp}" if sp > 1 else "")
+            if K.gemm_dual_attn_ok(ws, xs, at, wt, sp, red) and not _excluded(name):
+                out[name] = lambda prefetch=None, wt=wt, sp=sp, red=red: K.gemm_dual_attn(ws, xs, at, wt, sp, red,
+                                                                                          prefetch=prefetch)
+    return out
+
+
+def _parse_attn(name: str):
+    import re
+    m = re.fullmatch(r"attn(\d+)(?:([rk])(\d+))?", name)
+    if m is None:
+        return None
+    return int(m.group(1)), int(m.group(3) or 1), m.group(2) == "r"
+
+
+def _attn_bwd(attn: dict, dz, dqkv=None) -> None:
+    S, H, dh = attn["S"], attn["H"], attn["dh"]
+    K.attn_small_bwd(attn["qkv"], dz, attn["lse"], attn["dqkv"] if dqkv is None else dqkv, attn["mask"],
+                     attn["rows"] // S, S, H, dh, attn["ld_qkv"], H * dh, attn["scale"], attn["causal"])
+
+
+def gemm_pair(x: dict, w: dict, prefetch=None, attn: Optional[dict] = None) -> Optional[str]:
     def serial():
         gemm(**x)
-        return gemm(**w)
-
+        res = gemm(**w)
+        if attn is not None:
+            _attn_bwd(attn, x["C"])
+        return res
+
+    if attn is not None and ATTN_BWD_FUSE == "0":
+        raise ValueError("gemm_pair: attn= with IIT_ATTN_BWD_FUSE=0")
     if not _dual_eligible(x, w):
         return serial()
     fresh = bool(w.get("fresh")) and w["epi"] == K.EPI_F32_STORE
     key = ("dual", x["M"], x["N"], x["K"], x["epi"], x.get("colsum") is not None,
            w["M"], w["N"], w["K"], w["epi"], fresh, deterministic())
+    if attn is not None:
+        key += ("attn", attn["S"], attn["H"]) + (("fused",) if ATTN_BWD_FUSE == "1" else ())
     choice = DUAL_DECISIONS.get(key)
     if choice is None:
         shipped = _table().get(repr(key))
@@ -624,6 +668,14 @@
         calls = _dual_candidates(x, w, xc, wc, cs, bs, sq)
         calls["serial"] = lambda: (gemm(**{**x, "C": xc, "colsum": cs}),
                                    gemm(**{**w, "C": wc, "bsum": bs, "gsq": sq}))
+        if attn is not None:
+            dq = torch.empty_like(attn["dqkv"])
+            calls = {n: (lambda f=f: (f(), _attn_bwd(attn, xc, dq))) for n, f in calls.items()}
+            if ATTN_BWD_FUSE == "1":
+                calls = {}
+            calls.update(_attn_candidates(x, w, attn, wc, bs, sq, dq))
+            if not calls:
+                raise ValueError(f"IIT_ATTN_BWD_FUSE=1: no fused configuration covers the pair {key!r}")
         times = {n: min(_time(f) for _ in range(2)) for n, f in calls.items()}
         for n in sorted(times, key=times.get)[:3] if len(times) > 1 else ():
             times[n] = min(_time(calls[n], reps=30) for _ in range(3))
@@ -631,17 +683,25 @@
         choice = DUAL_DECISIONS[key] = (best, times)
     name = FORCE.get(key, choice[0])
     cfg = _parse_dual(name)
+    acfg = _parse_attn(name) if attn is not None else None
     ws, xs = _dual_specs(x, w, x["C"], w["C"], x.get("colsum"), w.get("bsum"), w.get("gsq"))
-    if cfg is None or not K.gemm_dual_ok(ws, xs, *cfg):
+    if acfg is not None and not K.gemm_dual_attn_ok(ws, xs, attn, *acfg):
+        acfg = None
+    if acfg is None and (cfg is None or not K.gemm_dual_ok(ws, xs, *cfg)):
         name, cfg = "serial", None
     s_ev = e_ev = None
     if TIMING is not None:
         s_ev, e_ev = torch.cuda.Event(enable_timing=True), torch.cuda.Event(enable_timing=True)
         s_ev.record()
-    if cfg is None:
+    if acfg is not None:
+        K.gemm_dual_attn(ws, xs, attn, *acfg, prefetch=prefetch)
+        res = name
+    elif cfg is None:
         res = serial()
     else:
         K.gemm_dual(ws, xs, *cfg, prefetch=prefetch)
+        if attn is not None:
+            _attn_bwd(attn, x["C"])
         res = name
     if TIMING is not None:
         e_ev.record()
diff --git a/iit_amd/ops/hip_kernels.py b/iit_amd/ops/hip_kernels.py
--- a/iit_amd/ops/hip_kernels.py
+++ b/iit_amd/ops/hip_kernels.py
@@ -117,6 +117,11 @@
     "iit_gemm_dual_ok": [c_void_p] * 3 + [c_long] * 3 + [c_int] * 7 + [c_void_p] * 4 + [c_long] * 4 + [c_int] * 5,
     "iit_gemm_dual": [c_void_p] * 3 + [c_long] * 3 + [c_int] * 6 + [c_void_p] * 2 + [c_void_p] * 4 + [c_long] * 4
                      + [c_int] * 5 + [c_void_p] * 3 + [c_void_p, c_long, c_void_p, c_long, c_int, c_void_p],
+    "iit_gemm_dual_attn_ok": [c_void_p] * 3 + [c_long] * 3 + [c_int] * 7 + [c_void_p] * 2 + [c_long] * 2 + [c_int] * 3
+                             + [c_void_p] * 3 + [c_long] + [c_int] * 4 + [c_void_p],
+    "iit_gemm_dual_attn": [c_void_p] * 3 + [c_long] * 3 + [c_int] * 6 + [c_void_p] * 4 + [c_long] * 2 + [c_int] * 3
+                          + [c_void_p] * 5 + [c_long, c_ull] + [c_int] * 3 + [c_float, c_int, c_int, c_void_p]
+                          + [c_void_p, c_long, c_void_p, c_long, c_int, c_void_p],
     "iit_gemm_glds_set_group_m": [c_int],
     "iit_ioi_hl_label": [c_void_p, c_void_p, c_void_p, c_int, c_int, c_int, c_int, c_int, c_void_p, c_void_p],
     "iit_tile_table": [c_int, c_void_p, c_int],
@@ -150,7 +155,7 @@
     return _LIB
 
 
-TILE_FAMILIES = ("glds", "edge", "dual_w", "dual_x", "conv", "conv_wgrad")
+TILE_FAMILIES = ("glds", "edge", "dual_w", "dual_x", "conv", "conv_wgrad", "dual_attn_x")
 TILE_FIELDS = ("bm", "bn", "bk", "ns", "nw", "occ", "aux")
 
 
@@ -166,7 +171,8 @@
 def check_tile_tables(L=None) -> None:
     ours = {"glds": GLDS_TILES, "edge": {t: GLDS_TILES.get(t) for t in GLDS_EDGE_TILES}, "conv": CONV_TILES,
             "conv_wgrad": CONV_WG_TILES, "dual_w": {t: v + DUAL_W_WAVES.get(t, ()) for t, v in DUAL_W_TILES.items()},
-            "dual_x": {t: v + DUAL_X_WAVES.get(t, ()) for t, v in DUAL_X_TILES.items()}}
+            "dual_x": {t: v + DUAL_X_WAVES.get(t, ()) for t, v in DUAL_X_TILES.items()},
+            "dual_attn_x": {t: DUAL_X_TILES.get(t, ()) + DUAL_X_WAVES.get(t, ()) for t in DUAL_ATTN_X_TILES}}
     for family, mine in ours.items():
         theirs = {t: (r["bm"], r["bn"], r["nw"], r["occ"])[:4 if family.startswith("dual") else 2]
                   for t, r in tile_table(family, L).items()}
@@ -542,6 +548,7 @@
 
 DUAL_W_WAVES = {0: (4, 2), 1: (4, 2), 2: (4, 2), 3: (4, 2), 4: (4, 2), 5: (8, 1), 6: (8, 1), 7: (4, 1), 8: (4, 1)}
 DUAL_X_WAVES = {0: (4, 2), 1: (4, 2), 2: (4, 2), 3: (4, 2), 4: (8, 1), 5: (8, 1), 6: (8, 1), 7: (4, 1), 8: (4, 1)}
+DUAL_ATTN_X_TILES = (3,)
 
 
 def dual_family_ok(wtile: int, xtile: int) -> bool:
@@ -578,6 +585,52 @@
         x.get("ldc2", 0), x["M"], x["N"], x["K"], x["epi"], xtile, _p(x.get("csum")), _p(w.get("bsum")),
         _p(w.get("gsq")) if w["epi"] == EPI_F32_STORE else None, *_prefetch_args(prefetch), _stream()),
         "iit_gemm_dual")
+
+
+def _dual_attn_head(w: dict, x: dict, wtile: int, splits: int):
+    return (_p(w["A"]), _p(w["B"]), _p(w["C"]), w["lda"], w["ldb"], w["ldc"], w["M"], w["N"], w["K"], w["epi"], wtile,
+            splits)
+
+
+def _dual_attn_x(x: dict):
+    return (_p(x["A"]), _p(x["B"]), x["lda"], x["ldb"], x["M"], x["N"], x["K"])
+
+
+def gemm_dual_attn_ok(w: dict, x: dict, attn: dict, wtile: int, splits: int = 1, reduce: bool = False) -> bool:
+    if not _bf16_cuda(w["A"], w["B"], x["A"], x["B"], attn["qkv"], attn["dqkv"]):
+        return False
+    lse = attn["lse"]
+    if lse is None or not lse.is_cuda or lse.dtype != torch.float32:
+        return False
+    return bool(lib().iit_gemm_dual_attn_ok(
+        *_dual_attn_head(w, x, wtile, splits), int(reduce), *_dual_attn_x(x), _p(attn["qkv"]), _p(lse),
+        _p(attn["dqkv"]), attn["ld_qkv"], attn["S"], attn["H"], attn["dh"], int(attn.get("pair_seqs", 0)),
+        attn.get("spec")))
+
+
+def gemm_dual_attn(w: dict, x: dict, attn: dict, wtile: int, splits: int = 1, reduce: bool = False,
+                   prefetch=None) -> None:
+    if not gemm_dual_attn_ok(w, x, attn, wtile, splits, reduce):
+        raise ValueError(f"gemm_dual_attn: not covered (dX {x['M']}x{x['N']}x{x['K']}, S={attn['S']} H={attn['H']} "
+                         f"dh={attn['dh']} pair_seqs={attn.get('pair_seqs', 0)} spec={attn.get('spec') is not None}, "
+                         f"dW tile {wtile} splits {splits})")
+    ws = cnt = None
+    if reduce:
+        ws, cnt = split_workspace(w["M"], w["N"], DUAL_W_TILES[wtile], splits, w["A"].device)
+    qkv, dqkv, lse = attn["qkv"], attn["dqkv"], attn["lse"]
+    rows, S, H, dh, ld = x["M"], attn["S"], attn["H"], attn["dh"], attn["ld_qkv"]
+    _bounds("iit_gemm_dual_attn", ("qkv", qkv, rows, 3 * H * dh, ld), ("dqkv", dqkv, rows, 3 * H * dh, ld),
+            ("lse", lse, 1, rows * H, rows * H))
+    if CHECK_BOUNDS:
+        _gemm_bounds("iit_gemm_dual_attn(dW)", w["A"], w["B"], w["C"], None, None, w["M"], w["N"], w["K"], w["lda"],
+                     w["ldb"], w["ldc"], 0, 0, MODE_AKM | MODE_BKM)
+        _gemm_bounds("iit_gemm_dual_attn(dX)", x["A"], x["B"], None, None, None, x["M"], x["N"], x["K"],
+                     x["lda"], x["ldb"], x["N"], 0, 0, MODE_NN)
+    _check(lib().iit_gemm_dual_attn(
+        *_dual_attn_head(w, x, wtile, splits), _p(ws), _p(cnt), *_dual_attn_x(x), _p(w.get("bsum")),
+        _p(w.get("gsq")) if w["epi"] == EPI_F32_STORE else None, _p(qkv), _p(lse), _p(dqkv), ld,
+        int(attn.get("mask", 0)), S, H, dh, float(attn["scale"]), int(bool(attn["causal"])),
+        int(attn.get("pair_seqs", 0)), attn.get("spec"), *_prefetch_args(prefetch), _stream()), "iit_gemm_dual_attn")
 
 
 _PF_PER_MB = float(os.environ.get("IIT_DUAL_PREFETCH_WGS_PER_MB", "16"))
diff --git a/iit_amd/ops/hip_ops.py b/iit_amd/ops/hip_ops.py
--- a/iit_amd/ops/hip_ops.py
+++ b/iit_amd/ops/hip_ops.py
@@ -9,7 +9,7 @@
 
 from ..engine import grad_hooks
 from . import hip_kernels as K
-from .gemm_dispatch import gemm, gemm_pair
+from .gemm_dispatch import _attn_bwd, gemm, gemm_pair
 from .torch_ops import TorchOps, act_fn
 
 BF16 = torch.bfloat16
@@ -510,7 +510,58 @@
     return gW2, gW2.stride(0)
 
 
-def _wgrad_tail(ctx, xspec, x2, g2, ldg, Ws, C, ldc, store, gb):
+class _AttnLink:
+    __slots__ = ("qkv", "lse", "cfg", "dqkv", "stand_in")
+
+    def __init__(self, qkv, lse, cfg):
+        self.qkv, self.lse, self.cfg = qkv.detach(), lse, cfg
+        self.dqkv = self.stand_in = None
+
+
+_ZERO1: dict = {}
+
+
+def _zero1(device) -> torch.Tensor:
+    z = _ZERO1.get(device)
+    if z is None:
+        z = _ZERO1[device] = torch.zeros(1, dtype=BF16, device=device)
+    return z
+
+
+def _attn_fuse_on() -> bool:
+    from . import gemm_dispatch
+    return gemm_dispatch.ATTN_BWD_FUSE != "0"
+
+
+def _tag_attn(z):
+    link = getattr(getattr(z, "grad_fn", None), "attn_link", None)
+    if link is not None:
+        z._iit_attn = link
+    return z
+
+
+def _o_rows(z, shape):
+    x = z.reshape(*shape)
+    link = getattr(z, "_iit_attn", None)
+    if link is not None:
+        x._iit_attn = link
+    return x
+
+
+def _attn_spec(ctx, T: int, N: int):
+    link = getattr(ctx, "attn_link", None)
+    if link is None or not _attn_fuse_on() or link.dqkv is not None:
+        return None
+    B, S, _, H, dh = link.qkv.shape
+    if dh != 64 or S > 16 or 128 % S or B * S != T or H * dh != N or T % 128 or N % 128 or \
+            not link.qkv.is_contiguous() or not K._mfma_attn(S, dh):
+        return None
+    mask, causal, scale = link.cfg
+    return dict(qkv=link.qkv, lse=link.lse, dqkv=torch.empty_like(link.qkv), mask=mask, S=S, H=H, dh=dh, rows=T,
+                ld_qkv=3 * H * dh, scale=scale, causal=causal)
+
+
+def _wgrad_tail(ctx, xspec, x2, g2, ldg, Ws, C, ldc, store, gb, attn=None):
     bs = None
     if C is not None:
         T, N = g2.shape
@@ -518,11 +569,16 @@
         wspec = dict(A=x2, B=g2, C=C, M=x2.shape[1], N=N, K=T, lda=x2.shape[1], ldb=ldg, ldc=ldc,
                      mode=K.MODE_AKM | K.MODE_BKM, epi=K.EPI_F32_STORE if store else K.EPI_F32_ACC, fresh=store,
                      bsum=bs, gsq=_norm_slots(store, *Ws))
-        choice = gemm_pair(xspec, wspec, prefetch=_pf_next(ctx)) if xspec is not None else gemm(**wspec)
+        if xspec is not None:
+            choice = gemm_pair(xspec, wspec, prefetch=_pf_next(ctx), **({} if attn is None else {"attn": attn}))
+        else:
+            choice = gemm(**wspec)
         if store:
             _settle_claim(choice, *Ws)
     elif xspec is not None:
         gemm(**xspec)
+        if attn is not None:
+            _attn_bwd(attn, xspec["C"])
     return bs
 
 
@@ -605,6 +661,7 @@
         K.attn_small_fwd(qkv, z, lse, src, mask, B, S, H, dh, 3 * H * dh, H * dh, H * dh, scale, causal)
         ctx.save_for_backward(qkv, lse)
         ctx.cfg = (mask, causal, scale)
+        ctx.attn_link = _AttnLink(qkv, lse, ctx.cfg) if _attn_fuse_on() else None
         return z
 
     @staticmethod
@@ -614,9 +671,18 @@
         qkv, lse = ctx.saved_tensors
         mask, causal, scale = ctx.cfg
         B, S, _, H, dh = qkv.shape
+        link = getattr(ctx, "attn_link", None)
+        done = None
+        if link is not None and link.dqkv is not None:
+            done, stand_in = link.dqkv, link.stand_in
+            link.dqkv = link.stand_in = None
+            if dz.data_ptr() == stand_in.data_ptr() and not any(dz.stride()):
+                return done, None, None, None, None
         dz = dz.to(BF16).contiguous()
         dqkv = torch.empty_like(qkv)
         K.attn_small_bwd(qkv, dz, lse, dqkv, mask, B, S, H, dh, 3 * H * dh, H * dh, scale, causal)
+        if done is not None:
+            dqkv += done
         return dqkv, None, None, None, None
 
 
@@ -925,6 +991,7 @@
     _pf_register(ctx, xb, w)
     ctx.ldw = ldw
     ctx.meta = (x.shape[:-1], Kd, N, out_kind, x.dtype)
+    ctx.attn_link = getattr(x, "_iit_attn", None)
     return res
 
 
@@ -961,8 +1028,13 @@
                 dx = dxf.to(x_dtype).view(*lead, Kd)
         store, (gW,) = _wgrad_slots(True, W)
         gb = _grad_slot(b)
-        bs = _wgrad_tail(ctx, xspec, x2, g2, ldg, (W,), *_wgrad_rows(gW, Kd, N), store, gb)
-        if dxb is not None:
+        attn = _attn_spec(ctx, T, Kd) if xspec is not None and x_dtype == BF16 else None
+        bs = _wgrad_tail(ctx, xspec, x2, g2, ldg, (W,), *_wgrad_rows(gW, Kd, N), store, gb, attn)
+        if attn is not None:
+            link = ctx.attn_link
+            link.dqkv = attn["dqkv"]
+            link.stand_in = dx = _zero1(g2.device).expand(*lead, Kd)
+        elif dxb is not None:
             dx = (dxb if x_dtype == BF16 else dxb.to(x_dtype)).view(*lead, Kd)
         _bias_tail(bs, gb, g2, ldg, (b,), (W,))
         return dx, None, None, None, None, gres, None
@@ -1266,6 +1338,7 @@
             K.attn_small_fwd(qkv_full, z, lse, None, 0, B2, S, H, dh, 3 * H * dh, H * dh, H * dh, scale, causal)
         ctx.save_for_backward(qkv_full[:B], lse[:B * H * S])
         ctx.cfg = (mask, causal, scale)
+        ctx.attn_link = _AttnLink(qkv_full[:B], lse[:B * H * S], ctx.cfg) if _attn_fuse_on() else None
         box.append(z)
         return z[:B]
 
@@ -1463,16 +1536,16 @@
         if packed is None or getattr(k, "_iit_packed", None) is not packed or getattr(v, "_iit_packed", None) is not packed:
             packed = torch.stack([q, k, v], dim=2).to(BF16)
         mask = K.heads_to_mask(patch_heads)
-        return AttnFn.apply(packed, patch_src, mask, causal, 1.0 / attn_scale)
+        return _tag_attn(AttnFn.apply(packed, patch_src, mask, causal, 1.0 / attn_scale))
 
     def o_proj(self, z, W_O, b_O):
         B, S, H, dh = z.shape
-        return LinearFn.apply(z.reshape(B, S, H * dh), W_O, b_O, self._L(W_O)["o"], W_O.shape[-1], None, "bf16")
+        return LinearFn.apply(_o_rows(z, (B, S, H * dh)), W_O, b_O, self._L(W_O)["o"], W_O.shape[-1], None, "bf16")
 
     def o_proj_residual(self, z, W_O, b_O, resid):
         resid = _f32_of(resid)
         B, S, H, dh = z.shape
-        return LinearFn.apply(z.reshape(B, S, H * dh), W_O, b_O, self._L(W_O)["o"], W_O.shape[-1], resid, "resid")
+        return LinearFn.apply(_o_rows(z, (B, S, H * dh)), W_O, b_O, self._L(W_O)["o"], W_O.shape[-1], resid, "resid")
 
     def o_result(self, z, W_O):
         return torch.einsum("bshe,hed->bshd", z.to(BF16), W_O.to(BF16))
@@ -1588,7 +1661,7 @@
                        ) -> Paired:
         out, full = _one(AttnPairFn, p.base, causal, 1.0 / attn_scale, K.heads_to_mask(heads) if heads else 0,
                          p.full)
-        return Paired(out, full)
+        return Paired(_tag_attn(out), full)
 
     def pair_attention_spliced(self, p: Paired, causal: bool, attn_scale: float, index) -> Optional[Paired]:
         from .splice import patch_spec
@@ -1616,7 +1689,7 @@
         B2, S, H, dh = z.full.shape
         B = z.base.shape[0]
         rb, rf = resid.resid_operands()
-        out, full = _one(LinearPairFn, z.base.reshape(B, S, H * dh), W_O, b_O, self._L(W_O)["o"], W_O.shape[-1],
+        out, full = _one(LinearPairFn, _o_rows(z.base, (B, S, H * dh)), W_O, b_O, self._L(W_O)["o"], W_O.shape[-1],
                          rb, "resid", z.full.reshape(B2, S, H * dh), rf)
         return Paired(out, full)
 
```
